# Damo12320/OptixPathtracer

Measured on AMD Instinct MI355X. Metric: Msamples/sec at 1920x1080, max-depth 8; MSE vs reference, higher is better.
Workload: dtype f32; 1 GPU; BASELINE configs[1]: Diffuse sphere-in-box 1920x1080, 1024 spp, depth 8, 1xMI355X; scene=sphere_box_diffuse, triangles=34570, width=1920, height=1080, max_depth=8, material_mode=lambert, kernel=auto (wavefront), frames_per_launch=128, wavefront_streams=1, parallelism=spp-shard x1, batch_frames=128, queue_bytes=55207544320, queue_budget_bytes=77305217024, bvh_builder=auto (GPU binned SAH + GPU SAH-optimal BVH4 collapse), primary_dedup=True

## Files before the change

### include/ptamd.h

```cpp
#ifndef PTAMD_H
#define PTAMD_H
#include <stddef.h>
#include <stdint.h>

#ifdef __cplusplus
extern "C" {
#endif

#define PT_OK 0
#define PT_ERR_INVALID (-1)
#define PT_ERR_HIP (-2)
#define PT_ERR_STATE (-3)
#define PT_ERR_NOMEM (-4)

#define PT_MAT_DEFAULT 0
#define PT_MAT_LAMBERT 1
#define PT_MAT_CONDUCTOR 2
#define PT_MAT_DIELECTRIC 3
#define PT_MAT_LAYERED 4

#define PT_KERNEL_MEGA 0
#define PT_KERNEL_WAVEFRONT 1
#define PT_BVH_AUTO 0
#define PT_BVH_LBVH 1
// ... 21 lines not shown

typedef struct pt_texture {
    const uint32_t* rgba8;
    int32_t width;
    int32_t height;
} pt_texture;

typedef struct pt_scene {
    const pt_mesh* meshes;
    int32_t n_meshes;
    const pt_texture* textures;
    int32_t n_textures;
} pt_scene;

typedef struct pt_point_light {
    float position[3];
    float color[3];
} pt_point_light;

typedef struct pt_options {
    int32_t device;
    int32_t material_mode;
    int32_t kernel;
    int32_t bvh_builder;
    int32_t n_devices;
    int32_t reserved[3];
    const int32_t* device_list;
} pt_options;

typedef struct pt_stats {
    uint64_t segments;
    uint64_t samples;
    double last_render_ms;
    double total_render_ms;
    uint64_t render_calls;
    uint64_t kernel_launches;
    double bvh_build_ms;
    int32_t bvh_nodes;
    int32_t triangles;
    int32_t frames_per_launch;
    int32_t bvh_depth;
    uint64_t nodes_visited;
    uint64_t tri_tests;
    uint64_t rays;
    uint64_t stack_overflows;
    double trace_kernel_ms;
    uint64_t trace_kernel_launches;
    uint64_t shadow_rays;
    uint64_t trace_kernel_rays;
    uint64_t trace_kernel_bytes;
    uint64_t strict_retraces;
    uint64_t wave_steps;
    uint64_t wave_active_lanes;
    uint64_t wave_node_steps;
    uint64_t wave_tri_steps;
    uint64_t wave_refills;
    uint64_t lds_nodes_visited;
    double shade_kernel_ms;
    uint64_t shade_kernel_launches;
    uint64_t shade_kernel_items;
    uint64_t frames_rendered_ahead;
    uint64_t frames_served_ahead;
    uint64_t look_ahead_cancelled;
    double pair_kernel_ms;
    uint64_t pair_kernel_launches;
    uint64_t pair_kernel_rays;
    uint64_t pair_kernel_bytes;
    uint64_t pair_kernel_shadow_rays;
    uint64_t nee_unoccluded;
    uint64_t queue_bytes;
    uint64_t queue_budget;
    int32_t last_streams;
    int32_t last_batch_frames;
    uint64_t look_ahead_held;
    uint64_t lit_table_answers;
    uint64_t lit_table_cells;
    uint64_t lit_table_bits_set;
    uint64_t lit_table_bytes;
    double lit_table_build_ms;
    uint64_t occluder_table_bytes;
    uint64_t occluder_table_candidates;
    double occluder_table_build_ms;
    uint64_t occluder_table_answers;
    uint64_t geometry_commits;
    uint64_t geometry_refits;
    uint64_t geometry_rebuilds;
    double geometry_commit_ms;
    double bvh_sah_cost;
    double bvh_sah_cost_built;
} pt_stats;

typedef struct pt_renderer pt_renderer;

int pt_create(const pt_scene* scene, const pt_options* options, pt_renderer** out);
int pt_destroy(pt_renderer* r);

int pt_resize(pt_renderer* r, int32_t width, int32_t height);
int pt_set_camera(pt_renderer* r, const float position[3], const float inverse_view[16],
                  const float inverse_projection[16]);
int pt_set_lights(pt_renderer* r, const pt_point_light* lights, int32_t count);
int pt_set_max_bounces(pt_renderer* r, int32_t max_bounces);
int pt_set_material_mode(pt_renderer* r, int32_t material_mode);
int pt_set_kernel(pt_renderer* r, int32_t kernel);
int pt_set_frames_per_launch(pt_renderer* r, int32_t frames);
int pt_set_queue_budget(pt_renderer* r, int64_t bytes);
int pt_set_debug_hold(pt_renderer* r, int32_t on);
int pt_get_trace_coherence(pt_renderer* r, uint64_t hist[8]);
int pt_set_traversal_stats(pt_renderer* r, int32_t enable);
int pt_set_kernel_timing(pt_renderer* r, int32_t enable);
int pt_set_primary_dedup(pt_renderer* r, int32_t enable);
int pt_set_wavefront_streams(pt_renderer* r, int32_t streams);
int pt_set_band_split(pt_renderer* r, int32_t enable);
int pt_set_lit_table(pt_renderer* r, int32_t enable);
typedef struct pt_lit_table_info {
    int32_t active;
    int32_t lights;
    uint32_t triangles;
    uint32_t cells;
    uint32_t words_per_light;
    float delta;
    float margin;
} pt_lit_table_info;
int pt_lit_table_download(pt_renderer* r, pt_lit_table_info* info, uint32_t* tri_words, int64_t tri_bytes,
                          uint32_t* bits, int64_t bits_bytes);
int pt_set_occluder_table(pt_renderer* r, int32_t enable);
int pt_occluder_table_download(pt_renderer* r, int64_t* entries_out, int32_t* entries, int64_t bytes);
int pt_occluder_table_upload(pt_renderer* r, const int32_t* entries, int64_t bytes);

typedef struct pt_launch_params {
    struct {
        float* color_buffer;
        int32_t size[2];
        uint32_t id;
    } frame;
    struct {
        float position[3];
        float inverse_view_matrix[16];
        float inverse_projection_matrix[16];
    } camera;
    const pt_point_light* point_lights;
    int32_t point_light_count;
    int32_t max_bounces;
} pt_launch_params;

int pt_launch(pt_renderer* r, const pt_launch_params* params);

int pt_set_mesh_transform(pt_renderer* r, int32_t mesh, const float model_matrix[16]);
int pt_set_mesh_vertices(pt_renderer* r, int32_t mesh, const float* vertices, const float* normals);
#define PT_GEOM_REFIT 0
#define PT_GEOM_REBUILD 1
int pt_commit_geometry(pt_renderer* r, int32_t how);

int pt_render(pt_renderer* r, float* host_rgb);
int pt_set_render_ahead(pt_renderer* r, int32_t frames);
int pt_set_render_ahead_budget(pt_renderer* r, float max_ms);

int pt_accum_clear(pt_renderer* r);
int pt_render_frames(pt_renderer* r, uint32_t first_frame_id, uint32_t n_frames);
int pt_render_accumulate(pt_renderer* r, uint32_t spp, uint32_t first_frame_id, float* host_rgb_mean);
int pt_set_accum_device_buffer(pt_renderer* r, float* device_sum_rgb);
float* pt_accum_device_ptr(pt_renderer* r);
int pt_accum_download(pt_renderer* r, float* host_rgb, float scale);
int pt_set_accum_fp64(pt_renderer* r, int32_t on);
double* pt_accum_device_ptr64(pt_renderer* r);
int pt_accum_download64(pt_renderer* r, double* host_rgb);

int pt_synchronize(pt_renderer* r);
void* pt_stream(pt_renderer* r);
int32_t pt_device_count(const pt_renderer* r);
int pt_devices(const pt_renderer* r, int32_t* devices, int32_t max);
uint32_t pt_frame_id(const pt_renderer* r);
int pt_set_frame_id(pt_renderer* r, uint32_t frame_id);
int pt_get_stats(pt_renderer* r, pt_stats* out);
int pt_stats_reset(pt_renderer* r);

int pt_camera_from_blender(const float blender_position[3], const float blender_rotation_deg[3],
                           float fov_deg, int32_t width, int32_t height, float position[3],
                           float inverse_view[16], float inverse_projection[16]);

int pt_trace_rays(pt_renderer* r, const float* host_rays, int32_t n, int32_t* prim, float* t,
                  float* u, float* v, int32_t* backface, int32_t any_hit);

typedef struct pt_debug_bounce {
    int32_t bounce;
    int32_t prim;
    float position[3];
    float albedo[3];
    float shading_normal[3];
    float geometry_normal[3];
    float roughness, metallic;
    float beta[3];
    float radiance[3];
} pt_debug_bounce;
int pt_set_debug_pixel(pt_renderer* r, int32_t x, int32_t y, uint32_t frame_id);
int pt_get_debug_path(pt_renderer* r, pt_debug_bounce* out, int32_t max, int32_t* n_bounces);

int pt_bvh_download(pt_renderer* r, void* nodes, int64_t node_bytes, void* triangles, int64_t triangle_bytes);

const char* pt_last_error(void);
const char* pt_version(void);

int pt_display_reset(pt_renderer* r, int32_t max_samples);
int pt_display_add_frame(pt_renderer* r, int32_t* samples);
int pt_display_download(pt_renderer* r, float* rgb);

#define PT_AOV_ALBEDO 0
#define PT_AOV_NORMAL 1
#define PT_AOV_GEOM_NORMAL 2
#define PT_AOV_POSITION 3
#define PT_AOV_DEPTH 4
// ... 99 lines not shown
```

### optixpathtracer_amd/capi.py

```python
from __future__ import annotations

import ctypes as C
import os
from pathlib import Path

_HERE = Path(__file__).resolve().parent
LIB_PATH = _HERE / "libptamd.so"

PT_MAT_DEFAULT, PT_MAT_LAMBERT, PT_MAT_CONDUCTOR, PT_MAT_DIELECTRIC, PT_MAT_LAYERED = range(5)
PT_KERNEL_MEGA, PT_KERNEL_WAVEFRONT, PT_KERNEL_AUTO = 0, 1, 2
PT_BVH_AUTO, PT_BVH_LBVH, PT_BVH_SAH, PT_BVH_PLOC, PT_BVH_SAH_GPU = 0, 1, 2, 3, 4
PT_GEOM_REFIT, PT_GEOM_REBUILD = 0, 1
PT_OK, PT_ERR_INVALID, PT_ERR_HIP, PT_ERR_STATE, PT_ERR_NOMEM = 0, -1, -2, -3, -4

MATERIAL_MODES = {
    "default": PT_MAT_DEFAULT,
    "lambert": PT_MAT_LAMBERT,
    "conductor": PT_MAT_CONDUCTOR,
    "dielectric": PT_MAT_DIELECTRIC,
    "layered": PT_MAT_LAYERED,
}


class PTError(RuntimeError):
# ... 40 lines not shown

class pt_options(C.Structure):
    _fields_ = [
        ("device", C.c_int32),
        ("material_mode", C.c_int32),
        ("kernel", C.c_int32),
        ("bvh_builder", C.c_int32),
        ("n_devices", C.c_int32),
        ("reserved", C.c_int32 * 3),
        ("device_list", C.POINTER(C.c_int32)),
    ]


class pt_debug_bounce(C.Structure):
    _fields_ = [
        ("bounce", C.c_int32),
        ("prim", C.c_int32),
        ("position", C.c_float * 3),
        ("albedo", C.c_float * 3),
        ("shading_normal", C.c_float * 3),
        ("geometry_normal", C.c_float * 3),
        ("roughness", C.c_float),
        ("metallic", C.c_float),
        ("beta", C.c_float * 3),
        ("radiance", C.c_float * 3),
    ]


class pt_stats(C.Structure):
    _fields_ = [
        ("segments", C.c_uint64),
        ("samples", C.c_uint64),
        ("last_render_ms", C.c_double),
        ("total_render_ms", C.c_double),
        ("render_calls", C.c_uint64),
        ("kernel_launches", C.c_uint64),
        ("bvh_build_ms", C.c_double),
        ("bvh_nodes", C.c_int32),
        ("triangles", C.c_int32),
        ("frames_per_launch", C.c_int32),
        ("bvh_depth", C.c_int32),
        ("nodes_visited", C.c_uint64),
        ("tri_tests", C.c_uint64),
        ("rays", C.c_uint64),
        ("stack_overflows", C.c_uint64),
        ("trace_kernel_ms", C.c_double),
        ("trace_kernel_launches", C.c_uint64),
        ("shadow_rays", C.c_uint64),
        ("trace_kernel_rays", C.c_uint64),
        ("trace_kernel_bytes", C.c_uint64),
        ("strict_retraces", C.c_uint64),
        ("wave_steps", C.c_uint64),
        ("wave_active_lanes", C.c_uint64),
        ("wave_node_steps", C.c_uint64),
        ("wave_tri_steps", C.c_uint64),
        ("wave_refills", C.c_uint64),
        ("lds_nodes_visited", C.c_uint64),
        ("shade_kernel_ms", C.c_double),
        ("shade_kernel_launches", C.c_uint64),
        ("shade_kernel_items", C.c_uint64),
        ("frames_rendered_ahead", C.c_uint64),
        ("frames_served_ahead", C.c_uint64),
        ("look_ahead_cancelled", C.c_uint64),
        ("pair_kernel_ms", C.c_double),
        ("pair_kernel_launches", C.c_uint64),
        ("pair_kernel_rays", C.c_uint64),
        ("pair_kernel_bytes", C.c_uint64),
        ("pair_kernel_shadow_rays", C.c_uint64),
        ("nee_unoccluded", C.c_uint64),
        ("queue_bytes", C.c_uint64),
        ("queue_budget", C.c_uint64),
        ("last_streams", C.c_int32),
        ("last_batch_frames", C.c_int32),
        ("look_ahead_held", C.c_uint64),
        ("lit_table_answers", C.c_uint64),
        ("lit_table_cells", C.c_uint64),
        ("lit_table_bits_set", C.c_uint64),
        ("lit_table_bytes", C.c_uint64),
        ("lit_table_build_ms", C.c_double),
        ("occluder_table_bytes", C.c_uint64),
        ("occluder_table_candidates", C.c_uint64),
        ("occluder_table_build_ms", C.c_double),
        ("occluder_table_answers", C.c_uint64),
        ("geometry_commits", C.c_uint64),
        ("geometry_refits", C.c_uint64),
        ("geometry_rebuilds", C.c_uint64),
        ("geometry_commit_ms", C.c_double),
        ("bvh_sah_cost", C.c_double),
        ("bvh_sah_cost_built", C.c_double),
    ]


class pt_lit_table_info(C.Structure):
    _fields_ = [("active", C.c_int32), ("lights", C.c_int32), ("triangles", C.c_uint32), ("cells", C.c_uint32),
                ("words_per_light", C.c_uint32), ("delta", C.c_float), ("margin", C.c_float)]


PT_AOV_ALBEDO, PT_AOV_NORMAL, PT_AOV_GEOM_NORMAL, PT_AOV_POSITION, PT_AOV_DEPTH, PT_AOV_PRIM, PT_AOV_ROUGH_METAL = range(7)
PT_DENOISE_SRC_ACCUM, PT_DENOISE_SRC_DISPLAY, PT_DENOISE_SRC_HOST = range(3)

AOV_KINDS = {
    "albedo": PT_AOV_ALBEDO,
    "normal": PT_AOV_NORMAL,
    "geom_normal": PT_AOV_GEOM_NORMAL,
    "position": PT_AOV_POSITION,
    "depth": PT_AOV_DEPTH,
    "prim": PT_AOV_PRIM,
    "rough_metal": PT_AOV_ROUGH_METAL,
}


class pt_denoise_options(C.Structure):
    _fields_ = [("struct_size", C.c_uint32), ("iterations", C.c_int32), ("demodulate", C.c_int32),
                ("sigma_color", C.c_float), ("sigma_normal", C.c_float), ("sigma_position", C.c_float),
                ("albedo_floor", C.c_float)]


class pt_denoise_info(C.Structure):
    _fields_ = [("struct_size", C.c_uint32), ("iterations", C.c_int32), ("gbuffer_renders", C.c_uint64),
                ("hit_pixels", C.c_uint64), ("gbuffer_ms", C.c_double), ("filter_ms", C.c_double)]


PT_TEMPORAL_HISTORY_LENGTH, PT_TEMPORAL_MOMENTS, PT_TEMPORAL_VARIANCE, PT_TEMPORAL_COLOR = range(4)

TEMPORAL_KINDS = {
    "history_length": PT_TEMPORAL_HISTORY_LENGTH,
    "moments": PT_TEMPORAL_MOMENTS,
    "variance": PT_TEMPORAL_VARIANCE,
    "color": PT_TEMPORAL_COLOR,
}


class pt_temporal_options(C.Structure):
    _fields_ = [("struct_size", C.c_uint32), ("alpha", C.c_float), ("alpha_moments", C.c_float),
                ("max_history", C.c_int32), ("normal_cos", C.c_float), ("plane_distance", C.c_float),
                ("sigma_luminance", C.c_float), ("variance_history", C.c_int32), ("motion_vectors", C.c_int32)]


class pt_temporal_info(C.Structure):
    _fields_ = [("struct_size", C.c_uint32), ("history_valid", C.c_int32), ("calls", C.c_uint64),
                ("reprojected_pixels", C.c_uint64), ("reset_pixels", C.c_uint64), ("temporal_ms", C.c_double),
                ("variance_ms", C.c_double), ("filter_ms", C.c_double), ("moved_pixels", C.c_uint64),
                ("snapshot_ms", C.c_double), ("motion_used", C.c_int32), ("reserved", C.c_int32)]


PT_MOTION_BARYCENTRIC, PT_MOTION_PREV_POSITION, PT_MOTION_SCREEN = range(3)

MOTION_KINDS = {
    "barycentric": PT_MOTION_BARYCENTRIC,
    "prev_position": PT_MOTION_PREV_POSITION,
    "screen": PT_MOTION_SCREEN,
}


class _pt_launch_frame(C.Structure):
    _fields_ = [("color_buffer", C.c_void_p), ("size", C.c_int32 * 2), ("id", C.c_uint32)]


class _pt_launch_camera(C.Structure):
    _fields_ = [("position", C.c_float * 3), ("inverse_view_matrix", C.c_float * 16),
                ("inverse_projection_matrix", C.c_float * 16)]


class pt_launch_params(C.Structure):
    _fields_ = [("frame", _pt_launch_frame), ("camera", _pt_launch_camera), ("point_lights", C.c_void_p),
                ("point_light_count", C.c_int32), ("max_bounces", C.c_int32)]


_FP = C.POINTER(C.c_float)
_IP = C.POINTER(C.c_int32)
_R = C.c_void_p
_M = C.c_void_p
pt_image_decode_fn = C.CFUNCTYPE(C.c_int, C.c_void_p, C.c_size_t, C.POINTER(C.c_int32), C.POINTER(C.c_int32),
                                 C.c_void_p, C.c_void_p)

SIGNATURES = {
    "pt_create": (C.c_int, [C.POINTER(pt_scene), C.POINTER(pt_options), C.POINTER(C.c_void_p)]),
    "pt_destroy": (C.c_int, [_R]),
    "pt_resize": (C.c_int, [_R, C.c_int32, C.c_int32]),
    "pt_set_camera": (C.c_int, [_R, _FP, _FP, _FP]),
    "pt_set_lights": (C.c_int, [_R, C.POINTER(pt_point_light), C.c_int32]),
    "pt_set_max_bounces": (C.c_int, [_R, C.c_int32]),
    "pt_set_material_mode": (C.c_int, [_R, C.c_int32]),
    "pt_set_kernel": (C.c_int, [_R, C.c_int32]),
    "pt_set_mesh_transform": (C.c_int, [_R, C.c_int32, _FP]),
    "pt_set_mesh_vertices": (C.c_int, [_R, C.c_int32, _FP, _FP]),
    "pt_commit_geometry": (C.c_int, [_R, C.c_int32]),
    "pt_set_frames_per_launch": (C.c_int, [_R, C.c_int32]),
    "pt_set_render_ahead": (C.c_int, [_R, C.c_int32]),
    "pt_set_render_ahead_budget": (C.c_int, [_R, C.c_float]),
    "pt_set_queue_budget": (C.c_int, [_R, C.c_int64]),
    "pt_get_trace_coherence": (C.c_int, [_R, C.POINTER(C.c_uint64)]),
    "pt_set_debug_hold": (C.c_int, [_R, C.c_int32]),
    "pt_set_traversal_stats": (C.c_int, [_R, C.c_int32]),
    "pt_set_kernel_timing": (C.c_int, [_R, C.c_int32]),
    "pt_render": (C.c_int, [_R, _FP]),
    "pt_launch": (C.c_int, [_R, C.POINTER(pt_launch_params)]),
    "pt_accum_clear": (C.c_int, [_R]),
    "pt_render_frames": (C.c_int, [_R, C.c_uint32, C.c_uint32]),
    "pt_set_primary_dedup": (C.c_int, [_R, C.c_int32]),
    "pt_set_band_split": (C.c_int, [_R, C.c_int32]),
    "pt_set_wavefront_streams": (C.c_int, [_R, C.c_int32]),
    "pt_set_lit_table": (C.c_int, [_R, C.c_int32]),
    "pt_lit_table_download": (C.c_int, [_R, C.POINTER(pt_lit_table_info), C.c_void_p, C.c_int64, C.c_void_p,
                                        C.c_int64]),
    "pt_set_occluder_table": (C.c_int, [_R, C.c_int32]),
    "pt_occluder_table_download": (C.c_int, [_R, C.POINTER(C.c_int64), C.c_void_p, C.c_int64]),
    "pt_occluder_table_upload": (C.c_int, [_R, C.c_void_p, C.c_int64]),
    "pt_render_accumulate": (C.c_int, [_R, C.c_uint32, C.c_uint32, _FP]),
    "pt_set_accum_device_buffer": (C.c_int, [_R, C.c_void_p]),
    "pt_accum_device_ptr": (C.c_void_p, [_R]),
    "pt_accum_download": (C.c_int, [_R, _FP, C.c_float]),
    "pt_set_accum_fp64": (C.c_int, [_R, C.c_int32]),
    "pt_accum_device_ptr64": (C.c_void_p, [_R]),
    "pt_accum_download64": (C.c_int, [_R, C.POINTER(C.c_double)]),
    "pt_synchronize": (C.c_int, [_R]),
    "pt_stream": (C.c_void_p, [_R]),
    "pt_device_count": (C.c_int32, [_R]),
    "pt_devices": (C.c_int, [_R, C.POINTER(C.c_int32), C.c_int32]),
    "pt_frame_id": (C.c_uint32, [_R]),
    "pt_set_frame_id": (C.c_int, [_R, C.c_uint32]),
    "pt_get_stats": (C.c_int, [_R, C.POINTER(pt_stats)]),
    "pt_stats_reset": (C.c_int, [_R]),
    "pt_camera_from_blender": (C.c_int, [_FP, _FP, C.c_float, C.c_int32, C.c_int32, _FP, _FP, _FP]),
    "pt_trace_rays": (C.c_int, [_R, _FP, C.c_int32, _IP, _FP, _FP, _FP, _IP, C.c_int32]),
    "pt_bvh_download": (C.c_int, [_R, C.c_void_p, C.c_int64, C.c_void_p, C.c_int64]),
    "pt_set_debug_pixel": (C.c_int, [_R, C.c_int32, C.c_int32, C.c_uint32]),
    "pt_get_debug_path": (C.c_int, [_R, C.POINTER(pt_debug_bounce), C.c_int32, C.POINTER(C.c_int32)]),
    "pt_last_error": (C.c_char_p, []),
    "pt_version": (C.c_char_p, []),
    "pt_display_reset": (C.c_int, [_R, C.c_int32]),
    "pt_display_add_frame": (C.c_int, [_R, C.POINTER(C.c_int32)]),
    "pt_display_download": (C.c_int, [_R, _FP]),
    "pt_aov_channels": (C.c_int, [C.c_int32]),
    "pt_aov_download": (C.c_int, [_R, C.c_int32, C.c_void_p, C.c_int64]),
    "pt_aov_device_ptr": (C.c_void_p, [_R, C.c_int32]),
    "pt_denoise_options_default": (C.c_int, [C.POINTER(pt_denoise_options)]),
    "pt_denoise": (C.c_int, [_R, C.c_int32, _FP, C.c_float, C.POINTER(pt_denoise_options), _FP]),
    "pt_denoised_device_ptr": (C.c_void_p, [_R]),
    "pt_get_denoise_info": (C.c_int, [_R, C.POINTER(pt_denoise_info)]),
    "pt_temporal_options_default": (C.c_int, [C.POINTER(pt_temporal_options)]),
    "pt_denoise_temporal": (C.c_int, [_R, C.c_int32, _FP, C.c_float, C.POINTER(pt_temporal_options),
                                      C.POINTER(pt_denoise_options), _FP]),
    "pt_temporal_reset": (C.c_int, [_R]),
    "pt_temporal_channels": (C.c_int, [C.c_int32]),
    "pt_temporal_download": (C.c_int, [_R, C.c_int32, C.c_void_p, C.c_int64]),
    "pt_get_temporal_info": (C.c_int, [_R, C.POINTER(pt_temporal_info)]),
    "pt_motion_channels": (C.c_int, [C.c_int32]),
    "pt_motion_download": (C.c_int, [_R, C.c_int32, C.c_void_p, C.c_int64]),
    "pt_model_load_gltf": (C.c_int, [C.c_char_p, pt_image_decode_fn, C.c_void_p, C.POINTER(_M)]),
    "pt_model_scene": (C.POINTER(pt_scene), [_M]),
    "pt_model_mesh_name": (C.c_char_p, [_M, C.c_int32]),
    "pt_model_destroy": (C.c_int, [_M]),
    "pt_model_last_error": (C.c_char_p, []),
    "pt_image_decode_png": (C.c_int, [C.c_void_p, C.c_size_t, C.POINTER(C.c_int32), C.POINTER(C.c_int32),
                                      C.c_void_p]),
    "pt_image_write_exr": (C.c_int, [C.c_char_p, _FP, C.c_int32, C.c_int32]),
    "pt_image_write_bmp": (C.c_int, [C.c_char_p, _FP, C.c_int32, C.c_int32]),
    "pt_image_write_pfm": (C.c_int, [C.c_char_p, _FP, C.c_int32, C.c_int32]),
    "pt_image_read": (C.c_int, [C.c_char_p, _FP, C.POINTER(C.c_int32), C.POINTER(C.c_int32)]),
    "pt_image_mse": (C.c_double, [_FP, _FP, C.c_int64]),
    "pt_image_flip": (C.c_double, [_FP, _FP, C.c_int32, C.c_int32, C.c_float, _FP]),
    "pt_image_last_error": (C.c_char_p, []),
}

_lib = None


def load(path: str | os.PathLike | None = None) -> C.CDLL:
    global _lib
    if _lib is not None and path is None:
        return _lib
    p = Path(path) if path else Path(os.environ.get("PTAMD_LIB", LIB_PATH))
    if not p.exists():
        raise PTError(
            f"{p} not found: the HIP extension is not built (run `python -c 'import __graft_entry__ as g; g.build()'`)"
        )
    lib = C.CDLL(str(p))
    variant = path is None and "PTAMD_LIB" in os.environ
    for name, (res, args) in SIGNATURES.items():
        if variant and not hasattr(lib, name):
            continue
        fn = getattr(lib, name)
        fn.restype = res
        fn.argtypes = args
    if path is None:
        _lib = lib
    return lib


def check(status: int, what: str = "") -> None:
# ... 12 lines not shown
```

### optixpathtracer_amd/csrc/pt_capi.cpp

```cpp
#include "pt_renderer.h"

using namespace pt;

namespace pt {

thread_local std::string g_last_error;

int fail(int code, const std::string& msg) {
    g_last_error = msg;
    return code;
}
int hip_fail(hipError_t e, const char* where) {
    g_last_error = std::string(where) + ": " + hipGetErrorString(e);
    return e == hipErrorOutOfMemory ? PT_ERR_NOMEM : PT_ERR_HIP;
}

}

pt_renderer::~pt_renderer() {
    wavefront_free(wf);
    for (int k = 1; k < kMaxWFStreams; ++k) wavefront_free(xwf[k]);
}

namespace {
// ... 744 lines not shown
    *n_bounces = 0;
    if (!r->d_debug) return fail(PT_ERR_STATE, "pt_get_debug_path: call pt_set_debug_pixel first");
    PT_HIP(hipSetDevice(r->device), "hipSetDevice");
    PT_HIP(hipStreamSynchronize(r->stream), "hipStreamSynchronize");
    std::vector<pt_debug_bounce> rec(kDebugMaxBounces);
    PT_HIP(hipMemcpy(rec.data(), r->d_debug, sizeof(pt_debug_bounce) * rec.size(), hipMemcpyDeviceToHost),
           "download debug records");
    int n = 0;
    while (n < kDebugMaxBounces && rec[(size_t)n].bounce == n + 1) ++n;
    *n_bounces = n;
    for (int k = 0; k < n && k < max; ++k) out[k] = rec[(size_t)k];
    return PT_OK;
}

extern "C" int pt_set_traversal_stats(pt_renderer* r, int32_t enable) {
    if (!r) return fail(PT_ERR_INVALID, "pt_set_traversal_stats: NULL");
    r->trav_stats = enable != 0;
    for (pt_renderer* p : r->multi.peers) p->trav_stats = enable != 0;
    return PT_OK;
}

extern "C" int pt_set_wavefront_streams(pt_renderer* r, int32_t streams) {
    if (!r || streams < 0 || streams > pt_renderer::kMaxWFStreams)
        return fail(PT_ERR_INVALID, "pt_set_wavefront_streams: 0 (auto) or 1 to 4");
    int rc = collect_pending(r);
    if (rc != PT_OK) return rc;
    r->wf_streams = streams;
    for (pt_renderer* p : r->multi.peers)
        if ((rc = pt_set_wavefront_streams(p, streams)) != PT_OK) return rc;
    return PT_OK;
}

extern "C" int pt_set_primary_dedup(pt_renderer* r, int32_t enable) {
    if (!r) return fail(PT_ERR_INVALID, "pt_set_primary_dedup: NULL");
    int rc = collect_pending(r);
    if (rc) return rc;
    r->primary_dedup = enable != 0;
    for (pt_renderer* p : r->multi.peers) {
        if ((rc = pt_set_primary_dedup(p, enable)) != PT_OK) return rc;
    }
    return PT_OK;
}

extern "C" int pt_set_lit_table(pt_renderer* r, int32_t enable) {
    if (!r) return fail(PT_ERR_INVALID, "pt_set_lit_table: NULL");
    const int mode = enable < 0 ? -1 : (enable > 0 ? 1 : 0);
    r->lit.mode = mode;
    for (pt_renderer* p : r->multi.peers) p->lit.mode = mode;
    return PT_OK;
}

extern "C" int pt_lit_table_download(pt_renderer* r, pt_lit_table_info* info, uint32_t* tri_words, int64_t tri_bytes,
                                     uint32_t* bits, int64_t bits_bytes) {
    if (!r || !info) return fail(PT_ERR_INVALID, "pt_lit_table_download: NULL");
    PT_HIP(hipSetDevice(r->device), "hipSetDevice");
    return lit_table_download(r, info, tri_words, tri_bytes, bits, bits_bytes);
}

extern "C" int pt_set_occluder_table(pt_renderer* r, int32_t enable) {
    if (!r) return fail(PT_ERR_INVALID, "pt_set_occluder_table: NULL");
    const int mode = enable < 0 ? -1 : (enable > 0 ? 1 : 0);
    r->occ.mode = mode;
    for (pt_renderer* p : r->multi.peers) p->occ.mode = mode;
    return PT_OK;
}

extern "C" int pt_occluder_table_download(pt_renderer* r, int64_t* entries_out, int32_t* entries, int64_t bytes) {
    if (!r || !entries_out) return fail(PT_ERR_INVALID, "pt_occluder_table_download: NULL");
    PT_HIP(hipSetDevice(r->device), "hipSetDevice");
    return occ_table_download(r, entries_out, entries, bytes);
}

extern "C" int pt_occluder_table_upload(pt_renderer* r, const int32_t* entries, int64_t bytes) {
    if (!r || !entries) return fail(PT_ERR_INVALID, "pt_occluder_table_upload: NULL");
    PT_HIP(hipSetDevice(r->device), "hipSetDevice");
    int rc = occ_table_upload(r, entries, bytes);
    if (rc) return rc;
    for (pt_renderer* p : r->multi.peers) {
        if ((rc = pt_occluder_table_upload(p, entries, bytes)) != PT_OK) return rc;
    }
    return PT_OK;
}

extern "C" int pt_set_band_split(pt_renderer* r, int32_t enable) {
    if (!r) return fail(PT_ERR_INVALID, "pt_set_band_split: NULL");
    int rc = collect_pending(r);
    if (rc) return rc;
    r->band_split = enable != 0;
    for (pt_renderer* p : r->multi.peers) {
        if ((rc = pt_set_band_split(p, enable)) != PT_OK) return rc;
    }
    return PT_OK;
}

extern "C" int pt_set_kernel_timing(pt_renderer* r, int32_t enable) {
    if (!r) return fail(PT_ERR_INVALID, "pt_set_kernel_timing: NULL");
    int rc = collect_pending(r);
    if (rc) return rc;
    r->timing.kernel_timing = enable != 0;
    for (pt_renderer* p : r->multi.peers) {
        if ((rc = pt_set_kernel_timing(p, enable)) != PT_OK) return rc;
    }
    return PT_OK;
}
```

### optixpathtracer_amd/csrc/pt_capi_launch.cpp

```cpp
#include "pt_renderer.h"

using namespace pt;

namespace {

int next_event_pair(pt_renderer* r, hipEvent_t* a, hipEvent_t* b) {
    PT_HIP(r->timing.ev.next(a, b), "hipEventCreate");
    return PT_OK;
}

DevLaunch make_launch(const pt_renderer* r, float* accum, uint32_t frame_base, uint32_t n_frames,
                      double* accum64 = nullptr, size_t frame_stride = 0) {
    DevLaunch L;
    L.width = r->width;
    L.height = r->height;
    L.row0 = 0;
    L.image_height = r->height;
    std::memcpy(L.cam_pos, r->cam_pos, sizeof L.cam_pos);
    std::memcpy(L.inv_view, r->inv_view, sizeof L.inv_view);
    std::memcpy(L.inv_proj, r->inv_proj, sizeof L.inv_proj);
    L.lights = r->d_lights;
    L.n_lights = r->n_lights;
    L.max_bounces = r->max_bounces;
    L.frame_base = frame_base;
    L.n_frames = n_frames;
    L.accum = accum;
    L.accum64 = accum64;
    L.frame_stride = frame_stride;
    L.counters = r->d_counters;
    L.debug_pixel = r->d_debug ? r->debug_pixel : -1;
    L.debug_frame = r->debug_frame;
    L.debug = r->d_debug;
    L.lit_tri = r->lit.active ? r->lit.d_tri.get() : nullptr;
    L.lit_bits = r->lit.d_bits;
    L.lit_words = r->lit.words;
    L.occ_tab = r->lit.active && r->occ.active ? r->occ.d_tab.get() : nullptr;
    L.lit_cells = r->lit.cells;
    return L;
}

}

namespace pt {

size_t queue_bytes_held(const pt_renderer* r) {
    size_t b = r->wf.paths > 0 ? wavefront_bytes(r->wf.paths, r->wf.max_bounces) : 0;
    for (int k = 1; k < pt_renderer::kMaxWFStreams; ++k)
        if (r->xwf[k].paths > 0) b += wavefront_bytes(r->xwf[k].paths, r->xwf[k].max_bounces);
    return b;
}

size_t queue_budget_bytes(const pt_renderer* r) {
    if (r->queue_budget < 0) return SIZE_MAX;
    if (r->queue_budget > 0) return (size_t)r->queue_budget;
    size_t total = 0;
    if (hipDeviceTotalMem(&total, r->device) != hipSuccess || total == 0) {
        (void)hipGetLastError();
        return SIZE_MAX;
    }
    return total / 4;
}

}

namespace {

constexpr int kMaxWFPaths = 1 << 28;

struct WFPlan {
    int nf_cap = 1;
    int ns = 1;
    bool bands = false;
};

int reserve_queues(pt_renderer* r, WFPlan* plan, size_t budget) {
    const int P = r->width * r->height;
    const int maxb = std::max(1, r->max_bounces);
    int& nf_cap = plan->nf_cap;
    for (int k = 0; k < plan->ns; ++k) {
        WFState& w = k ? r->xwf[k] : r->wf;
        const bool over = budget != SIZE_MAX && w.paths > P &&
                          (size_t)plan->ns * wavefront_bytes(w.paths, w.max_bounces) > budget;
        if (w.paths < P * nf_cap || w.max_bounces < r->max_bounces || over) {
            for (int j = 0; j < pt_renderer::kMaxWFStreams; ++j)
                if (r->wf_stream(j)) PT_HIP(hipStreamSynchronize(r->wf_stream(j)), "hipStreamSynchronize");
            wavefront_free(w);
            hipError_t ae = wavefront_alloc(w, P * nf_cap, maxb);
            if (ae == hipErrorOutOfMemory && k == 0) {
                bool freed = false;
                for (int j = 1; j < pt_renderer::kMaxWFStreams; ++j)
                    if (r->xwf[j].paths > 0) {
                        wavefront_free(r->xwf[j]);
                        freed = true;
                    }
                if (freed) ae = wavefront_alloc(w, P * nf_cap, maxb);
            }
            while (ae == hipErrorOutOfMemory && k == 0 && nf_cap > 1) {
                nf_cap = (nf_cap + 1) / 2;
                r->nf_fit = nf_cap;
                ae = wavefront_alloc(w, P * nf_cap, maxb);
            }
            if (ae == hipErrorOutOfMemory && k > 0) {
                plan->ns = k;
                break;
            }
            PT_HIP(ae, "wavefront_alloc");
        }
    }
    return PT_OK;
}

int plan_wavefront(pt_renderer* r, uint32_t n, WFPlan* plan) {
    const int P = r->width * r->height;
    const int maxb = std::max(1, r->max_bounces);
    const int nf_full = std::max(1, std::min({r->frames_per_launch, (int)std::min<uint32_t>(n, 1u << 20),
                                              kMaxWFPaths / std::max(1, P)}));
    if (r->nf_fit > 0 && r->nf_fit < nf_full) {
        size_t free_b = 0, total_b = 0;
        if (hipMemGetInfo(&free_b, &total_b) == hipSuccess) {
            if (free_b + queue_bytes_held(r) >= wavefront_bytes(P * nf_full, maxb)) r->nf_fit = 0;
// ... 10 lines not shown
    const size_t budget = queue_budget_bytes(r);
    if (budget != SIZE_MAX) {
        const size_t per_frame = wavefront_bytes(P, maxb);
        const int nf_b = (int)std::max<size_t>(1, budget / ((size_t)ns * per_frame));
        nf_cap = std::min(nf_cap, nf_b);
        size_t used = (size_t)ns * wavefront_bytes(P * nf_cap, maxb);
        for (int k = ns; k < pt_renderer::kMaxWFStreams; ++k) {
            if (r->xwf[k].paths == 0) continue;
            const size_t held = wavefront_bytes(r->xwf[k].paths, r->xwf[k].max_bounces);
            if (used + held <= budget) {
                used += held;
                continue;
            }
            PT_HIP(hipStreamSynchronize(r->xstream[k]), "hipStreamSynchronize");
            wavefront_free(r->xwf[k]);
        }
    }
    plan->nf_cap = nf_cap;
    plan->ns = ns;
    plan->bands = bands;
    const int rc = reserve_queues(r, plan, budget);
    if (rc != PT_OK) return rc;
    r->last_streams = plan->ns;
    r->last_batch = plan->nf_cap;
    return PT_OK;
}

int fork_resources(pt_renderer* r, int ns, int nband) {
    if (ns > 1) {
        PT_HIP(r->ev_fork.ensure(hipEventDisableTiming), "hipEventCreate");
        for (Event& e : r->ev_accum) PT_HIP(e.ensure(hipEventDisableTiming), "hipEventCreate");
    }
    for (int k = 1; k < ns; ++k)
        if (!r->xstream[k]) {
            PT_HIP(r->xstream[k].create(), "hipStreamCreate");
            PT_HIP(r->ev_join[k].ensure(hipEventDisableTiming), "hipEventCreate");
        }
    if (nband > 1) PT_HIP(r->ev_band0.ensure(hipEventDisableTiming), "hipEventCreate");
    return PT_OK;
}

int timing_events(pt_renderer* r, bool fused, const hipEvent_t** tev, const hipEvent_t** sev) {
    pt_renderer::Timing& t = r->timing;
    *tev = *sev = nullptr;
    if (!t.kernel_timing) return PT_OK;
    t.tev_frame.resize(2 * (size_t)(r->max_bounces + 1));
    for (int k = 0; k <= r->max_bounces; ++k)
        PT_HIP((k > 0 && fused ? t.pev : t.tev).next(&t.tev_frame[2 * k], &t.tev_frame[2 * k + 1]), "hipEventCreate");
    *tev = t.tev_frame.data();
    t.sev_frame.resize(2 * (size_t)(r->max_bounces + 1));
    for (int k = 0; k <= r->max_bounces; ++k)
        PT_HIP(t.sev.next(&t.sev_frame[2 * k], &t.sev_frame[2 * k + 1]), "hipEventCreate");
    *sev = t.sev_frame.data();
    return PT_OK;
}

WFState batch_queues(pt_renderer* r, int sk, bool speculative, bool first_batch) {
    WFState wq = sk ? r->xwf[sk] : r->wf;
    if (speculative && r->ahead.d_cancel_seen) {
        wq.cancel_host = r->ahead.cancel.d;
        wq.cancel_seen = r->ahead.d_cancel_seen;
        wq.cancel_epoch = r->ahead.cancel_epoch;
        if (r->ahead.debug_hold && r->ahead.hold.d && first_batch) {
            wq.hold_release = r->ahead.hold.d;
            r->ahead.held++;
        }
    }
    return wq;
}

int enqueue_wavefront(pt_renderer* r, const WFPlan& plan, float* accum, uint32_t first, uint32_t n, double* accum64,
                      size_t frame_stride, bool speculative) {
    int rc = PT_OK;
    const DevScene S = r->scene();
    const bool fused = r->material_mode == PT_MAT_LAMBERT || r->material_mode == PT_MAT_CONDUCTOR ||
                       r->material_mode == PT_MAT_DIELECTRIC;
    const int ns = plan.ns, nf_cap = plan.nf_cap;
    const bool dual = ns > 1;
    const int nband = plan.bands && ns > 1 ? 2 : 1;
    if ((rc = fork_resources(r, ns, nband)) != PT_OK) return rc;
    int dev_cus = 256;
    (void)hipDeviceGetAttribute(&dev_cus, hipDeviceAttributeMultiprocessorCount, r->device);
    if ((rc = lit_prepare(r)) != PT_OK) return rc;
    hipEvent_t a = nullptr, b = nullptr;
    if (dual) {
        rc = next_event_pair(r, &a, &b);
        if (rc) return rc;
        PT_HIP(hipEventRecord(a, r->stream), "hipEventRecord");
        PT_HIP(hipEventRecord(r->ev_fork, r->stream), "hipEventRecord");
        for (int k = 1; k < ns; ++k) PT_HIP(hipStreamWaitEvent(r->xstream[k], r->ev_fork, 0), "hipStreamWaitEvent");
    }
    const int rows0 = r->height * 7 / 16;
    r->band0_rows = nband > 1 ? rows0 : 0;
    int batch = 0;
    for (uint32_t f = 0; f < n; ++batch) {
        const int nf = (int)std::min<uint32_t>((uint32_t)nf_cap, n - f);
        DevLaunch L = make_launch(r, frame_stride ? accum + (size_t)f * frame_stride : accum, first + f,
                                  (uint32_t)nf, accum64, frame_stride);
        const int band = nband > 1 ? batch : 0;
        if (nband > 1) {
            L.row0 = band == 0 ? 0 : rows0;
            L.height = band == 0 ? rows0 : r->height - rows0;
            const size_t off = 3 * (size_t)r->width * (size_t)L.row0;
            L.accum += off;
            if (L.accum64) L.accum64 += off;
        }
        const int sk = batch % ns;
        hipStream_t st = r->wf_stream(sk);
        if (!dual) {
            rc = next_event_pair(r, &a, &b);
            if (rc) return rc;
        }
        const hipEvent_t* tev = nullptr;
        const hipEvent_t* sev = nullptr;
        if ((rc = timing_events(r, fused, &tev, &sev)) != PT_OK) return rc;
        if (!dual) PT_HIP(hipEventRecord(a, r->stream), "hipEventRecord");
        int n_timed = 0, n_stimed = 0;
        const WFState wq = batch_queues(r, sk, speculative, batch == 0);
        const hipEvent_t accum_wait = dual && batch > 0 && nband == 1 ? r->ev_accum[(batch - 1) & 1].e : nullptr;
        const hipEvent_t accum_done = dual && nband == 1 ? r->ev_accum[batch & 1].e : nullptr;
        PT_HIP(launch_wavefront_frame(r->material_mode, r->trav_stats, S, L, wq, first + f,
                                      nf, r->primary_dedup, dev_cus, st, tev, &n_timed,
                                      accum_wait, accum_done, sev, &n_stimed, ns == 1 && r->wide_trace),
               "wavefront launch");
        if (tev) {
            const int unused = r->max_bounces + 1 - n_timed;
            const int unused_pair = fused ? std::min(unused, r->max_bounces) : 0;
            r->timing.pev.give_back((size_t)unused_pair);
            r->timing.tev.give_back((size_t)(unused - unused_pair));
        }
        if (sev) r->timing.sev.give_back((size_t)(r->max_bounces + 1 - n_stimed));
        if (!dual) PT_HIP(hipEventRecord(b, r->stream), "hipEventRecord");
        if (nband > 1 && band == 0) PT_HIP(hipEventRecord(r->ev_band0, st), "hipEventRecord");
        if (band + 1 == nband) f += (uint32_t)nf;
    }
    if (dual) {
        for (int k = 1; k < ns; ++k) {
            PT_HIP(hipEventRecord(r->ev_join[k], r->xstream[k]), "hipEventRecord");
            PT_HIP(hipStreamWaitEvent(r->stream, r->ev_join[k], 0), "hipStreamWaitEvent");
        }
        PT_HIP(hipEventRecord(b, r->stream), "hipEventRecord");
    }
    return PT_OK;
}

int enqueue_megakernel(pt_renderer* r, int kernel, float* accum, uint32_t first, uint32_t n) {
    const DevScene S = r->scene();
    const uint32_t chunk = (uint32_t)std::max(1, r->frames_per_launch);
    for (uint32_t done = 0; done < n;) {
        uint32_t k = std::min(chunk, n - done);
        DevLaunch L = make_launch(r, accum, first + done, k);
        hipEvent_t a, b;
        const int rc = next_event_pair(r, &a, &b);
        if (rc) return rc;
        PT_HIP(hipEventRecord(a, r->stream), "hipEventRecord");
        PT_HIP(launch_render(kernel, r->material_mode, r->trav_stats, S, L, r->stream), "render launch");
        PT_HIP(hipEventRecord(b, r->stream), "hipEventRecord");
        done += k;
    }
    return PT_OK;
}

}

namespace pt {

int launch_frames(pt_renderer* r, float* accum, uint32_t first, uint32_t n, double* accum64, size_t frame_stride,
                  bool speculative) {
    int rc = PT_OK;
    const pt_renderer::Timing& t = r->timing;
    if (t.ev.used + t.tev.used + t.pev.used + t.sev.used > kMaxPendingEvents && (rc = collect_pending(r)) != PT_OK)
        return rc;
    r->timing.pending = true;
    r->band0_rows = 0;
    r->lit.active = false;
    int kernel = r->kernel;
    if (kernel == PT_KERNEL_AUTO) kernel = PT_KERNEL_WAVEFRONT;
    if (accum64 && kernel != PT_KERNEL_WAVEFRONT)
        return fail(PT_ERR_INVALID, "fp64 accumulation (pt_set_accum_fp64) runs with the wavefront kernel");
    if (frame_stride && kernel != PT_KERNEL_WAVEFRONT)
        return fail(PT_ERR_INVALID, "per-frame images (render-ahead) run with the wavefront kernel");
    if (kernel == PT_KERNEL_WAVEFRONT) {
        WFPlan plan;
        if ((rc = plan_wavefront(r, n, &plan)) != PT_OK) return rc;
        rc = enqueue_wavefront(r, plan, accum, first, n, accum64, frame_stride, speculative);
    } else {
        rc = enqueue_megakernel(r, kernel, accum, first, n);
    }
    if (rc != PT_OK) return rc;
    r->timing.samples += (uint64_t)n * (uint64_t)r->width * (uint64_t)r->height;
    r->timing.calls++;
    return PT_OK;
}

int render_frames_multi(pt_renderer* r, uint32_t first, uint32_t n) {
    const int N = (int)r->multi.comms.size();
    const size_t count = 3 * (size_t)r->width * (size_t)r->height;
    uint32_t f = first;
    for (int g = 0; g < N; ++g) {
        const uint32_t per = n / (uint32_t)N, extra = n % (uint32_t)N;
        const uint32_t ng = per + ((uint32_t)g < extra ? 1u : 0u);
        pt_renderer* d = g == 0 ? r : r->multi.peers[(size_t)g - 1];
        if (ng > 0) {
            PT_HIP(hipSetDevice(d->device), "hipSetDevice");
            const int rc = launch_frames(d, g == 0 ? r->multi.d_part : d->accum(), f, ng,
                                         r->accum64 ? (g == 0 ? r->multi.d_part64 : d->d_accum64) : nullptr);
            if (rc) return rc;
        }
        f += ng;
    }
    ncclResult_t nr = ncclGroupStart();
    for (int g = 0; g < N && nr == ncclSuccess; ++g) {
        pt_renderer* d = g == 0 ? r : r->multi.peers[(size_t)g - 1];
        if (r->accum64) {
            const double* send = g == 0 ? r->multi.d_part64 : d->d_accum64;
            double* recv = g == 0 ? r->d_accum64 : d->d_accum64;
            nr = ncclReduce(send, recv, count, ncclFloat64, ncclSum, 0, r->multi.comms[(size_t)g], d->stream);
        } else {
            const float* send = g == 0 ? r->multi.d_part : d->accum();
            float* recv = g == 0 ? r->accum() : d->accum();
            nr = ncclReduce(send, recv, count, ncclFloat32, ncclSum, 0, r->multi.comms[(size_t)g], d->stream);
        }
    }
    const ncclResult_t ne = ncclGroupEnd();
    (void)hipSetDevice(r->device);
    if (nr != ncclSuccess || ne != ncclSuccess)
        return fail(PT_ERR_HIP, std::string("ncclReduce: ") + ncclGetErrorString(nr != ncclSuccess ? nr : ne));
    if (r->accum64) PT_HIP(accum_f64_to_f32(r->d_accum64, r->accum(), count, r->stream), "fp64 -> fp32 sum");
    return PT_OK;
}

}
```

### optixpathtracer_amd/csrc/pt_capi_scene.cpp

```cpp
#include "pt_renderer.h"

using namespace pt;

namespace {

int need_tex_kernels(pt_renderer* r) {
    if (r->d_texinfo) return PT_OK;
    bool any = false;
    for (int m = 0; m < r->nmesh; ++m) any = any || r->geom.host.normal_mode(m) == 2;
    if (!any) return PT_OK;
    PT_HIP(r->d_texinfo.alloc(1), "hipMalloc texinfo");
    PT_HIP(hipMemset(r->d_texinfo, 0, sizeof(int4)), "hipMemset texinfo");
    return PT_OK;
}

int build_tree(pt_renderer* r, const std::vector<float4>& tri, const std::vector<float4>& nrm, const float cmin[3],
               const float cmax[3], BuildOutput& bo, float* ms_out = nullptr) {
    const size_t ntri = tri.size() / 3;
    DevBuf<float4> d_uv_orig, d_nrm_orig, d_tri_orig;
    hipError_t e = d_tri_orig.alloc(3 * ntri);
    if (e == hipSuccess) e = d_nrm_orig.alloc(3 * ntri);
    if (e == hipSuccess && bo.tuv) e = d_uv_orig.alloc(2 * ntri);
    if (e == hipSuccess && bo.tuv)
        e = hipMemcpyAsync(d_uv_orig, r->geom.host.uvs.data(), sizeof(float4) * 2 * ntri, hipMemcpyHostToDevice,
// ... 96 lines not shown
    r->d_isect.swap(isect);
    r->d_shade.swap(shade);
    r->d_tuv.swap(tuv);
    r->bvh_nodes = bo.n_nodes;
    r->bvh_depth = bo.depth;
    r->geom.level_base = bo.level_base;
    r->geom.commit_ms += bms;
    return PT_OK;
}

}

namespace pt {

int upload_scene(pt_renderer* r, const pt_scene* scene, const std::vector<int4>& texinfo, size_t ntexel) {
    const std::vector<float4>& mats = r->geom.mats;
    const int ntex = scene->n_textures;
    PT_HIP(r->stream.create(), "hipStreamCreate");
    PT_HIP(r->dl_stream.create(), "hipStreamCreate");
    PT_HIP(r->xstream[1].create(), "hipStreamCreate");
    PT_HIP(r->ev_join[1].ensure(hipEventDisableTiming), "hipEventCreate");
    PT_HIP(r->d_counters.alloc(kCounters), "hipMalloc counters");
    PT_HIP(hipMemsetAsync(r->d_counters, 0, kCounters * sizeof(unsigned long long), r->stream), "hipMemset");
    PT_HIP(r->d_mats.alloc(mats.size()), "hipMalloc mats");
    PT_HIP(hipMemcpyAsync(r->d_mats, mats.data(), sizeof(float4) * mats.size(), hipMemcpyHostToDevice, r->stream),
           "upload mats");
    if (ntex > 0) {
        PT_HIP(r->d_texinfo.alloc((size_t)ntex), "hipMalloc texinfo");
        PT_HIP(hipMemcpyAsync(r->d_texinfo, texinfo.data(), sizeof(int4) * (size_t)ntex, hipMemcpyHostToDevice,
                              r->stream),
               "upload texinfo");
        PT_HIP(r->d_texels.alloc(ntexel), "hipMalloc texels");
        for (int k = 0; k < ntex; ++k) {
            const pt_texture& tx = scene->textures[k];
            PT_HIP(hipMemcpy(r->d_texels + texinfo[(size_t)k].x, tx.rgba8,
                             sizeof(uint32_t) * (size_t)tx.width * (size_t)tx.height, hipMemcpyHostToDevice),
                   "upload texels");
        }
    }
    return need_tex_kernels(r);
}

int build_scene(pt_renderer* r, bool any_tex) {
    const size_t ntri = (size_t)r->ntri;
    if (ntri > 0) {
        std::vector<float4> tri, nrm;
        float cmin[3], cmax[3];
        bake_scene(r->geom.host, tri, nrm, cmin, cmax);
        if (any_tex) PT_HIP(r->d_tuv.alloc(2 * ntri), "hipMalloc tuv");
        PT_HIP(r->d_isect.alloc(3 * ntri), "hipMalloc isect");
        PT_HIP(r->d_shade.alloc(4 * ntri), "hipMalloc shade");
        PT_HIP(r->d_nodes.alloc(std::max<size_t>(1, ntri)), "hipMalloc nodes");
        BuildOutput bo;
        bo.nodes = r->d_nodes;
        bo.isect = r->d_isect;
        bo.shade = r->d_shade;
        bo.tuv = r->d_tuv;
        int rc = build_tree(r, tri, nrm, cmin, cmax, bo);
        if (rc != PT_OK) return rc;
        r->bvh_nodes = bo.n_nodes;
        r->bvh_depth = bo.depth;
        r->geom.level_base = bo.level_base;
        if (3 * bo.depth > kMinTraversalStack)
            return fail(PT_ERR_INVALID, "pt_create: BVH too deep for the traversal stack (depth " +
                                            std::to_string(bo.depth) + ")");
        const size_t nv = r->geom.host.verts.size();
        PT_HIP(r->geom.d_overts.alloc(std::max<size_t>(1, nv)), "hipMalloc vertices");
        PT_HIP(r->geom.d_onorms.alloc(std::max<size_t>(1, nv)), "hipMalloc normals");
        PT_HIP(r->geom.d_tidx.alloc(ntri), "hipMalloc indices");
        PT_HIP(r->geom.d_rmesh.alloc((size_t)std::max(1, r->nmesh)), "hipMalloc mesh records");
        PT_HIP(r->geom.d_sah_part.alloc((size_t)sah_partial_blocks((int)ntri) + 1), "hipMalloc SAH partials");
        PT_HIP(r->geom.ev[0].ensure(), "hipEventCreate");
        PT_HIP(r->geom.ev[1].ensure(), "hipEventCreate");
        if (nv > 0) {
            PT_HIP(hipMemcpy(r->geom.d_overts, r->geom.host.verts.data(), sizeof(float4) * nv, hipMemcpyHostToDevice),
                   "upload vertices");
            PT_HIP(hipMemcpy(r->geom.d_onorms, r->geom.host.norms.data(), sizeof(float4) * nv, hipMemcpyHostToDevice),
                   "upload normals");
        }
        PT_HIP(hipMemcpy(r->geom.d_tidx, r->geom.host.tidx.data(), sizeof(int4) * ntri, hipMemcpyHostToDevice),
               "upload indices");
        if ((rc = sah_cost_now(r, true)) != PT_OK) return rc;
        if ((rc = lit_resubdivide(r)) != PT_OK) return rc;
    }
    PT_HIP(hipStreamSynchronize(r->stream), "hipStreamSynchronize");
    return PT_OK;
}

int commit_geometry(pt_renderer* r, int how) {
    cancel_look_ahead(r, true);
    PT_HIP(hipStreamSynchronize(r->stream), "hipStreamSynchronize");
    for (int k = 1; k < pt_renderer::kMaxWFStreams; ++k)
        if (r->xstream[k]) PT_HIP(hipStreamSynchronize(r->xstream[k]), "hipStreamSynchronize");
    if (r->dl_stream) PT_HIP(hipStreamSynchronize(r->dl_stream), "hipStreamSynchronize");
    int rc = collect_pending(r);
    if (rc) return rc;

    std::vector<RefitMesh> rm((size_t)std::max(1, r->nmesh));
    if ((rc = apply_staged(r, rm)) != PT_OK) return rc;
    r->geom.any_staged = false;
    r->geom.version++;
    r->geom.commits++;
    r->geom.commit_ms = 0.0;
    if (r->ntri <= 0) {
        if (how == PT_GEOM_REBUILD) r->geom.rebuilds++;
        else r->geom.refits++;
        return PT_OK;
    }

    PT_HIP(hipMemcpy(r->d_mats, r->geom.mats.data(), sizeof(float4) * r->geom.mats.size(), hipMemcpyHostToDevice),
           "upload mats");
    if ((rc = need_tex_kernels(r)) != PT_OK) return rc;
    PT_HIP(hipMemcpy(r->geom.d_rmesh, rm.data(), sizeof(RefitMesh) * rm.size(), hipMemcpyHostToDevice),
           "upload mesh records");
    PT_HIP(hipEventRecord(r->geom.ev[0], r->stream), "hipEventRecord");
    PT_HIP(refit_rebake(r->geom.d_rmesh, r->geom.d_overts, r->geom.d_onorms, r->geom.d_tidx, r->ntri, r->d_isect,
                        r->d_shade, r->stream),
           "k_rebake");
    PT_HIP(refit_levels(r->d_nodes, r->d_isect, r->geom.level_base, r->stream), "k_refit_level");
    if ((rc = sah_cost_now(r, false, r->geom.ev[1])) != PT_OK) return rc;
    float ms = 0.0f;
    PT_HIP(hipEventElapsedTime(&ms, r->geom.ev[0], r->geom.ev[1]), "hipEventElapsedTime");
    r->geom.commit_ms = ms;

    int rebuild_rc = PT_OK;
    std::string rebuild_msg;
    if (how == PT_GEOM_REBUILD) {
        rebuild_rc = rebuild_tree(r);
        if (rebuild_rc != PT_OK) rebuild_msg = g_last_error;
        if (rebuild_rc == PT_OK && (rc = sah_cost_now(r, true)) != PT_OK) return rc;
    }
    if (how == PT_GEOM_REBUILD && rebuild_rc == PT_OK) r->geom.rebuilds++;
    else r->geom.refits++;

    if ((rc = lit_resubdivide(r)) != PT_OK) return rc;
    if (rebuild_rc != PT_OK) return fail(rebuild_rc, rebuild_msg);
    return PT_OK;
}

}
```

### optixpathtracer_amd/csrc/pt_capi_stats.cpp

```cpp
#include "pt_renderer.h"

using namespace pt;

namespace pt {

int collect_pending(pt_renderer* r) {
    if (!r->timing.pending) return PT_OK;
    double sum = 0.0, tsum = 0.0, ssum = 0.0;
    size_t n = 0, tn = 0, sn = 0;
    PT_HIP(r->timing.ev.collect(&sum, &n), "frame events");
    PT_HIP(r->timing.tev.collect(&tsum, &tn), "trace-kernel events");
    double psum = 0.0;
    size_t pn = 0;
    PT_HIP(r->timing.pev.collect(&psum, &pn), "pair-kernel events");
    tsum += psum;
    tn += pn;
    r->timing.pair_ms += psum;
    r->timing.pair_launches += pn;
    PT_HIP(r->timing.sev.collect(&ssum, &sn), "shading-kernel events");
    r->ahead.spec_pending = false;
    r->timing.launches += n;
    r->timing.last_ms = sum;
    r->timing.total_ms += sum;
    r->timing.trace_ms += tsum;
    r->timing.trace_launches += tn;
    r->timing.shade_ms += ssum;
    r->timing.shade_launches += sn;
    r->timing.pending = false;
    return PT_OK;
}

}

namespace {

constexpr uint64_t pt_stats::*kSummed[] = {
    &pt_stats::segments, &pt_stats::samples, &pt_stats::nodes_visited, &pt_stats::tri_tests, &pt_stats::rays,
    &pt_stats::stack_overflows, &pt_stats::wave_steps, &pt_stats::wave_active_lanes, &pt_stats::wave_node_steps,
    &pt_stats::wave_tri_steps, &pt_stats::wave_refills, &pt_stats::lds_nodes_visited, &pt_stats::shade_kernel_items,
    &pt_stats::shadow_rays, &pt_stats::trace_kernel_rays, &pt_stats::trace_kernel_bytes, &pt_stats::strict_retraces,
    &pt_stats::nee_unoccluded,
    &pt_stats::pair_kernel_rays, &pt_stats::pair_kernel_bytes, &pt_stats::pair_kernel_shadow_rays,
    &pt_stats::lit_table_answers, &pt_stats::occluder_table_answers, &pt_stats::queue_bytes};

int table_stats(pt_renderer* r, pt_stats* out) {
    r->lit.built.harvest();
    if (lit_wanted(r) && table_current(r, r->lit.built)) {
        const size_t nw = (size_t)r->lit.words * (size_t)r->lit.built.n;
        if (r->lit.built.count < 0) {
            std::vector<uint32_t> hb(nw);
            PT_HIP(hipMemcpy(hb.data(), r->lit.d_bits, sizeof(uint32_t) * nw, hipMemcpyDeviceToHost),
                   "download lit table");
            int64_t n = 0;
            for (uint32_t w : hb) n += __builtin_popcount(w);
            r->lit.built.count = n;
        }
        out->lit_table_cells = r->lit.cells;
        out->lit_table_bits_set = (uint64_t)r->lit.built.count;
        out->lit_table_bytes = sizeof(uint32_t) * ((size_t)r->ntri + (size_t)r->lit.words * kLitMaxLights);
        out->lit_table_build_ms = r->lit.built.build_ms;
    }
    r->occ.built.harvest();
    if (occ_wanted(r) && r->occ.d_tab && table_current(r, r->occ.built)) {
        const size_t ne = (size_t)r->lit.cells * (size_t)r->occ.built.n;
        if (r->occ.built.count < 0) {
            std::vector<int> ho(ne);
            PT_HIP(hipMemcpy(ho.data(), r->occ.d_tab, sizeof(int) * ne, hipMemcpyDeviceToHost), "download occluder table");
            int64_t n = 0;
            for (int t : ho) n += t >= 0;
            r->occ.built.count = n;
        }
        out->occluder_table_bytes = sizeof(int) * ne;
        out->occluder_table_candidates = (uint64_t)r->occ.built.count;
        out->occluder_table_build_ms = r->occ.built.build_ms;
    }
    return PT_OK;
}

}

extern "C" {

int pt_get_stats(pt_renderer* r, pt_stats* out) {
    if (!r || !out) return fail(PT_ERR_INVALID, "pt_get_stats: NULL");
    int rc = pt_synchronize(r);
    if (rc) return rc;
    unsigned long long c[kCounters];
    PT_HIP(hipMemcpy(c, r->d_counters, sizeof c, hipMemcpyDeviceToHost), "download counters");
    std::memset(out, 0, sizeof *out);
    out->segments = c[kCtrSegments];
    out->samples = r->timing.samples;
    out->last_render_ms = r->timing.last_ms;
    out->total_render_ms = r->timing.total_ms;
    out->render_calls = r->timing.calls;
    out->kernel_launches = r->timing.launches;
    out->frames_per_launch = r->frames_per_launch;
    out->bvh_build_ms = r->timing.bvh_ms;
    out->bvh_nodes = r->bvh_nodes;
    out->bvh_depth = r->bvh_depth;
    out->nodes_visited = c[kCtrNodes];
    out->tri_tests = c[kCtrTriTests];
    out->rays = c[kCtrRays];
    out->stack_overflows = c[kCtrStackOverflows];
    out->triangles = r->ntri;
    out->trace_kernel_ms = r->timing.trace_ms;
    out->trace_kernel_launches = r->timing.trace_launches;
    out->pair_kernel_ms = r->timing.pair_ms;
    out->pair_kernel_launches = r->timing.pair_launches;
    out->shadow_rays = c[kCtrShadowRays];
    out->trace_kernel_rays = c[kCtrTraceRays];
    out->trace_kernel_bytes = c[kCtrTraceBytes];
    out->strict_retraces = c[kCtrRetraces];
    out->wave_steps = c[kCtrWaveSteps];
    out->wave_active_lanes = c[kCtrWaveActive];
    out->wave_node_steps = c[kCtrWaveNodeSteps];
    out->wave_tri_steps = c[kCtrWaveTriSteps];
    out->wave_refills = c[kCtrWaveRefills];
    out->lds_nodes_visited = c[kCtrLdsNodes];
    out->shade_kernel_ms = r->timing.shade_ms;
    out->shade_kernel_launches = r->timing.shade_launches;
    out->shade_kernel_items = c[kCtrShadeItems];
    out->frames_rendered_ahead = r->ahead.rendered;
    out->frames_served_ahead = r->ahead.served;
    out->look_ahead_cancelled = r->ahead.cancelled;
    out->pair_kernel_rays = c[kCtrPairRays];
    out->pair_kernel_bytes = c[kCtrPairBytes];
    out->pair_kernel_shadow_rays = c[kCtrPairShadowRays];
    out->nee_unoccluded = c[kCtrNeeUnoccluded];
    out->queue_bytes = queue_bytes_held(r);
    const size_t qb = queue_budget_bytes(r);
    out->queue_budget = qb == SIZE_MAX ? 0 : qb;
    out->last_streams = r->last_streams;
    out->last_batch_frames = r->last_batch;
    out->look_ahead_held = r->ahead.held;
    out->lit_table_answers = c[kCtrLitAnswers];
    out->occluder_table_answers = c[kCtrOccAnswers];
    if ((rc = table_stats(r, out)) != PT_OK) return rc;
    out->geometry_commits = r->geom.commits;
    out->geometry_refits = r->geom.refits;
    out->geometry_rebuilds = r->geom.rebuilds;
    out->geometry_commit_ms = r->geom.commit_ms;
    out->bvh_sah_cost = r->geom.sah_cost;
    out->bvh_sah_cost_built = r->geom.sah_cost_built;
    for (pt_renderer* p : r->multi.peers) {
        pt_stats ps;
        rc = pt_get_stats(p, &ps);
        if (rc) return rc;
        for (uint64_t pt_stats::*f : kSummed) out->*f += ps.*f;
    }
    return PT_OK;
}

int pt_stats_reset(pt_renderer* r) {
    if (!r) return fail(PT_ERR_INVALID, "pt_stats_reset: NULL");
    int rc = pt_synchronize(r);
    if (rc) return rc;
    for (pt_renderer* p : r->multi.peers) {
        if ((rc = pt_stats_reset(p)) != PT_OK) return rc;
    }
    PT_HIP(hipSetDevice(r->device), "hipSetDevice");
    PT_HIP(hipMemset(r->d_counters, 0, kCounters * sizeof(unsigned long long)), "hipMemset counters");
    r->timing.reset_counts();
    r->ahead.reset_counts();
    return PT_OK;
}

}
```

### optixpathtracer_amd/csrc/pt_capi_tables.cpp

```cpp
#include "pt_renderer.h"

using namespace pt;

namespace pt {

int BuiltTable::begin(hipStream_t stream) {
    PT_HIP(ev[0].ensure(), "hipEventCreate");
    PT_HIP(ev[1].ensure(), "hipEventCreate");
    PT_HIP(hipEventRecord(ev[0], stream), "hipEventRecord");
    return PT_OK;
}
int BuiltTable::end(hipStream_t stream, uint32_t v, const void* l, int nl) {
    PT_HIP(hipEventRecord(ev[1], stream), "hipEventRecord");
    ev_pending = true;
    count = -1;
    version = v;
    lights = l;
    n = nl;
    return PT_OK;
}
void BuiltTable::harvest() {
    if (!ev_pending) return;
    float ms = 0.0f;
    if (hipEventElapsedTime(&ms, ev[0], ev[1]) == hipSuccess)
        build_ms = ms;
    else
        (void)hipGetLastError();
    ev_pending = false;
}
bool table_current(const pt_renderer* r, const BuiltTable& t) {
    return t.current(r->lit.version, r->d_lights, r->n_lights);
}

#ifndef PT_LIT_TABLE
#define PT_LIT_TABLE 1
#endif
bool lit_wanted(const pt_renderer* r) {
    const bool pays = r->material_mode == PT_MAT_LAMBERT || r->material_mode == PT_MAT_DEFAULT ||
                      r->material_mode == PT_MAT_LAYERED;
    const bool on = r->lit.mode < 0 ? PT_LIT_TABLE != 0 && pays && !r->lit.launch_call : r->lit.mode > 0;
    return on && r->lit.d_tri && r->d_lights && r->n_lights >= 1 && r->n_lights <= kLitMaxLights;
}
#ifndef PT_OCC_TABLE
#define PT_OCC_TABLE 1
#endif
bool occ_wanted(const pt_renderer* r) {
    const bool has_code = r->material_mode == PT_MAT_LAMBERT || r->material_mode == PT_MAT_DEFAULT ||
                          r->material_mode == PT_MAT_LAYERED;
    const bool pays = has_code;
    const bool on = r->occ.mode < 0 ? PT_OCC_TABLE != 0 && pays && r->lit.mode < 0 : r->occ.mode > 0;
    return on && has_code && !r->occ.alloc_failed && lit_wanted(r);
}
static int occ_prepare(pt_renderer* r) {
    r->occ.active = occ_wanted(r);
    if (!r->occ.active) return PT_OK;
    if (table_current(r, r->occ.built)) return PT_OK;
    const size_t need = (size_t)r->lit.cells * (size_t)r->n_lights;
    if (need > r->occ.d_tab.size() && r->occ.d_tab.alloc(need) != hipSuccess) {
        r->occ.alloc_failed = true;
        r->occ.active = false;
        return PT_OK;
    }
    int rc = r->occ.built.begin(r->stream);
    if (rc != PT_OK) return rc;
    PT_HIP(occ_build(r->scene(), r->lit.d_tri, r->lit.cells, r->lit.words, r->d_lights, r->n_lights, r->lit.d_bits,
                     r->occ.d_tab, r->stream),
           "occ_build");
    return r->occ.built.end(r->stream, r->lit.version, r->d_lights, r->n_lights);
}
int lit_prepare(pt_renderer* r) {
    r->lit.active = lit_wanted(r);
    r->occ.active = false;
    if (!r->lit.active) return PT_OK;
    if (table_current(r, r->lit.built)) return occ_prepare(r);
    int rc = r->lit.built.begin(r->stream);
    if (rc != PT_OK) return rc;
    PT_HIP(lit_build(r->scene(), r->lit.d_tri, r->lit.cells, r->lit.words, r->d_lights, r->n_lights, r->lit.d_bits,
                     r->lit.diag, r->stream),
           "lit_build");
    if ((rc = r->lit.built.end(r->stream, r->lit.version, r->d_lights, r->n_lights)) != PT_OK) return rc;
    return occ_prepare(r);
}

int lit_resubdivide(pt_renderer* r) {
    const size_t ntri = (size_t)r->ntri;
    std::vector<float4> isect_host(3 * ntri);
    PT_HIP(hipMemcpy(isect_host.data(), r->d_isect, sizeof(float4) * 3 * ntri, hipMemcpyDeviceToHost), "download isect");
    std::vector<uint32_t> lit_words_host;
    uint32_t cells = 0;
    float diag = 0.0f;
    r->lit.version++;
    r->lit.built.invalidate_count();
    if (!lit_subdivide(isect_host.data(), (int)ntri, lit_words_host, &cells, &diag)) {
        r->lit.d_tri.reset();
        r->lit.cells = r->lit.words = 0;
        return PT_OK;
    }
    const uint32_t words = (cells + 31) / 32;
    hipError_t e = hipSuccess;
    if (words > r->lit.words_cap) {
        e = r->lit.d_bits.alloc((size_t)words * kLitMaxLights);
        r->lit.words_cap = e == hipSuccess ? words : 0;
    }
    if (e == hipSuccess && !r->lit.d_tri) e = r->lit.d_tri.alloc(ntri);
    if (e == hipSuccess)
        e = hipMemcpy(r->lit.d_tri, lit_words_host.data(), sizeof(uint32_t) * ntri, hipMemcpyHostToDevice);
    if (e != hipSuccess) {
        r->lit.d_tri.reset();
        r->lit.cells = r->lit.words = 0;
        return hip_fail(e, "lit table");
    }
    r->lit.cells = cells;
    r->lit.words = words;
    r->lit.diag = diag;
    r->occ.alloc_failed = false;
    return PT_OK;
}

int lit_table_download(pt_renderer* r, pt_lit_table_info* info, uint32_t* tri_words, int64_t tri_bytes, uint32_t* bits,
                       int64_t bits_bytes) {
    int rc = lit_prepare(r);
    if (rc) return rc;
    std::memset(info, 0, sizeof *info);
    info->active = r->lit.active ? 1 : 0;
    info->delta = kLitDelta;
    if (!r->lit.active) return PT_OK;
    info->lights = r->n_lights;
    info->triangles = (uint32_t)r->ntri;
    info->cells = r->lit.cells;
    info->words_per_light = r->lit.words;
    info->margin = lit_margin(r->lit.diag);
    PT_HIP(hipStreamSynchronize(r->stream), "hipStreamSynchronize");
    if (tri_words) {
        if (tri_bytes != (int64_t)(sizeof(uint32_t) * (size_t)r->ntri))
            return fail(PT_ERR_INVALID, "pt_lit_table_download: tri_words size mismatch");
        PT_HIP(hipMemcpy(tri_words, r->lit.d_tri, (size_t)tri_bytes, hipMemcpyDeviceToHost), "download lit table");
    }
    if (bits) {
        if (bits_bytes != (int64_t)(sizeof(uint32_t) * (size_t)r->lit.words * (size_t)r->n_lights))
            return fail(PT_ERR_INVALID, "pt_lit_table_download: bits size mismatch");
        PT_HIP(hipMemcpy(bits, r->lit.d_bits, (size_t)bits_bytes, hipMemcpyDeviceToHost), "download lit table");
    }
    return PT_OK;
}

int occ_table_download(pt_renderer* r, int64_t* entries_out, int32_t* entries, int64_t bytes) {
    int rc = lit_prepare(r);
    if (rc) return rc;
    *entries_out = r->occ.active ? (int64_t)r->lit.cells * (int64_t)r->n_lights : 0;
    if (!r->occ.active || !entries) return PT_OK;
    if (bytes != (int64_t)sizeof(int32_t) * *entries_out)
        return fail(PT_ERR_INVALID, "pt_occluder_table_download: size mismatch");
    PT_HIP(hipStreamSynchronize(r->stream), "hipStreamSynchronize");
    PT_HIP(hipMemcpy(entries, r->occ.d_tab, (size_t)bytes, hipMemcpyDeviceToHost), "download occluder table");
    return PT_OK;
}

int occ_table_upload(pt_renderer* r, const int32_t* entries, int64_t bytes) {
    int rc = pt_synchronize(r);
    if (rc) return rc;
    if ((rc = lit_prepare(r)) != PT_OK) return rc;
    if (!r->occ.active) return fail(PT_ERR_INVALID, "pt_occluder_table_upload: the table is not in use");
    const int64_t n = (int64_t)r->lit.cells * (int64_t)r->n_lights;
    if (bytes != (int64_t)sizeof(int32_t) * n) return fail(PT_ERR_INVALID, "pt_occluder_table_upload: size mismatch");
    for (int64_t i = 0; i < n; ++i)
        if (entries[i] < -1 || entries[i] >= r->ntri)
            return fail(PT_ERR_INVALID, "pt_occluder_table_upload: entry out of range");
    PT_HIP(hipStreamSynchronize(r->stream), "hipStreamSynchronize");
    PT_HIP(hipMemcpy(r->occ.d_tab, entries, (size_t)bytes, hipMemcpyHostToDevice), "upload occluder table");
    r->occ.built.invalidate_count();
    return PT_OK;
}

}
```

### optixpathtracer_amd/csrc/pt_device.h

```cpp
#pragma once
#include "pt_bsdf.h"

namespace pt {

constexpr int kEmptyChild = (int)0x80000000;

struct __align__(16) BNode4 {
    float4 lox, hix, loy, hiy, loz, hiz;
    int4 child;
    int4 pad;
};

__device__ __forceinline__ int leaf_first(int c) { return (~c) >> 3; }
__device__ __forceinline__ int leaf_count(int c) { return ((~c) & 7) + 1; }

struct DevScene {
    const BNode4* nodes;
    const float4* isect;
    const float4* shade;
    const float4* mats;
    const float4* tuv;
    const uint32_t* texels;
    const int4* texinfo;
    int ntri;
    int n_nodes;
    const BNode4* lds_nodes;
    int n_lds;
};

constexpr int kMatStride = 6;
constexpr float kNormalNone = 0.0f, kNormalBaked = 1.0f, kNormalObject = 2.0f;
PT_HD float mat_row_dir(float4 row, f3 n) { return (row.x * n.x + row.y * n.y) + (row.z * n.z + row.w * 0.0f); }

struct DevLight {
    float px, py, pz, cr, cg, cb;
};

struct DevLaunch {
    int width, height;
    int row0, image_height;
    float cam_pos[3];
    float inv_view[16];
    float inv_proj[16];
    const DevLight* lights;
    int n_lights;
    int max_bounces;
    uint32_t frame_base;
    uint32_t n_frames;
    float* accum;
    double* accum64;
    size_t frame_stride;
    unsigned long long* counters;
    int debug_pixel;
    uint32_t debug_frame;
    float* debug;
    const uint32_t* lit_tri;
    const uint32_t* lit_bits;
    uint32_t lit_words;
    const int* occ_tab;
    uint32_t lit_cells;
};
enum Counter : int {
    kCtrSegments = 0,
    kCtrNodes,
    kCtrTriTests,
    kCtrRays,
    kCtrStackOverflows,
    kCtrShadowRays,
    kCtrTraceRays,
    kCtrTraceBytes,
    kCtrRetraces,
    kCtrWaveSteps,
    kCtrWaveActive,
    kCtrWaveNodeSteps,
    kCtrWaveTriSteps,
    kCtrWaveRefills,
    kCtrLdsNodes,
    kCtrShadeItems,
    kCtrPairRays,
    kCtrPairBytes,
    kCtrNeeUnoccluded,
    kCtrPairShadowRays,
    kCtrCoh0,
    kCtrCohLanes = kCtrCoh0 + 6,
    kCtrLitAnswers,
    kCtrOccAnswers,
    kCounters
};
static_assert(kCtrCoh0 == 20 && kCounters == 29, "the counter slots keep their numbers");
constexpr int kDebugMaxBounces = 64;
constexpr int kDebugRecordFloats = 22;

__device__ __forceinline__ int debug_path_id(const DevLaunch& L) {
    const uint32_t f = L.debug_frame - L.frame_base;
    const int P = L.width * L.height, p = L.debug_pixel - L.width * L.row0;
    return (L.debug_pixel >= 0 && p >= 0 && p < P && f < L.n_frames) ? (int)f * P + p : -1;
}

struct Hit {
    float t, u, v;
    int tri;
    int orig;
    bool back;
};

#ifndef PT_CYCLE_PROBE
#define PT_CYCLE_PROBE 0
#endif
__device__ __forceinline__ uint64_t probe_clock() {
    __builtin_amdgcn_sched_barrier(0);
    const uint64_t t = __builtin_amdgcn_s_memtime();
    __builtin_amdgcn_sched_barrier(0);
    return t;
}
template <class T>
__device__ __forceinline__ uint64_t probe_clock(const T& dep) {
    T v = dep;
    __asm__ volatile("" : "+v"(v));
    __builtin_amdgcn_s_waitcnt(0);
    return probe_clock();
}

struct TravStats {
    uint32_t nodes = 0, tris = 0, rays = 0, overflow = 0, retrace = 0;
    uint32_t lds_nodes = 0;
    uint32_t unocc = 0;
    uint32_t steps = 0, active = 0, node_steps = 0, tri_steps = 0, refills = 0;
    uint32_t coh[6] = {0, 0, 0, 0, 0, 0};
    uint32_t coh_lanes = 0;
#if PT_CYCLE_PROBE
    uint64_t probe_t = 0;
#endif
};

constexpr float kSlabWiden = 1.000244140625f;
__device__ __forceinline__ float ray_inv(float d) { return d != 0.0f ? 1.0f / d : copysignf(1e30f, d); }
__device__ __forceinline__ f3 safe_inv(f3 d) { return mk(ray_inv(d.x), ray_inv(d.y), ray_inv(d.z)); }

PT_HD float box_pad(float x) { return fabsf(x) * 9.5367431640625e-7f + 1e-6f; }
PT_HD void tri_box_padded(f3 v0, f3 e1, f3 e2, float lo[3], float hi[3]) {
    const float a[3] = {v0.x, v0.y, v0.z}, b[3] = {e1.x, e1.y, e1.z}, c[3] = {e2.x, e2.y, e2.z};
    for (int k = 0; k < 3; ++k) {
        const float p1 = a[k] + b[k], p2 = a[k] + c[k];
        const float l = fminf(fminf(a[k], p1), p2), h = fmaxf(fmaxf(a[k], p1), p2);
        lo[k] = l - box_pad(l);
        hi[k] = h + box_pad(h);
    }
}

__device__ __forceinline__ bool tri_accept(const float4 A, const float4 E1, const float4 E2, f3 inv, f3 io, float t) {
    float lo[3], hi[3];
    tri_box_padded(mk(A.x, A.y, A.z), mk(E1.x, E1.y, E1.z), mk(E2.x, E2.y, E2.z), lo, hi);
    const float ax = __fmaf_rn(lo[0], inv.x, -io.x), bx = __fmaf_rn(hi[0], inv.x, -io.x);
    const float ay = __fmaf_rn(lo[1], inv.y, -io.y), by = __fmaf_rn(hi[1], inv.y, -io.y);
    const float az = __fmaf_rn(lo[2], inv.z, -io.z), bz = __fmaf_rn(hi[2], inv.z, -io.z);
    const float tn = fmaxf(fmaxf(fminf(ax, bx), fminf(ay, by)), fminf(az, bz));
    const float tfk = fminf(fminf(fmaxf(ax, bx), fmaxf(ay, by)), fmaxf(az, bz)) * kSlabWiden;
    return tn <= t * kSlabWiden && t <= tfk && tn <= tfk;
}

__device__ __forceinline__ void cswap(float& ta, int& ca, float& tb, int& cb) {
    bool s = tb < ta;
    float t0 = s ? tb : ta, t1 = s ? ta : tb;
    int c0 = s ? cb : ca, c1 = s ? ca : cb;
    ta = t0; tb = t1; ca = c0; cb = c1;
}

constexpr int kSpillDepth = 64;
#ifndef PT_WF_STACK
#define PT_WF_STACK 11
#endif
#ifndef PT_MK_STACK
#define PT_MK_STACK 32
#endif
constexpr int stack_capacity(int lds) { return (kSpillDepth / (lds / 2)) * (lds / 2) + lds; }

__device__ __forceinline__ float srgb_to_linear(float c) {
    const float m = (c < 0.04045f) ? 0.0f : 1.0f;
    const float a = c / 12.92f;
    const float b = pt_powf_unit((c + 0.055f) / 1.055f, 2.4f);
    return a * (1.0f - m) + b * m;
}
__device__ __forceinline__ int wrapi(int i, int n) {
    const int r = i % n;
    return r < 0 ? r + n : r;
}
__device__ __forceinline__ float4 tex_sample(const DevScene& S, int tex, float x, float y, bool srgb) {
    const int4 ti = S.texinfo[tex];
    const int W = ti.y, H = ti.z;
    x = x - floorf(x);
    y = y - floorf(y);
    const float xb = x * (float)W - 0.5f, yb = y * (float)H - 0.5f;
    const float fx = floorf(xb), fy = floorf(yb);
    const float ax = rintf((xb - fx) * 256.0f) * (1.0f / 256.0f);
    const float ay = rintf((yb - fy) * 256.0f) * (1.0f / 256.0f);
    const int i0 = wrapi((int)fx, W), i1 = wrapi((int)fx + 1, W);
    const int j0 = wrapi((int)fy, H), j1 = wrapi((int)fy + 1, H);
    const uint32_t* px = S.texels + ti.x;
    const uint32_t p00 = px[(size_t)j0 * W + i0], p10 = px[(size_t)j0 * W + i1];
    const uint32_t p01 = px[(size_t)j1 * W + i0], p11 = px[(size_t)j1 * W + i1];
    float o[4];
#pragma unroll
    for (int c = 0; c < 4; ++c) {
        const float t00 = (float)((p00 >> (8 * c)) & 0xff) / 255.0f, t10 = (float)((p10 >> (8 * c)) & 0xff) / 255.0f;
        const float t01 = (float)((p01 >> (8 * c)) & 0xff) / 255.0f, t11 = (float)((p11 >> (8 * c)) & 0xff) / 255.0f;
        const float r0 = t00 * (1.0f - ax) + t10 * ax;
        const float r1 = t01 * (1.0f - ax) + t11 * ax;
        const float v = r0 * (1.0f - ay) + r1 * ay;
        o[c] = srgb ? srgb_to_linear(v) : v;
    }
    return make_float4(o[0], o[1], o[2], o[3]);
}
__device__ __forceinline__ void tri_texcoord(const DevScene& S, int ti, float u, float v, float& x, float& y) {
    const float4 a = S.tuv[2 * ti], b = S.tuv[2 * ti + 1];
    const float w = 1.0f - u - v;
    x = (w * a.x + u * a.z) + v * b.x;
    y = (w * a.y + u * a.w) + v * b.y;
}
__device__ __forceinline__ bool alpha_cut(const DevScene& S, int ti, int mi, float u, float v) {
    const int at = __float_as_int(S.mats[kMatStride * mi + 1].z);
    float x, y;
    tri_texcoord(S, ti, u, v, x, y);
    return tex_sample(S, at, x, y, true).w < 0.9f;
}

struct TravState {
    f3 o, d, inv, io;
    float tmin, best;
    int cur, sp, spc;
    int leaf;
    int nx, ny, nz;
    bool any;
    bool strict;
    int path;
    Hit h;
};

enum { kRayClosest = 0, kRayAny = 1, kRayMixed = 2 };

__device__ __forceinline__ void trav_init(TravState& s, f3 o, f3 d, float tmin, float tmax) {
    s.o = o;
    s.d = d;
    s.inv = safe_inv(d);
    s.io = mk(o.x * s.inv.x, o.y * s.inv.y, o.z * s.inv.z);
    s.nx = s.inv.x < 0.0f ? 16 : 0;
    s.ny = s.inv.y < 0.0f ? 16 : 0;
    s.nz = s.inv.z < 0.0f ? 16 : 0;
    s.tmin = tmin;
    s.best = tmax;
    s.cur = 0;
    s.sp = 0;
    s.spc = 0;
    s.leaf = kEmptyChild;
    s.any = false;
    s.strict = false;
    s.h.tri = -1;
    s.h.orig = 0x7fffffff;
}

template <int ANY>
__device__ __forceinline__ bool is_any(const TravState& s) {
    return ANY == kRayAny || (ANY == kRayMixed && s.any);
}

__device__ __forceinline__ bool tri_test(const float4 A, const float4 E1, const float4 E2, f3 o, f3 d, float tmin,
                                         float tmax, float& th, float& uh, float& vh, bool& back) {
    f3 v0 = mk(A.x, A.y, A.z), e1 = mk(E1.x, E1.y, E1.z), e2 = mk(E2.x, E2.y, E2.z);
    f3 p = cross(d, e2);
    float det = dot(e1, p);
    float inv = 1.0f / det;
    f3 tv = o - v0;
    float u = dot(tv, p) * inv;
    f3 q = cross(tv, e1);
    float v = dot(d, q) * inv;
    float t = dot(e2, q) * inv;
    th = t;
    uh = u;
    vh = v;
    back = det < 0.0f;
    return (det != 0.0f) & !(u < 0.0f || u > 1.0f) & !(v < 0.0f || u + v > 1.0f) & (t >= tmin && t <= tmax);
}

template <int DEPTH, bool STATS>
__device__ __forceinline__ void stack_spill(TravState& s, int* __restrict__ stk, int stride, int* spill,
                                         TravStats& ts) {
    if (s.spc + (DEPTH / 2) <= kSpillDepth) {
        for (int k = 0; k < (DEPTH / 2); ++k) spill[s.spc + k] = stk[k * stride];
        s.spc += (DEPTH / 2);
    } else if (STATS) {
        ts.overflow++;
    }
    for (int k = (DEPTH / 2); k < s.sp; ++k) stk[(k - (DEPTH / 2)) * stride] = stk[k * stride];
    s.sp -= (DEPTH / 2);
}

template <int DEPTH>
__device__ __forceinline__ void stack_refill(TravState& s, int* __restrict__ stk, int stride, const int* spill) {
    s.spc -= (DEPTH / 2);
    for (int k = 0; k < (DEPTH / 2); ++k) stk[k * stride] = spill[s.spc + k];
    s.sp = (DEPTH / 2);
}

typedef float pt_f2 __attribute__((ext_vector_type(2)));

struct NodeLoad {
    float4 ax, bx, ay, by, az, bz;
    int4 ch;
};

__device__ __forceinline__ NodeLoad node_load(const DevScene& S, const TravState& s, int ni) {
    NodeLoad n;
    if (ni < S.n_lds) {
        const char* b = reinterpret_cast<const char*>(S.lds_nodes + ni);
        auto ld = [&](int off) { return *reinterpret_cast<const float4*>(b + off); };
        n.ax = ld(s.nx);
        n.bx = ld(16 - s.nx);
        n.ay = ld(32 + s.ny);
        n.by = ld(48 - s.ny);
        n.az = ld(64 + s.nz);
        n.bz = ld(80 - s.nz);
        n.ch = *reinterpret_cast<const int4*>(b + 96);
        return n;
    }
    const __amdgpu_buffer_rsrc_t rs = __builtin_amdgcn_make_buffer_rsrc((void*)S.nodes, 0, 0x7fffffff, 0x00020000);
    const int nb = ni << 7;
    auto ld = [&](int off) {
        return __builtin_bit_cast(float4, __builtin_amdgcn_raw_buffer_load_b128(rs, nb + off, 0, 0));
    };
    n.ax = ld(s.nx);
    n.bx = ld(16 - s.nx);
    n.ay = ld(32 + s.ny);
    n.by = ld(48 - s.ny);
    n.az = ld(64 + s.nz);
    n.bz = ld(80 - s.nz);
    n.ch = __builtin_bit_cast(int4, __builtin_amdgcn_raw_buffer_load_b128(rs, nb + 96, 0, 0));
    return n;
}

template <int K>
__device__ __forceinline__ void stage_top_nodes(DevScene& S, BNode4* top) {
    const int n = K > 0 ? min(S.n_nodes, K) : 0;
    const float4* src = reinterpret_cast<const float4*>(S.nodes);
    float4* dst = reinterpret_cast<float4*>(top);
    for (int i = (int)threadIdx.x; i < n * 8; i += (int)blockDim.x) dst[i] = src[i];
    __syncthreads();
// ... 139 lines not shown
};

__device__ __forceinline__ int lane_prefix(unsigned long long m) {
    return (int)__builtin_amdgcn_mbcnt_hi((uint32_t)(m >> 32), __builtin_amdgcn_mbcnt_lo((uint32_t)m, 0u));
}

template <int ANY, bool STATS, bool TEX>
__device__ __forceinline__ void wave_tri_batch(const DevScene& S, TravState& s, bool has, TriBatchLds* L,
                                               TravStats& ts) {
    const int lane = (int)(threadIdx.x & 63);
    const int c1 = has ? leaf_count(s.leaf) - 1 : 0;
    const int first = leaf_first(s.leaf);
    const unsigned long long m0 = __ballot(has), m1 = __ballot(has && (c1 & 1)), m2 = __ballot(has && (c1 & 2));
    const int pre = lane_prefix(m0) + lane_prefix(m1) + 2 * lane_prefix(m2);
    const int total = (int)(__popcll(m0) + __popcll(m1) + 2 * __popcll(m2));
    if (has) {
        L->pair[pre] = ((uint32_t)first << 6) | (uint32_t)lane;
        if (c1 >= 1) L->pair[pre + 1] = ((uint32_t)(first + 1) << 6) | (uint32_t)lane;
        if (c1 >= 2) L->pair[pre + 2] = ((uint32_t)(first + 2) << 6) | (uint32_t)lane;
        if (c1 >= 3) L->pair[pre + 3] = ((uint32_t)(first + 3) << 6) | (uint32_t)lane;
        s.leaf = kEmptyChild;
    }
    L->key[lane] = ~0ull;
    const int flags = is_any<ANY>(s) ? 2 : 0;
    __builtin_amdgcn_wave_barrier();
    for (int base = 0; base < total; base += 64) {
        const int k = base + lane;
        const bool valid = k < total;
        const uint32_t pair = L->pair[valid ? k : 0];
        const int owner = (int)(pair & 63u), ti = (int)(pair >> 6);
        const f3 o = mk(__shfl(s.o.x, owner, 64), __shfl(s.o.y, owner, 64), __shfl(s.o.z, owner, 64));
        const f3 d = mk(__shfl(s.d.x, owner, 64), __shfl(s.d.y, owner, 64), __shfl(s.d.z, owner, 64));
        const float tmax = __shfl(s.best, owner, 64);
        bool bk = false;
        float t, u, v;
        if (STATS && valid) ts.tris++;
        const float4 A = S.isect[3 * ti], E1 = S.isect[3 * ti + 1], E2 = S.isect[3 * ti + 2];
        bool hit = tri_test(A, E1, E2, o, d, 0.0f, tmax, t, u, v, bk) && valid;
        if (TEX && hit && __float_as_int(E2.w) != 0) hit = !alpha_cut(S, ti, __float_as_int(E1.w), u, v);
        const int oi = __float_as_int(A.w);
        if (__ballot(hit)) {
            const f3 inv = mk(__shfl(s.inv.x, owner, 64), __shfl(s.inv.y, owner, 64), __shfl(s.inv.z, owner, 64));
            const f3 io = mk(__shfl(s.io.x, owner, 64), __shfl(s.io.y, owner, 64), __shfl(s.io.z, owner, 64));
            if (hit) hit = tri_accept(A, E1, E2, inv, io, t);
        }
        const unsigned long long key =
            ((unsigned long long)(__float_as_uint(t) & 0x7fffffffu) << 32) | (unsigned long long)(uint32_t)oi;
        if (hit) atomicMin(&L->key[owner], key);
        __builtin_amdgcn_wave_barrier();
        if (hit && L->key[owner] == key)
        {
            L->res_uv[owner] = make_float2(u, v);
            L->res_code[owner] = ti | (bk ? (int)0x80000000 : 0);
        }
        __builtin_amdgcn_wave_barrier();
        const unsigned long long w = L->key[lane];
        if (w != ~0ull) {
            const float tw = __uint_as_float((uint32_t)(w >> 32));
            const int ow = (int)(uint32_t)w;
            const float2 ruv = L->res_uv[lane];
            const float4 r = make_float4(ruv.x, ruv.y, __int_as_float(L->res_code[lane]), 0.0f);
            const int code = __float_as_int(r.z);
            if (flags & 2) {
                s.h.tri = code & 0x7fffffff;
                s.path = __float_as_int(tw);
            } else if (tw < s.best || (tw == s.best && ow < s.h.orig)) {
                s.best = tw;
                s.h.t = tw;
                s.h.u = r.x;
                s.h.v = r.y;
                s.h.tri = code & 0x7fffffff;
                s.h.back = code < 0;
                s.h.orig = ow;
            }
            L->key[lane] = ~0ull;
        }
        __builtin_amdgcn_wave_barrier();
    }
}

template <int ANY, bool STATS, int DEPTH>
__device__ __forceinline__ bool trav_node_step(const DevScene& S, TravState& s, int* __restrict__ stk, int stride,
                                               int* spill, TravStats& ts) {
    if (s.cur >= 0) {
        if (STATS) {
            ts.nodes++;
            ts.lds_nodes += s.cur < S.n_lds;
        }
        float t0, t1, t2, t3;
        int c0, c1, c2, c3;
        const NodeLoad nl = node_load(S, s, s.cur);
#if PT_CYCLE_PROBE
        if (STATS) ts.probe_t = probe_clock(nl.ch.x);
#endif
        node_eval(nl, s, t0, t1, t2, t3, c0, c1, c2, c3);
        if (ANY != kRayAny) {
            cswap(t0, c0, t1, c1);
            cswap(t2, c2, t3, c3);
            cswap(t0, c0, t2, c2);
            cswap(t1, c1, t3, c3);
            cswap(t1, c1, t2, c2);
        }
        if (s.sp > DEPTH - 3) stack_spill<DEPTH, STATS>(s, stk, stride, spill, ts);
        {
            int sp = s.sp;
            stk[sp * stride] = c3;
            sp += c3 != kEmptyChild;
            stk[sp * stride] = c2;
            sp += c2 != kEmptyChild;
            stk[sp * stride] = c1;
            sp += c1 != kEmptyChild;
            s.sp = sp;
        }
        s.cur = c0;
    }
    if (s.cur == kEmptyChild) stack_pop<DEPTH>(s, stk, stride, spill);
    if (s.cur < 0 && s.cur != kEmptyChild && s.leaf == kEmptyChild) {
        s.leaf = s.cur;
        stack_pop<DEPTH>(s, stk, stride, spill);
    }
    return s.cur == kEmptyChild && s.leaf == kEmptyChild;
}

template <int ANY>
__device__ __forceinline__ bool trav_hit_acceptable(const TravState& s, const float4 A, const float4 E1,
                                                    const float4 E2) {
    const float t = is_any<ANY>(s) ? __int_as_float(s.path) : s.h.t;
    return tri_accept(A, E1, E2, s.inv, s.io, t);
}
template <int ANY, bool TEX>
__device__ __forceinline__ bool trav_result_ok(const DevScene& S, const TravState& s) {
    if (s.strict || s.h.tri < 0) return true;
    const int ti = s.h.tri;
    return trav_hit_acceptable<ANY>(s, S.isect[3 * ti], S.isect[3 * ti + 1], S.isect[3 * ti + 2]);
}

template <int ANY>
__device__ __forceinline__ void trav_restart_strict(TravState& s, float tmax_closest) {
    s.cur = 0;
    s.sp = 0;
    s.spc = 0;
    s.leaf = kEmptyChild;
    s.strict = true;
    s.h.tri = -1;
    if (!is_any<ANY>(s)) {
        s.best = tmax_closest;
        s.h.orig = 0x7fffffff;
    }
}

template <int ANY, bool STATS, int DEPTH, bool TEX>
__device__ __forceinline__ bool traverse(const DevScene& S, f3 o, f3 d, float tmin, float tmax, Hit& h,
                                         int* __restrict__ stk, int stride, TravStats& ts) {
    if (STATS) ts.rays++;
    TravState s;
    trav_init(s, o, d, tmin, tmax);
    if (S.ntri > 0) {
        int spill[kSpillDepth];
        while (true) {
            while (!trav_step<ANY, STATS, DEPTH, TEX>(S, s, stk, stride, spill, ts)) {
            }
            if (trav_result_ok<ANY, TEX>(S, s)) break;
            if (STATS) ts.retrace++;
            trav_restart_strict<ANY>(s, tmax);
        }
    }
    h = s.h;
    return s.h.tri >= 0;
}

__device__ __forceinline__ void camera_ray(const DevLaunch& L, int x, int y, f3& o, f3& d) {
    float xs = ((float)x + 0.5f) / (float)L.width;
    float ys = ((float)(y + L.row0) + 0.5f) / (float)L.image_height;
    float ndc[4] = {xs * 2.0f - 1.0f, ys * 2.0f - 1.0f, 1.0f, 1.0f};
    float pv[4], pw[4];
    mat4_mul_vec4(L.inv_proj, ndc, pv);
    float pv0[4] = {pv[0], pv[1], pv[2], 0.0f};
    mat4_mul_vec4(L.inv_view, pv0, pw);
    float d4 = (pw[0] * pw[0] + pw[1] * pw[1]) + (pw[2] * pw[2] + pw[3] * pw[3]);
    float inv = 1.0f / sqrtf(d4);
    d = mk(pw[0] * inv, pw[1] * inv, pw[2] * inv);
    o = mk(L.cam_pos[0], L.cam_pos[1], L.cam_pos[2]);
}

struct SurfaceHit {
    f3 pos, ng;
    Frame fr;
    f3 wo;
    f3 albedo;
    float metallic, roughness;
};

__device__ __forceinline__ void apply_textures(const DevScene& S, int ti, float u, float v, const float4 M1,
                                               const float4 M2, f3& albedo, float& metallic, float& roughness,
                                               f3& Ns) {
    const int at = __float_as_int(M1.z), nt = __float_as_int(M1.w), mt = __float_as_int(M2.x);
    float x, y;
    tri_texcoord(S, ti, u, v, x, y);
    f3 ntex = mk(0.0f, 0.0f, 0.0f);
    if (at >= 0) {
        const float4 c = tex_sample(S, at, x, y, true);
        albedo = albedo * mk(c.x, c.y, c.z);
    }
    if (nt >= 0) {
        const float4 c = tex_sample(S, nt, x, y, false);
        ntex = mk(c.x, c.y, c.z);
    }
    if (mt >= 0) {
        const float4 c = tex_sample(S, mt, x, y, false);
        metallic = c.x;
        roughness = c.y;
    }
    if (ntex.x != 0.0f || ntex.y != 0.0f || ntex.z != 0.0f) {
        f3 d1 = cross(Ns, mk(0.0f, 0.0f, 1.0f));
        f3 d2 = cross(Ns, mk(0.0f, 1.0f, 0.0f));
        f3 T0 = (length(d1) > length(d2)) ? d1 : d2;
        T0 = normalize(T0);
        const f3 B0 = cross(T0, Ns);
        const f3 tn = mk(ntex.x * 2.0f - 1.0f, ntex.y * 2.0f - 1.0f, ntex.z * 2.0f - 1.0f);
        Ns = normalize(mk((T0.x * tn.x + B0.x * tn.y) + Ns.x * tn.z, (T0.y * tn.x + B0.y * tn.y) + Ns.y * tn.z,
                          (T0.z * tn.x + B0.z * tn.y) + Ns.z * tn.z));
    }
}

template <bool TEX>
__device__ __forceinline__ void reconstruct(const DevScene& S, const Hit& h, f3 d, SurfaceHit& s) {
    const int ti = h.tri;
    const float4 A = S.isect[3 * ti];
    const float4 S0 = S.shade[4 * ti], S1 = S.shade[4 * ti + 1], S2 = S.shade[4 * ti + 2], S3 = S.shade[4 * ti + 3];
    const float4 E1 = make_float4(S0.x - A.x, S0.y - A.y, S0.z - A.z, 0.0f);
    const float4 E2 = make_float4(S1.x - A.x, S1.y - A.y, S1.z - A.z, 0.0f);
    const int mi = __float_as_int(S3.w);
    const float4 M0 = S.mats[kMatStride * mi], M1 = S.mats[kMatStride * mi + 1];
    f3 wo_w = normalize(-d);
    f3 v0 = mk(A.x, A.y, A.z), v1 = mk(S0.x, S0.y, S0.z), v2 = mk(S1.x, S1.y, S1.z);
    f3 n0 = mk(S0.w, S1.w, S2.x), n1 = mk(S2.y, S2.z, S2.w), n2 = mk(S3.x, S3.y, S3.z);
    f3 Ng = cross(mk(E1.x, E1.y, E1.z), mk(E2.x, E2.y, E2.z));
    const float u = h.u, v = h.v;
    float w = 1.0f - u - v;
    f3 Ns = mk(w * n0.x + u * n1.x + v * n2.x, w * n0.y + u * n1.y + v * n2.y, w * n0.z + u * n1.z + v * n2.z);
    if (M1.y != kNormalNone) {
        if (TEX && M1.y == kNormalObject) {
            const float4 R0 = S.mats[kMatStride * mi + 3], R1 = S.mats[kMatStride * mi + 4],
                         R2 = S.mats[kMatStride * mi + 5];
            Ns = mk(mat_row_dir(R0, Ns), mat_row_dir(R1, Ns), mat_row_dir(R2, Ns));
        }
        Ns = normalize(Ns);
    }
    if (dot(wo_w, Ng) < 0.0f) Ng = -Ng;
    Ng = normalize(Ng);
    if (dot(Ng, Ns) < 0.0f) Ns = -Ns;
    Ns = normalize(Ns);
    if (h.back) {
        Ns = Ns * -1.0f;
        Ng = Ng * -1.0f;
    }
    s.pos = mk(w * v0.x + u * v1.x + v * v2.x, w * v0.y + u * v1.y + v * v2.y, w * v0.z + u * v1.z + v * v2.z);
    s.ng = Ng;
    s.albedo = mk(M0.x, M0.y, M0.z);
    s.metallic = M0.w;
    s.roughness = M1.x;
    if (TEX) {
        const float4 M2 = S.mats[kMatStride * mi + 2];
        if (M2.y != 0.0f) apply_textures(S, ti, u, v, M1, M2, s.albedo, s.metallic, s.roughness, Ns);
    }
    f3 c1 = cross(Ns, mk(0.0f, 0.0f, 1.0f));
    f3 c2 = cross(Ns, mk(0.0f, 1.0f, 0.0f));
    f3 T = (length(c1) > length(c2)) ? c1 : c2;
    T = normalize(T);
    s.fr.t = T;
    s.fr.b = cross(T, Ns);
    s.fr.n = Ns;
    s.wo = to_local(s.fr, wo_w);
}

struct PathState {
    f3 o, d, beta, radiance;
    uint32_t seed;
    int bounce;
    bool end;
};

__device__ __forceinline__ void path_start(PathState& p, f3 o, f3 d, uint32_t seed) {
    p.o = o;
    p.d = d;
    p.beta = mk(1.0f, 1.0f, 1.0f);
    p.radiance = mk(0.0f, 0.0f, 0.0f);
    p.seed = seed;
    p.bounce = 0;
    p.end = false;
}

__device__ __forceinline__ void debug_record(const DevLaunch& L, int bounce, int prim, const SurfaceHit& sf, f3 beta,
                                             f3 radiance) {
    if (bounce < 1 || bounce > kDebugMaxBounces) return;
    float* r = L.debug + (size_t)(bounce - 1) * kDebugRecordFloats;
    const float v[kDebugRecordFloats] = {__int_as_float(bounce), __int_as_float(prim),
                                         sf.pos.x, sf.pos.y, sf.pos.z, sf.albedo.x, sf.albedo.y, sf.albedo.z,
                                         sf.fr.n.x, sf.fr.n.y, sf.fr.n.z, sf.ng.x, sf.ng.y, sf.ng.z,
                                         sf.roughness, sf.metallic, beta.x, beta.y, beta.z,
                                         radiance.x, radiance.y, radiance.z};
    for (int k = 0; k < kDebugRecordFloats; ++k) r[k] = v[k];
}

__device__ __forceinline__ bool path_alive(const DevLaunch& L, const PathState& p) {
    return !p.end && p.bounce < L.max_bounces && length(p.beta) > 0.00001f;
}

template <int MODE, bool STATS, int DEPTH, bool TEX>
__device__ __forceinline__ void path_segment(const DevScene& S, const DevLaunch& L, PathState& p, int* stk,
                                             int stride, TravStats& ts, bool debug_path) {
    Hit h;
    bool hit = traverse<false, STATS, DEPTH, TEX>(S, p.o, p.d, 0.0f, 100.0f, h, stk, stride, ts);
    if (!hit) {
        p.beta = mk(0, 0, 0);
        p.bounce = 100;
        return;
    }
    p.bounce++;
    if (p.bounce > L.max_bounces) {
        p.end = true;
        return;
    }
    SurfaceHit sf;
    reconstruct<TEX>(S, h, p.d, sf);
    if (debug_path) debug_record(L, p.bounce, __float_as_int(S.isect[3 * h.tri].w), sf, p.beta, p.radiance);
    const bool conductor = rnd(p.seed) < sf.metallic;
    float P = 0.0f;
    int li = 0;
    if (L.n_lights == 1) {
        P = 1.0f;
    } else if (L.n_lights > 1) {
        float r = rnd(p.seed);
        li = (int)(r * (float)L.n_lights);
        if (li >= L.n_lights) li = L.n_lights - 1;
        P = 1.0f / (float)L.n_lights;
    }
    if (P > 0.0f) {
        const DevLight lt = L.lights[li];
        f3 lpos = mk(lt.px, lt.py, lt.pz);
        f3 ldir = lpos - sf.pos;
// ... 36 lines not shown
```

### optixpathtracer_amd/csrc/pt_internal.h

```cpp
#pragma once
#include <hip/hip_runtime.h>

#include <algorithm>
#include <vector>

#include "pt_device.h"

namespace pt {

struct BuildInput {
    const float4* tri_orig;
    const float4* nrm_orig;
    const float4* uv_orig;
    int n;
    float cmin[3], cmax[3];
    int builder;
    const float4* tri_host;
};
constexpr int kBuilderPLOC = 0;
constexpr int kBuilderLBVH = 1;
constexpr int kBuilderSAH = 2;
constexpr int kBuilderSAHGPU = 3;

void sah_binary_tree(const float4* tri, int n, std::vector<uint32_t>& order, std::vector<int2>& child,
                     std::vector<int2>& range, std::vector<float4>& box);
hipError_t sah_build_gpu(const float4* tri, int n, uint32_t* order, int2* child, int2* range, float4* box,
                         hipStream_t stream);
#ifndef PT_SAH_REINSERT
#define PT_SAH_REINSERT 0
#endif
double sah_reinsert(std::vector<uint32_t>& order, std::vector<int2>& child, std::vector<int2>& range,
                    std::vector<float4>& box, const float4* tri, int rounds);

struct BuildOutput {
    BNode4* nodes;
    float4* isect;
    float4* shade;
    float4* tuv;
    int n_nodes;
    int depth;
    std::vector<int> level_base;
};

#ifndef PT_SAH_CTRI
#define PT_SAH_CTRI 0.5f
#endif
constexpr float kSahCNode = 1.0f;
constexpr float kSahCTri = PT_SAH_CTRI;

hipError_t lbvh_build(const BuildInput& in, BuildOutput& out, hipStream_t stream, float* ms);

struct WFState {
    float4* ray_o[2] = {nullptr, nullptr};
    float4* ray_d[2] = {nullptr, nullptr};
    float4* hit = nullptr;
    float4* beta = nullptr;
    float4* beta_q = nullptr;
    float4* L = nullptr;
    float4* sh_o = nullptr;
    float4* sh_d = nullptr;
    float4* sh_c = nullptr;
    int* aux = nullptr;
    int* vis = nullptr;
    int* nq = nullptr;
    int* sq = nullptr;
    int* count = nullptr;
    int paths = 0;
    int max_bounces = 0;
    const unsigned* cancel_host = nullptr;
    unsigned* cancel_seen = nullptr;
    unsigned cancel_epoch = 0;
    const unsigned* hold_release = nullptr;
};
size_t wavefront_bytes(int paths, int max_bounces);
hipError_t accum_f64_to_f32(const double* sum64, float* sum32, size_t n, hipStream_t stream);
hipError_t wavefront_alloc(WFState& W, int paths, int max_bounces);
void wavefront_free(WFState& W);
hipError_t launch_wavefront_frame(int mode, bool stats, const DevScene& S, const DevLaunch& L, const WFState& W,
                                  uint32_t frame, int nf, bool primary_dedup, int cus, hipStream_t stream,
                                  const hipEvent_t* trace_events,
                                  int* n_timed = nullptr, hipEvent_t accum_wait = nullptr,
                                  hipEvent_t accum_done = nullptr, const hipEvent_t* shade_events = nullptr,
                                  int* n_shade_timed = nullptr, bool wide_trace = false);

hipError_t launch_render(int kernel, int mode, bool stats, const DevScene& S, const DevLaunch& L,
                         hipStream_t stream);
hipError_t launch_trace(const DevScene& S, const float* d_rays, int n, int* d_prim, float* d_thit, float* d_u,
                        float* d_v, int* d_back, int any_hit, hipStream_t stream);

bool lit_subdivide(const float4* isect, int ntri, std::vector<uint32_t>& words, uint32_t* cells, float* diagonal);
hipError_t lit_build(const DevScene& S, const uint32_t* tri_words, uint32_t cells, uint32_t words,
                     const DevLight* lights, int n_lights, uint32_t* bits, float diag, hipStream_t stream);
hipError_t occ_build(const DevScene& S, const uint32_t* tri_words, uint32_t cells, uint32_t words,
                     const DevLight* lights, int n_lights, const uint32_t* bits, int* occ, hipStream_t stream);

struct RefitMesh {
    float m[16];
    int dirty;
    int normal_mode;
    int pad[2];
};
hipError_t refit_rebake(const RefitMesh* meshes, const float4* overts, const float4* onorms, const int4* tidx, int n,
                        float4* isect, float4* shade, hipStream_t stream);
hipError_t refit_levels(BNode4* nodes, const float4* isect, const std::vector<int>& level_base, hipStream_t stream);
int sah_partial_blocks(int n_nodes);
hipError_t sah_partial_launch(const BNode4* nodes, int n_nodes, double* partial, hipStream_t stream);

hipError_t display_fill(float* p, size_t n, float v, hipStream_t stream);
hipError_t display_blend(float* fb, const float* frame, size_t n, float w, bool continuous, hipStream_t stream);

struct AovBuffers {
    float *albedo, *normal, *gnormal, *position, *depth, *rough_metal;
    int* prim;
    float4 *guide_n, *guide_p, *guide_a, *guide_b;
    unsigned long long* hits;
};
hipError_t gbuffer_render(const DevScene& S, const DevLaunch& L, const AovBuffers& B, hipStream_t stream);
struct AtrousParams {
    const float4* cin;
    float4* cout;
    float* out;
    const float4 *gn, *gp, *ga;
    int w, h, step;
    float inv_c, inv_n, inv_p, floor;
    int demodulate;
};
constexpr int kAtrousLdsMaxStep = 16;
constexpr int kAtrousLdsDefaultStep = 16;
hipError_t atrous_pack(const float* in, float scale, bool demodulate, float floor, const float4* gn, const float4* ga,
                       float4* c, size_t n, hipStream_t stream);
hipError_t atrous_iteration(const AtrousParams& A, bool last, int lds_max_step, hipStream_t stream);

struct TemporalParams {
    const float4* c;
    const float4 *gn, *gp;
    const float4 *pgn, *pgp;
    const float4 *hc, *hm;
    float4 *tc, *tm;
    unsigned long long* count;
    int w, h, history;
    float prev_view[16], prev_proj[16];
    float alpha, alpha_moments, max_history, normal_cos, plane_distance;
    const float4 *gb, *snap;
    float4* pp;
    int ntri;
};
hipError_t temporal_blend(const TemporalParams& T, bool motion, hipStream_t stream);
hipError_t temporal_snapshot(const float4* isect, const float4* shade, int ntri, float4* snap, hipStream_t stream);
hipError_t temporal_motion_screen(const float4* pp, const float4* gn, const float* prev_view, const float* prev_proj,
                                  int history, int w, int h, float* out, hipStream_t stream);
hipError_t temporal_variance(const float4* gn, const float4* gp, const float4* tm, float4* tc, int w, int h, float inv_n,
                             float inv_p, float variance_history, hipStream_t stream);
hipError_t temporal_luminance_scale(const float4* cin, const float4* gn, float* den, int w, int h, float sigma_luminance,
                                    hipStream_t stream);
hipError_t temporal_atrous_iteration(const AtrousParams& A, const float* den, float4* hist, bool last, int lds_max_step,
                                     hipStream_t stream);

}
```

### optixpathtracer_amd/csrc/pt_lit.hip

```cpp
#include "pt_internal.h"
#include "pt_lit.h"

namespace pt {

bool lit_subdivide(const float4* isect, int ntri, std::vector<uint32_t>& words, uint32_t* cells, float* diagonal) {
    words.clear();
    *cells = 0;
    *diagonal = 0.0f;
    if (ntri <= 0) return false;
    float lo[3] = {INFINITY, INFINITY, INFINITY}, hi[3] = {-INFINITY, -INFINITY, -INFINITY};
    for (int t = 0; t < ntri; ++t) {
        const float4 A = isect[3 * t], E1 = isect[3 * t + 1], E2 = isect[3 * t + 2];
        const float v[3][3] = {{A.x, A.y, A.z}, {A.x + E1.x, A.y + E1.y, A.z + E1.z}, {A.x + E2.x, A.y + E2.y, A.z + E2.z}};
        for (int k = 0; k < 3; ++k)
            for (int a = 0; a < 3; ++a) {
                if (!(fabsf(v[k][a]) <= kLitMaxCoord)) return false;
                lo[a] = std::min(lo[a], v[k][a]);
                hi[a] = std::max(hi[a], v[k][a]);
            }
    }
    const double dx = (double)hi[0] - lo[0], dy = (double)hi[1] - lo[1], dz = (double)hi[2] - lo[2];
    const float diag = (float)std::sqrt(dx * dx + dy * dy + dz * dz);
    if (!(diag > 0.0f)) return false;
    const float target = kLitCellFraction * diag;
    words.resize((size_t)ntri);
    uint64_t n = 0;
    for (int t = 0; t < ntri; ++t) {
        const float4 E1 = isect[3 * t + 1], E2 = isect[3 * t + 2];
        const double a[3] = {E1.x, E1.y, E1.z}, b[3] = {E2.x, E2.y, E2.z}, o[3] = {0.0, 0.0, 0.0};
        LitPlane p;
        int k = kLitNoCells;
        if (lit_plane_through(o, a, b, p)) {
            const double l1 = std::sqrt(a[0] * a[0] + a[1] * a[1] + a[2] * a[2]);
            const double l2 = std::sqrt(b[0] * b[0] + b[1] * b[1] + b[2] * b[2]);
            const double c[3] = {b[0] - a[0], b[1] - a[1], b[2] - a[2]};
            const double l3 = std::sqrt(c[0] * c[0] + c[1] * c[1] + c[2] * c[2]);
            k = lit_level_for((float)std::max(l1, std::max(l2, l3)), target);
        }
        if (n > kLitMaxCells) return false;
        words[(size_t)t] = lit_word(k, (uint32_t)n);
        n += lit_cells(k);
    }
    if (n == 0 || n > kLitMaxCells) return false;
    *cells = (uint32_t)n;
    *diagonal = diag;
    return true;
}

namespace {

constexpr int kLitBlock = 64;
constexpr int kLitStack = 72;

__global__ __launch_bounds__(kLitBlock) void k_lit_build(DevScene S, const uint32_t* __restrict__ tri_words,
                                                        uint32_t cells, uint32_t words, const DevLight* __restrict__ lights,
                                                        int n_lights, uint32_t* __restrict__ bits, float diag) {
    __shared__ int lds_stack[kLitStack * kLitBlock];
    int* const stack = lds_stack + threadIdx.x;
    const uint64_t id = (uint64_t)blockIdx.x * kLitBlock + threadIdx.x;
    if (id >= (uint64_t)cells * (uint64_t)n_lights) return;
    const int li = (int)(id / cells);
    const uint32_t cell = (uint32_t)(id - (uint64_t)li * cells);
    int a = 0, b = S.ntri - 1;
    while (a < b) {
        const int m = (a + b + 1) >> 1;
        if (lit_first(tri_words[m]) <= cell) a = m; else b = m - 1;
    }
    const int t = a;
    const uint32_t w = tri_words[t];
    const int k = lit_level(w);
    if (k == kLitNoCells || cell - lit_first(w) >= lit_cells(k)) return;
    const float4 A = S.isect[3 * t], E1 = S.isect[3 * t + 1], E2 = S.isect[3 * t + 2];
    const float v0[3] = {A.x, A.y, A.z}, e1[3] = {E1.x, E1.y, E1.z}, e2[3] = {E2.x, E2.y, E2.z};
    const DevLight lt = lights[li];
    const float lp[3] = {lt.px, lt.py, lt.pz};
    if (!(fabsf(lp[0]) <= kLitMaxCoord && fabsf(lp[1]) <= kLitMaxCoord && fabsf(lp[2]) <= kLitMaxCoord)) return;
    LitPyramid P;
    const float margin = lit_margin_cell(diag, lit_cell_reach(v0, e1, e2, k, cell - lit_first(w), lp));
    if (!lit_pyramid(v0, e1, e2, k, cell - lit_first(w), lp, kLitDelta, margin, P)) return;
    int sp = 0;
    stack[kLitBlock * sp++] = 0;
    while (sp > 0) {
        const int c = stack[kLitBlock * --sp];
        if (c >= 0) {
            const BNode4 nd = S.nodes[c];
            const float lox[4] = {nd.lox.x, nd.lox.y, nd.lox.z, nd.lox.w}, hix[4] = {nd.hix.x, nd.hix.y, nd.hix.z, nd.hix.w};
            const float loy[4] = {nd.loy.x, nd.loy.y, nd.loy.z, nd.loy.w}, hiy[4] = {nd.hiy.x, nd.hiy.y, nd.hiy.z, nd.hiy.w};
            const float loz[4] = {nd.loz.x, nd.loz.y, nd.loz.z, nd.loz.w}, hiz[4] = {nd.hiz.x, nd.hiz.y, nd.hiz.z, nd.hiz.w};
            const int ch[4] = {nd.child.x, nd.child.y, nd.child.z, nd.child.w};
            for (int q = 0; q < 4; ++q) {
                if (ch[q] == kEmptyChild) continue;
                const double lo[3] = {lox[q], loy[q], loz[q]}, hi[3] = {hix[q], hiy[q], hiz[q]};
                if (lit_box_outside(P, lo, hi)) continue;
                if (sp >= kLitStack) return;
                stack[kLitBlock * sp++] = ch[q];
            }
        } else {
            const int first = leaf_first(c), cnt = leaf_count(c);
            for (int q = 0; q < cnt; ++q) {
                const int u = first + q;
                const float4 UA = S.isect[3 * u], U1 = S.isect[3 * u + 1], U2 = S.isect[3 * u + 2];
                const double pa[3] = {UA.x, UA.y, UA.z};
                const double pb[3] = {(double)UA.x + U1.x, (double)UA.y + U1.y, (double)UA.z + U1.z};
                const double pc[3] = {(double)UA.x + U2.x, (double)UA.y + U2.y, (double)UA.z + U2.z};
                if (!lit_tri_outside(P, pa, pb, pc)) return;
            }
        }
    }
    atomicOr(&bits[(size_t)li * words + (cell >> 5)], 1u << (cell & 31));
}

constexpr int kOccStack = 2 * kSpillDepth + 2;
static_assert(kOccStack / 2 > kSpillDepth && kOccStack - 3 > 72, "k_occ_build: the spill must stay unused");

__global__ __launch_bounds__(kLitBlock) void k_occ_build(DevScene S, const uint32_t* __restrict__ tri_words,
                                                        uint32_t cells, uint32_t words, const DevLight* __restrict__ lights,
                                                        int n_lights, const uint32_t* __restrict__ bits,
                                                        int* __restrict__ occ) {
    __shared__ int lds_stack[kOccStack * kLitBlock];
    __shared__ int lds_spill[1];
    const uint64_t id = (uint64_t)blockIdx.x * kLitBlock + threadIdx.x;
    if (id >= (uint64_t)cells * (uint64_t)n_lights) return;
    const int li = (int)(id / cells);
    const uint32_t cell = (uint32_t)(id - (uint64_t)li * cells);
    int cand = -1;
    do {
        if ((bits[(size_t)li * words + (cell >> 5)] >> (cell & 31)) & 1u) break;
        int a = 0, b = S.ntri - 1;
        while (a < b) {
            const int m = (a + b + 1) >> 1;
            if (lit_first(tri_words[m]) <= cell) a = m; else b = m - 1;
        }
        const int t = a;
        const uint32_t w = tri_words[t];
        const int k = lit_level(w);
        if (k == kLitNoCells || cell - lit_first(w) >= lit_cells(k)) break;
        const DevLight lt = lights[li];
        if (!(fabsf(lt.px) <= kLitMaxCoord && fabsf(lt.py) <= kLitMaxCoord && fabsf(lt.pz) <= kLitMaxCoord)) break;
        const float4 A = S.isect[3 * t], E1 = S.isect[3 * t + 1], E2 = S.isect[3 * t + 2];
        int cu[3], cv[3];
        lit_cell_corners(k, cell - lit_first(w), cu, cv);
        const float s = 1.0f / (3.0f * (float)(1 << k));
        const float u = (float)(cu[0] + cu[1] + cu[2]) * s, v = (float)(cv[0] + cv[1] + cv[2]) * s;
        const f3 e1 = mk(E1.x, E1.y, E1.z), e2 = mk(E2.x, E2.y, E2.z);
        const f3 p = mk(A.x, A.y, A.z) + u * e1 + v * e2;
        const f3 n = cross(e1, e2);
        const float nl = length(n);
        if (!(nl > 0.0f)) break;
        f3 ng = n / nl;
        const f3 ldir = mk(lt.px, lt.py, lt.pz) - p;
        float h = dot(ldir, ng);
        if (h < 0.0f) {
            ng = -ng;
            h = -h;
        }
        if (!(h > kLitDelta)) break;
        TravState st;
        TravStats ts;
        trav_init(st, p + 1e-3f * ng, normalize(ldir), 0.0f, length(ldir));
        while (!trav_step<kRayClosest, false, kOccStack, false>(S, st, lds_stack + threadIdx.x, kLitBlock, lds_spill, ts)) {
        }
        if (st.h.tri >= 0 && st.h.tri < S.ntri && __float_as_int(S.isect[3 * st.h.tri + 2].w) == 0) cand = st.h.tri;
    } while (false);
    occ[id] = cand;
}

}

hipError_t occ_build(const DevScene& S, const uint32_t* tri_words, uint32_t cells, uint32_t words,
                     const DevLight* lights, int n_lights, const uint32_t* bits, int* occ, hipStream_t stream) {
    if (n_lights <= 0 || cells == 0) return hipSuccess;
    const uint64_t n = (uint64_t)cells * (uint64_t)n_lights;
    hipLaunchKernelGGL(k_occ_build, dim3((unsigned)((n + kLitBlock - 1) / kLitBlock)), dim3(kLitBlock), 0, stream, S,
                       tri_words, cells, words, lights, n_lights, bits, occ);
    return hipGetLastError();
}

hipError_t lit_build(const DevScene& S, const uint32_t* tri_words, uint32_t cells, uint32_t words,
                     const DevLight* lights, int n_lights, uint32_t* bits, float diag, hipStream_t stream) {
    hipError_t e = hipMemsetAsync(bits, 0, sizeof(uint32_t) * (size_t)words * (size_t)n_lights, stream);
    if (e != hipSuccess || n_lights <= 0) return e;
    const uint64_t n = (uint64_t)cells * (uint64_t)n_lights;
    hipLaunchKernelGGL(k_lit_build, dim3((unsigned)((n + kLitBlock - 1) / kLitBlock)), dim3(kLitBlock), 0, stream, S,
                       tri_words, cells, words, lights, n_lights, bits, diag);
    return hipGetLastError();
}

}
```

### optixpathtracer_amd/csrc/pt_renderer.h

```cpp
#pragma once
#include <hip/hip_runtime.h>
#include <rccl/rccl.h>

#include <algorithm>
#include <cmath>
#include <cstdio>
#include <cstdlib>
#include <cstring>
#include <string>
#include <vector>

#include "../../include/ptamd.h"
#include "pt_internal.h"
#include "pt_lit.h"
#include "pt_resource.h"

namespace pt {

extern thread_local std::string g_last_error;
int fail(int code, const std::string& msg);
int hip_fail(hipError_t e, const char* where);

#define PT_HIP(call, where)                              \
    do {                                                 \
// ... 160 lines not shown
        pt::DevBuf<float4> d_onorms;
        pt::DevBuf<int4> d_tidx;
        pt::DevBuf<pt::RefitMesh> d_rmesh;
        pt::DevBuf<double> d_sah_part;
        pt::Event ev[2];
        uint32_t version = 0;
        uint64_t commits = 0, refits = 0, rebuilds = 0;
        double commit_ms = 0.0;
        double sah_cost = 0.0, sah_cost_built = 0.0;
        double sah_root_built = 0.0;
    } geom;

    struct Ahead {
        int max_frames = 64;
        double budget_ms = 50.0;
        double frame_ms_est = 0.0;
        int oom_cap = 1 << 30;
        pt::RingSlot ring[2];
        int ring_k = 1, ring_last = 0;
        bool spec_pending = false;
        uint64_t rendered = 0, served = 0;
        pt::PinnedWord cancel;
        pt::DevBuf<unsigned> d_cancel_seen;
        unsigned cancel_epoch = 0;
        uint64_t cancelled = 0;
        bool debug_hold = false;
        pt::PinnedWord hold;
        uint64_t held = 0;
        void reset_counts() { rendered = served = cancelled = held = 0; }
    } ahead;

    struct Timing {
        pt::EventPool ev;
        uint64_t launches = 0;
        bool kernel_timing = false;
        pt::EventPool tev;
        std::vector<hipEvent_t> tev_frame;
        double trace_ms = 0.0;
        uint64_t trace_launches = 0;
        pt::EventPool pev;
        double pair_ms = 0.0;
        uint64_t pair_launches = 0;
        pt::EventPool sev;
        std::vector<hipEvent_t> sev_frame;
        double shade_ms = 0.0;
        uint64_t shade_launches = 0;
        bool pending = false;
        uint64_t samples = 0;
        double last_ms = 0.0, total_ms = 0.0;
        uint64_t calls = 0;
        double bvh_ms = 0.0;
        void reset_counts() {
            samples = calls = launches = trace_launches = pair_launches = shade_launches = 0;
            last_ms = total_ms = trace_ms = pair_ms = shade_ms = 0.0;
        }
    } timing;

    struct Multi {
        std::vector<pt_renderer*> peers;
        std::vector<ncclComm_t> comms;
        pt::DevBuf<float> d_part;
        pt::DevBuf<double> d_part64;
    } multi;

    struct Lit {
        int mode = -1;
        pt::DevBuf<uint32_t> d_tri;
        pt::DevBuf<uint32_t> d_bits;
        uint32_t cells = 0, words = 0;
        uint32_t words_cap = 0;
        float diag = 0.0f;
        uint32_t version = 1;
        bool active = false;
        bool launch_call = false;
        pt::BuiltTable built;
    } lit;
    struct Occ {
        int mode = -1;
        pt::DevBuf<int> d_tab;
        bool alloc_failed = false;
        bool active = false;
        pt::BuiltTable built;
    } occ;

    struct Aov {
        pt::DevBuf<float> d_albedo, d_normal, d_gnormal, d_position, d_depth, d_rough_metal;
        pt::DevBuf<int> d_prim;
        pt::DevBuf<float4> d_gn, d_gp, d_ga, d_gb;
        pt::DevBuf<unsigned long long> d_hits;
        pt::DevBuf<float4> d_c[2];
        pt::DevBuf<float> d_out, d_in;
        pt::ViewKey key;
        bool rendered = false;
        uint64_t renders = 0;
        int iterations = 0;
        pt::Event ev_g[2], ev_f[2];
        bool g_timed = false, f_timed = false;
        void release() {
            for (pt::DevBuf<float>* b :
                 {&d_albedo, &d_normal, &d_gnormal, &d_position, &d_depth, &d_rough_metal, &d_out, &d_in})
                b->reset();
            for (pt::DevBuf<float4>* b : {&d_gn, &d_gp, &d_ga, &d_gb, &d_c[0], &d_c[1]}) b->reset();
            d_prim.reset();
            rendered = g_timed = f_timed = false;
        }
    } aov;

    struct Temporal {
        pt::DevBuf<float4> d_pgn, d_pgp;
        pt::DevBuf<float4> d_hc;
        pt::DevBuf<float4> d_m[2];
        pt::DevBuf<float4> d_tc;
        pt::DevBuf<float> d_den;
        pt::DevBuf<unsigned long long> d_count;
        int cur = 0;
        bool valid = false;
        float inv_view[16] = {}, inv_proj[16] = {};
        uint64_t calls = 0;
        pt::Event ev[4];
        bool timed = false;
        pt::DevBuf<float4> d_snap, d_pp;
        uint32_t snap_version = 0;
        bool snap_have = false, snap_prev = false;
        bool mv_last = false, mv_used = false;
        bool had_history = false;
        float prev_view[16] = {}, prev_proj[16] = {};
        pt::Event ev_s[2];
        bool snap_timed = false;
        void release() {
            for (pt::DevBuf<float4>* b : {&d_pgn, &d_pgp, &d_hc, &d_m[0], &d_m[1], &d_tc, &d_snap, &d_pp}) b->reset();
            d_den.reset();
            valid = timed = snap_have = snap_prev = mv_last = mv_used = had_history = snap_timed = false;
        }
    } temporal;

    pt_renderer() = default;
    ~pt_renderer();
    pt::DevScene scene() const {
        pt::DevScene S;
        S.nodes = d_nodes;
        S.isect = d_isect;
        S.shade = d_shade;
        S.mats = d_mats;
        S.tuv = d_tuv;
        S.texels = d_texels;
        S.texinfo = d_texinfo;
        S.ntri = ntri;
        S.n_nodes = bvh_nodes;
        S.lds_nodes = nullptr;
        S.n_lds = 0;
        return S;
    }
    float* accum() const { return user_accum ? user_accum : d_accum.get(); }
};

namespace pt {

int ingest_scene(const pt_scene* scene, GeomHost& G, std::vector<float4>& mats, std::vector<int4>& texinfo,
                 size_t* ntexel, bool* any_tex, std::string* err);
void bake_scene(const GeomHost& G, std::vector<float4>& tri, std::vector<float4>& nrm, float cmin[3], float cmax[3]);

int upload_scene(pt_renderer* r, const pt_scene* scene, const std::vector<int4>& texinfo, size_t ntexel);
int build_scene(pt_renderer* r, bool any_tex);
int commit_geometry(pt_renderer* r, int how);

size_t queue_bytes_held(const pt_renderer* r);
size_t queue_budget_bytes(const pt_renderer* r);
int launch_frames(pt_renderer* r, float* accum, uint32_t first, uint32_t n, double* accum64 = nullptr,
                  size_t frame_stride = 0, bool speculative = false);
int render_frames_multi(pt_renderer* r, uint32_t first, uint32_t n);

ViewKey view_key(const pt_renderer* r);
void ring_free(pt_renderer* r);
void cancel_look_ahead(pt_renderer* r, bool force = false);
int render_frame_image(pt_renderer* r, const float** img, hipEvent_t* ready = nullptr, bool look_ahead = false,
                       hipEvent_t* part_ready = nullptr, size_t* part_floats = nullptr);

bool lit_wanted(const pt_renderer* r);
bool occ_wanted(const pt_renderer* r);
bool table_current(const pt_renderer* r, const BuiltTable& t);
int lit_prepare(pt_renderer* r);
int lit_resubdivide(pt_renderer* r);
int lit_table_download(pt_renderer* r, pt_lit_table_info* info, uint32_t* tri_words, int64_t tri_bytes, uint32_t* bits,
                       int64_t bits_bytes);
int occ_table_download(pt_renderer* r, int64_t* entries_out, int32_t* entries, int64_t bytes);
int occ_table_upload(pt_renderer* r, const int32_t* entries, int64_t bytes);

int collect_pending(pt_renderer* r);

template <class T>
size_t versioned_bytes(const T* s) {
    return s->struct_size < sizeof(uint32_t) ? 0 : std::min<size_t>(s->struct_size, sizeof(T));
}
template <class T>
size_t versioned_merge(T& into, const T* user) {
    const size_t n = user ? versioned_bytes(user) : sizeof(T);
    if (user && n) std::memcpy(&into, user, n);
    return n;
}
template <class T>
size_t versioned_write(T* user, T d) {
    const size_t n = versioned_bytes(user);
    d.struct_size = user->struct_size;
    std::memcpy(user, &d, n);
    return n;
}

int gbuffer_prepare(pt_renderer* r);
struct DenoiseCall {
    const char* fn;
    pt_renderer* r;
    int32_t source;
    const float* host_in;
    pt_denoise_options o;
    size_t n;
    const float* src;
    int lds;
    AtrousParams P;

    int err(int code, const char* what) const;
    int check_source() const;
    int merge(const pt_denoise_options* opt);
    int begin(bool reads_sigma_color);
    int finish(float* host_out) const;
};

void mat4_inverse(const float* m, float* out);

}
```

### optixpathtracer_amd/csrc/pt_wavefront.hip

```cpp
#include <type_traits>
#include <unordered_map>

#include "pt_internal.h"
#include "pt_lit.h"

namespace pt {

namespace {

constexpr int kBlockWF = 256;
#ifndef PT_TRACE_BLOCK
#define PT_TRACE_BLOCK 256
#endif
constexpr int kBlockTrace = PT_TRACE_BLOCK;
constexpr int kStack = PT_WF_STACK;
#ifndef PT_LDS_NODES
#define PT_LDS_NODES 49
#endif
constexpr int kLdsNodes = PT_LDS_NODES;
#ifndef PT_TRACE_BLOCK_WIDE
#define PT_TRACE_BLOCK_WIDE 768
#endif
#ifndef PT_LDS_NODES_WIDE
#define PT_LDS_NODES_WIDE 150
#endif
constexpr int kBlockTraceWide = PT_TRACE_BLOCK_WIDE;
template <int BLK>
constexpr int lds_nodes_of() { return BLK == kBlockTrace ? kLdsNodes : PT_LDS_NODES_WIDE; }
#ifndef PT_WF_WAVES
#define PT_WF_WAVES 6
#endif
#ifndef PT_WF_WAVES_TEX
#define PT_WF_WAVES_TEX 6
#endif
constexpr int wf_waves(bool tex) { return tex ? PT_WF_WAVES_TEX : PT_WF_WAVES; }
constexpr int kMissTri = -1;

__device__ __forceinline__ int lane_id() { return threadIdx.x & 63; }

__device__ __forceinline__ bool wf_cancel_poll(const WFState& W, bool relay) {
    if (relay) {
        const unsigned h = __hip_atomic_load(W.cancel_host, __ATOMIC_RELAXED, __HIP_MEMORY_SCOPE_SYSTEM);
        __hip_atomic_fetch_max(W.cancel_seen, h, __ATOMIC_RELAXED, __HIP_MEMORY_SCOPE_AGENT);
    }
    const unsigned v = __hip_atomic_load(W.cancel_seen, __ATOMIC_RELAXED, __HIP_MEMORY_SCOPE_AGENT);
    return __builtin_amdgcn_readfirstlane(v) > W.cancel_epoch;
}
__device__ __forceinline__ bool wf_cancelled(const WFState& W) {
    if (!W.cancel_seen) return false;
    return wf_cancel_poll(W, (blockIdx.x & 63) == 0 && threadIdx.x == 0);
}

__global__ void k_hold(WFState W) {
    if (threadIdx.x != 0 || blockIdx.x != 0) return;
    const unsigned long long t0 = wall_clock64();
    for (int it = 0; it < (1 << 22); ++it) {
        const unsigned h = __hip_atomic_load(W.cancel_host, __ATOMIC_RELAXED, __HIP_MEMORY_SCOPE_SYSTEM);
        if (h > W.cancel_epoch) {
            __hip_atomic_fetch_max(W.cancel_seen, h, __ATOMIC_RELAXED, __HIP_MEMORY_SCOPE_AGENT);
            return;
        }
        if (__hip_atomic_load(W.hold_release, __ATOMIC_RELAXED, __HIP_MEMORY_SCOPE_SYSTEM) != 0u) return;
        if (wall_clock64() - t0 > 1000000000ull) return;
        __builtin_amdgcn_s_sleep(64);
    }
}

__device__ __forceinline__ float4 hit_record(const Hit& h, int path) {
    const float x = __int_as_float(path);
    return h.tri >= 0 ? make_float4(x, h.u, h.v, __int_as_float(h.tri | (h.back ? (int)0x80000000 : 0)))
                      : make_float4(x, 0.0f, 0.0f, __int_as_float(kMissTri));
}

__device__ __forceinline__ unsigned long long wave_sum_u64(unsigned long long v) {
#pragma unroll
    for (int o = 32; o >= 1; o >>= 1) v += __shfl_xor(v, o, 64);
    return v;
}

template <bool STATS>
__device__ __forceinline__ void flush_trav_stats(unsigned long long* counters, const TravStats& ts) {
    if (!STATS || !counters) return;
    const unsigned long long a = wave_sum_u64(ts.nodes), c = wave_sum_u64(ts.tris), d = wave_sum_u64(ts.rays);
    const unsigned long long e = wave_sum_u64(ts.overflow), r = wave_sum_u64(ts.retrace);
    const unsigned long long l = wave_sum_u64(ts.lds_nodes), u = wave_sum_u64(ts.unocc);
    if (lane_id() == 0) {
        atomicAdd(&counters[kCtrNodes], a);
        atomicAdd(&counters[kCtrTriTests], c);
        atomicAdd(&counters[kCtrRays], d);
        atomicAdd(&counters[kCtrStackOverflows], e);
        atomicAdd(&counters[kCtrRetraces], r);
        atomicAdd(&counters[kCtrWaveSteps], (unsigned long long)ts.steps);
        atomicAdd(&counters[kCtrWaveActive], (unsigned long long)ts.active);
        atomicAdd(&counters[kCtrWaveNodeSteps], (unsigned long long)ts.node_steps);
        atomicAdd(&counters[kCtrWaveTriSteps], (unsigned long long)ts.tri_steps);
        atomicAdd(&counters[kCtrWaveRefills], (unsigned long long)ts.refills);
        atomicAdd(&counters[kCtrLdsNodes], l);
        atomicAdd(&counters[kCtrNeeUnoccluded], u);
        for (int k = 0; k < 6; ++k) atomicAdd(&counters[kCtrCoh0 + k], (unsigned long long)ts.coh[k]);
        atomicAdd(&counters[kCtrCohLanes], (unsigned long long)ts.coh_lanes);
    }
}

constexpr int kShadeBuckets = 3;
#ifndef PT_NEE_CLASSES
#define PT_NEE_CLASSES 2
#endif
#ifndef PT_NEE_DARK
#define PT_NEE_DARK 0.5f
#endif
#ifndef PT_NEE_MID
#define PT_NEE_MID 0.7f
#endif
constexpr int kNeeClasses = PT_NEE_CLASSES;
constexpr int kNeeBuckets = 2 + 2 * kNeeClasses;
constexpr int kNeeRegions = kNeeBuckets / 2;
constexpr int kNeeCross = 1;
static_assert(kNeeBuckets <= 8, "a shadow ray's item code holds the NEE bucket in bits 28-30");
constexpr int kCnt = 5 + kNeeBuckets + kShadeBuckets;
constexpr int kCntStride = 32;
enum { kQueue = 0, kShadowQ = 1, kNee0 = 2, kSmp0 = 2 + kNeeBuckets, kPool = 2 + kNeeBuckets + kShadeBuckets, kPoolExt, kPoolSh };
__device__ __forceinline__ int* cnt(const WFState& W, int b, int k) { return W.count + (kCnt * b + k) * kCntStride; }
__device__ __forceinline__ size_t nee_index(const WFState& W, int q, int slot) {
    const size_t r = (size_t)(q >> 1) * W.paths;
    return (q & 1) ? r + W.paths - 1 - slot : r + slot;
}
__device__ __forceinline__ int nee_layered_bucket(int bk, f3 albedo) {
    const float m = fmaxf(fmaxf(albedo.x, albedo.y), albedo.z);
    int cls = 0;
    if (kNeeClasses >= 3 && m < PT_NEE_MID) cls = 1;
    if (kNeeClasses >= 2 && m < PT_NEE_DARK) cls = kNeeClasses - 1;
    return 2 + 2 * cls + (bk - 1);
}
__device__ __forceinline__ size_t smp_index(const WFState& W, int q, int slot) {
    return (size_t)q * W.paths + slot;
}
__device__ __forceinline__ float4* queue_beta(const WFState& W, int b) { return (b & 1) ? W.beta_q : W.beta; }
inline size_t count_bytes(int max_bounces) { return sizeof(int) * kCntStride * kCnt * (size_t)(max_bounces + 2); }

constexpr int kBlockSh = 1024;
constexpr int kWavesSh = kBlockSh / 64;
#ifndef PT_SHA_BLOCK
#define PT_SHA_BLOCK 1024
#endif
constexpr int kBlockShA = PT_SHA_BLOCK, kWavesShA = kBlockShA / 64;
#ifndef PT_SHF_WAVES
#define PT_SHF_WAVES 8
#endif
#ifndef PT_SHF_WAVES_OTHER
#define PT_SHF_WAVES_OTHER 1
#endif
constexpr int shf_waves(int mode) { return (mode == 1 || mode == 3)  ? PT_SHF_WAVES : PT_SHF_WAVES_OTHER; }
#ifndef PT_SHF_BLOCK_DIELECTRIC
#define PT_SHF_BLOCK_DIELECTRIC 256
#endif
#ifndef PT_SHF_BLOCK_CONDUCTOR
#define PT_SHF_BLOCK_CONDUCTOR 256
#endif
#ifndef PT_SHF_BLOCK_LAMBERT
#define PT_SHF_BLOCK_LAMBERT 1024
#endif
constexpr int shf_block(int mode) {
    return mode == 3 ? PT_SHF_BLOCK_DIELECTRIC : mode == 2 ? PT_SHF_BLOCK_CONDUCTOR : PT_SHF_BLOCK_LAMBERT;
}
#ifndef PT_SHB_BLOCK
#define PT_SHB_BLOCK 256
#endif
#ifndef PT_SHB_WAVES
#define PT_SHB_WAVES 4
#endif
#ifndef PT_SMP_WAVES
#define PT_SMP_WAVES 5
#endif
constexpr int kBlockShB = PT_SHB_BLOCK;

template <int WAVES>
__device__ __forceinline__ int block_append(int* counter, bool pred, int* lds) {
    const unsigned long long m = __ballot(pred ? 1 : 0);
    const int prefix = __builtin_amdgcn_mbcnt_hi((uint32_t)(m >> 32), __builtin_amdgcn_mbcnt_lo((uint32_t)m, 0u));
    const int wave = threadIdx.x >> 6;
    if (lane_id() == 0) lds[wave] = __popcll(m);
// ... 282 lines not shown
        S, n_trace, ts, W,
        [&](int ri, TravState& st) {
            const float4 a = ro[ri], c = rd[ri];
            trav_init(st, mk(a.x, a.y, a.z), mk(c.x, c.y, c.z), 0.0f, 100.0f);
            st.path = __float_as_int(a.w);
        },
        [&](int ri, const TravState& st) {
            for (int k = 0; k < copies; ++k) {
                float4* rec = W.hit + ri + (size_t)k * n_trace;
                *rec = hit_record(st.h, st.path + k * n_trace);
            }
        }, cnt(W, b, kPoolExt));
    if (blockIdx.x == 0 && threadIdx.x == 0 && counters) {
        atomicAdd(&counters[kCtrSegments], (unsigned long long)n);
        atomicAdd(&counters[kCtrTraceRays], (unsigned long long)n_trace);
        atomicAdd(&counters[kCtrTraceBytes], (32ull + 16ull * (unsigned long long)copies) * (unsigned long long)n_trace);
    }
    flush_trav_stats<STATS>(counters, ts);
}

__device__ __forceinline__ Hit decode_hit(float4 hv) {
    Hit h;
    const int code = __float_as_int(hv.w);
    h.t = hv.x;
    h.u = hv.y;
    h.v = hv.z;
    h.back = code != kMissTri && (code & (int)0x80000000);
    h.tri = code == kMissTri ? -1 : (code & 0x7fffffff);
    return h;
}

__device__ __forceinline__ float pick_light(const DevLaunch& L, uint32_t& seed, int& li) {
    li = 0;
    if (L.n_lights == 1) return 1.0f;
    if (L.n_lights <= 0) return 0.0f;
    float r = rnd(seed);
    li = (int)(r * (float)L.n_lights);
    if (li >= L.n_lights) li = L.n_lights - 1;
    return 1.0f / (float)L.n_lights;
}

__device__ __forceinline__ bool continue_path(const SurfaceHit& sf, const BSample& bs, f3& beta, f3& o, f3& d,
                                              int next_bounce, int max_bounces) {
    float ac = abs_dot(bs.dir, mk(0.0f, 0.0f, 1.0f));
    beta = beta * mk(bs.color.x * ac / bs.pdf, bs.color.y * ac / bs.pdf, bs.color.z * ac / bs.pdf);
    f3 off = 1e-3f * sf.ng;
    if (dot(bs.dir, mk(0.0f, 0.0f, 1.0f)) < 0.0f) off = -off;
    o = sf.pos + off;
    d = normalize(to_world(sf.fr, bs.dir));
    return next_bounce < max_bounces && length(beta) > 0.00001f;
}

__device__ __forceinline__ int lit_cell(const DevLaunch& L, const Hit& h) {
    const uint32_t w = L.lit_tri[h.tri];
    const int k = lit_level(w);
    return k == kLitNoCells ? -1 : (int)(lit_first(w) + lit_cell_index(k, h.u, h.v));
}
__device__ __forceinline__ bool lit_bit(const DevLaunch& L, int li, int cell) {
    return (L.lit_bits[(size_t)li * L.lit_words + ((uint32_t)cell >> 5)] >> (cell & 31)) & 1u;
}
__device__ __forceinline__ void lit_count_wave(bool answered, int* lds) {
    const unsigned long long m = __ballot(answered ? 1 : 0);
    if (lane_id() == 0) lds[threadIdx.x >> 6] = __popcll(m);
}
template <int WAVES, int SLOT = kCtrLitAnswers>
__device__ __forceinline__ void lit_count_block(const DevLaunch& L, const int* lds) {
    if (threadIdx.x != 0 || !L.counters) return;
    int tot = 0;
    for (int w = 0; w < WAVES; ++w) tot += lds[w];
    if (tot > 0) atomicAdd(&L.counters[SLOT], (unsigned long long)tot);
}
template <bool TEX>
__device__ __forceinline__ bool occ_answers(const DevScene& S, int t, f3 o, f3 d, float tmax) {
    if (t < 0) return false;
    const float4 A = S.isect[3 * t], E1 = S.isect[3 * t + 1], E2 = S.isect[3 * t + 2];
    float th, uh, vh;
    bool bk;
    if (!tri_test(A, E1, E2, o, d, 0.0f, tmax, th, uh, vh, bk)) return false;
    if (TEX && __float_as_int(E2.w) != 0) return false;
    const f3 inv = safe_inv(d);
    return tri_accept(A, E1, E2, inv, mk(o.x * inv.x, o.y * inv.y, o.z * inv.z), th);
}

__device__ __forceinline__ int vis0_index(const DevLaunch& L, int path, int li) {
    const int P1 = L.width * L.height;
    return li * P1 + path % P1;
}

template <bool TEX>
__global__ __launch_bounds__(kBlockWF) void k_shadow0_setup(DevScene S, DevLaunch L, WFState W) {
    const int P1 = L.width * L.height;
    const int nl = L.n_lights;
    const int n = P1 * nl;
    if (wf_cancelled(W)) return;
    for (int k = blockIdx.x * blockDim.x + threadIdx.x; k < n; k += gridDim.x * blockDim.x) {
        const int li = k / P1, p = k - li * P1;
        const Hit h = decode_hit(W.hit[p]);
        float4 so = make_float4(0.0f, 0.0f, 0.0f, __int_as_float(k)), sd = make_float4(0.0f, 0.0f, 1.0f, 0.0f);
        if (h.tri >= 0) {
            const float4 c = W.ray_d[0][p];
            SurfaceHit sf;
            reconstruct<TEX>(S, h, mk(c.x, c.y, c.z), sf);
            const DevLight lt = L.lights[li];
            const f3 ldir = mk(lt.px, lt.py, lt.pz) - sf.pos;
            const f3 o = sf.pos + 1e-3f * sf.ng;
            const f3 d = normalize(ldir);
            so = make_float4(o.x, o.y, o.z, __int_as_float(k));
            sd = make_float4(d.x, d.y, d.z, length(ldir));
        }
        W.sh_o[k] = so;
        W.sh_d[k] = sd;
    }
    if (blockIdx.x == 0 && threadIdx.x == 0) *cnt(W, 0, kShadowQ) = n;
}

template <int MODE, bool TEX, bool SHADE0>
__global__ __launch_bounds__(shf_block(MODE), shf_waves(MODE)) void k_shade_fused(DevScene S, DevLaunch L, WFState W, int b, int vis0) {
    constexpr bool shade0 = SHADE0;
    constexpr bool kBetaQ = MODE == kModeLambert;
    constexpr bool kShareOrigin = MODE == kModeLambert;
    constexpr int kBlock = shf_block(MODE), kWaves = kBlock / 64;
    const int n = *cnt(W, b, kQueue);
    const float4* rd = W.ray_d[b & 1];
    float4* no = W.ray_o[(b + 1) & 1];
    float4* nd = W.ray_d[(b + 1) & 1];
    __shared__ int lds_sh[kWaves + 1], lds_q[kWaves + 1];
    __shared__ int lds_lit[kWaves];
    constexpr bool kOcc = MODE == kModeLambert;
    __shared__ int lds_occ[kOcc ? kWaves : 1];
    const bool lit = !vis0 && L.lit_tri;
    const bool occ = kOcc && lit && L.occ_tab;
    if (blockIdx.x == 0 && threadIdx.x == 0 && L.counters) atomicAdd(&L.counters[kCtrShadeItems], (unsigned long long)n);
    if ((int)(blockIdx.x * kBlock) >= n) return;
    {
        const int i = (int)(blockIdx.x * kBlock + threadIdx.x);
        const bool valid = i < n && !wf_cancelled(W);
        bool emit_shadow = false, emit_next = false, lit_answer = false;
        f3 so, sdir, contrib, o, d, beta;
        uint32_t seed = 0;
        float stmax = 0.0f;
        int path = 0;
        int occ_t = -1;
        const int P1 = L.width * L.height;
        float4 l0 = make_float4(0.0f, 0.0f, 0.0f, 0.0f);
        if (valid) {
            const float4 hv = ldqs(W.hit + i);
            const float4 c_q = shade0 ? make_float4(0.0f, 0.0f, 0.0f, 0.0f) : ldqs(rd + i);
            const float4 bv_q = (!shade0 && kBetaQ) ? ldqs(queue_beta(W, b) + i) : make_float4(0.0f, 0.0f, 0.0f, 0.0f);
            path = __float_as_int(hv.x);
            const Hit h = decode_hit(hv);
            if (h.tri >= 0) {
                const int lit_c = lit ? lit_cell(L, h) : -1;
                const float4 c = shade0 ? ldqs(rd + path % P1) : c_q;
                d = mk(c.x, c.y, c.z);
                SurfaceHit sf;
                reconstruct<TEX>(S, h, d, sf);
                if (shade0) {
                    seed = tea16((uint32_t)(path % P1 + L.width * L.row0), L.frame_base + (uint32_t)(path / P1));
                    beta = mk(1.0f, 1.0f, 1.0f);
                } else {
                    float4 bv = kBetaQ ? bv_q : ldqs(W.beta + path);
                    seed = __float_as_uint(bv.w);
                    beta = mk(bv.x, bv.y, bv.z);
                }
                if (path == debug_path_id(L)) {
                    const float4 l = shade0 ? l0 : W.L[path];
                    debug_record(L, b + 1, __float_as_int(S.isect[3 * h.tri].w), sf, beta, mk(l.x, l.y, l.z));
                }
                const bool conductor = rnd(seed) < sf.metallic;
                int li;
                const float P = pick_light(L, seed, li);
                if (P > 0.0f) {
                    const DevLight lt = L.lights[li];
                    f3 lpos = mk(lt.px, lt.py, lt.pz);
                    f3 ldir = lpos - sf.pos;
                    f3 ldn = normalize(ldir);
                    f3 lds = to_local(sf.fr, ldn);
                    f3 f = bsdf_f<MODE>(seed, sf.albedo, sf.roughness, conductor, sf.wo, lds);
                    f3 spectrum = f * abs_dot(lds, mk(0.0f, 0.0f, 1.0f));
                    if (!is_zero(spectrum)) {
                        f3 dd = sf.pos - lpos;
                        float d2 = dd.x * dd.x + dd.y * dd.y + dd.z * dd.z;
                        f3 Li = mk(lt.cr, lt.cg, lt.cb) / d2;
                        contrib = ((beta * spectrum) * Li) / (P * 1.0f);
                        lit_answer = lit_c >= 0 && dot(ldir, sf.ng) > kLitDelta && lit_bit(L, li, lit_c);
                        if (vis0 || lit_answer) {
                            if (lit_answer || W.vis[vis0_index(L, path, li)]) {
                                const float4 l = shade0 ? l0 : W.L[path];
                                l0 = make_float4(l.x + contrib.x, l.y + contrib.y, l.z + contrib.z, 0.0f);
                                if (!shade0) W.L[path] = l0;
                            }
                        } else {
                            so = sf.pos + 1e-3f * sf.ng;
                            sdir = normalize(ldir);
                            stmax = length(ldir);
                            emit_shadow = true;
                            if (kOcc && occ && lit_c >= 0 && dot(ldir, sf.ng) > kLitDelta)
                                occ_t = L.occ_tab[li * (int)L.lit_cells + lit_c];
                        }
                    }
                }
                BSample bs;
                if (b + 1 < L.max_bounces &&
                    bsdf_sample<MODE>(seed, sf.albedo, sf.roughness, conductor, sf.wo, bs)) {
                    emit_next = continue_path(sf, bs, beta, o, d, b + 1, L.max_bounces);
                    if (!kBetaQ) stqs(W.beta + path, make_float4(beta.x, beta.y, beta.z, __uint_as_float(seed)));
                }
            }
        }
        if (shade0 && valid) W.L[path] = l0;
        if (lit) lit_count_wave(lit_answer, lds_lit);
        const int qi = block_append<kWaves>(cnt(W, b + 1, kQueue), emit_next, lds_q);
        if (lit) lit_count_block<kWaves>(L, lds_lit);
        if (emit_next) {
            stqs(no + qi, make_float4(o.x, o.y, o.z, __int_as_float(path)));
            stqs(nd + qi, make_float4(d.x, d.y, d.z, 0.0f));
            if (kBetaQ) stqs(queue_beta(W, b + 1) + qi, make_float4(beta.x, beta.y, beta.z, __uint_as_float(seed)));
        }
        if constexpr (kOcc) {
            if (occ) {
                bool answered = false;
                if (occ_t >= 0) answered = occ_answers<TEX>(S, occ_t, (kShareOrigin && emit_next) ? o : so, sdir, stmax);
                if (answered) emit_shadow = false;
                lit_count_wave(answered, lds_occ);
            }
        }
        const int si = block_append<kWaves>(cnt(W, b, kShadowQ), emit_shadow, lds_sh);
        if constexpr (kOcc) {
            if (occ) lit_count_block<kWaves, kCtrOccAnswers>(L, lds_occ);
        }
        if (emit_shadow) {
            const bool share = kShareOrigin && emit_next;
            if (!share) stqs(W.sh_o + si, make_float4(so.x, so.y, so.z, __int_as_float(path)));
            stqs(W.sh_d + si, make_float4(sdir.x, sdir.y, sdir.z, stmax));
            stqs(W.sh_c + si, make_float4(contrib.x, contrib.y, contrib.z, __int_as_float(share ? qi : -1)));
        }
    }
}

template <int MODE, bool TEX>
__global__ __launch_bounds__(shf_block(MODE), 1) void k_shade0_pixel(DevScene S, DevLaunch L, WFState W, int nf) {
    constexpr bool kBetaQ = MODE == kModeLambert;
    constexpr int kBlock = shf_block(MODE), kWaves = kBlock / 64;
    const int P1 = L.width * L.height;
    __shared__ int lds_q[kWaves + 1];
    if (blockIdx.x == 0 && threadIdx.x == 0 && L.counters)
        atomicAdd(&L.counters[kCtrShadeItems], (unsigned long long)P1 * (unsigned long long)nf);
    if ((int)(blockIdx.x * kBlock) >= P1) return;
    const int p = (int)(blockIdx.x * kBlock + threadIdx.x);
    const bool valid = p < P1 && !wf_cancelled(W);
    int tri = -1;
    SurfaceHit sf;
    if (valid) {
        const float4 hv = W.hit[p];
        const Hit h = decode_hit(hv);
        tri = h.tri;
        if (tri >= 0) {
            const float4 c = W.ray_d[0][p];
            reconstruct<TEX>(S, h, mk(c.x, c.y, c.z), sf);
        }
    }
    const int dbg = debug_path_id(L);
    float4* no = W.ray_o[1];
    float4* nd = W.ray_d[1];
    for (int f = 0; f < nf; ++f) {
        const int path = f * P1 + p;
        bool emit_next = false;
        f3 o, d, beta = mk(1.0f, 1.0f, 1.0f);
        uint32_t seed = 0;
        float4 l0 = make_float4(0.0f, 0.0f, 0.0f, 0.0f);
        if (valid && tri >= 0) {
            seed = tea16((uint32_t)(p + L.width * L.row0), L.frame_base + (uint32_t)f);
            if (path == dbg) debug_record(L, 1, __float_as_int(S.isect[3 * tri].w), sf, beta, mk(0.0f, 0.0f, 0.0f));
            const bool conductor = rnd(seed) < sf.metallic;
            int li;
            const float P = pick_light(L, seed, li);
            if (P > 0.0f) {
                const DevLight lt = L.lights[li];
                f3 lpos = mk(lt.px, lt.py, lt.pz);
                f3 lds = to_local(sf.fr, normalize(lpos - sf.pos));
                f3 fv = bsdf_f<MODE>(seed, sf.albedo, sf.roughness, conductor, sf.wo, lds);
                f3 spectrum = fv * abs_dot(lds, mk(0.0f, 0.0f, 1.0f));
                if (!is_zero(spectrum) && W.vis[vis0_index(L, path, li)]) {
                    f3 dd = sf.pos - lpos;
                    float d2 = dd.x * dd.x + dd.y * dd.y + dd.z * dd.z;
                    f3 Li = mk(lt.cr, lt.cg, lt.cb) / d2;
                    f3 contrib = ((beta * spectrum) * Li) / (P * 1.0f);
                    l0 = make_float4(0.0f + contrib.x, 0.0f + contrib.y, 0.0f + contrib.z, 0.0f);
                }
            }
            BSample bs;
            if (1 < L.max_bounces && bsdf_sample<MODE>(seed, sf.albedo, sf.roughness, conductor, sf.wo, bs)) {
                emit_next = continue_path(sf, bs, beta, o, d, 1, L.max_bounces);
                if (!kBetaQ) stqs(W.beta + path, make_float4(beta.x, beta.y, beta.z, __uint_as_float(seed)));
            }
        }
        if (valid) stqs(W.L + path, l0);
        const int qi = block_append<kWaves>(cnt(W, 1, kQueue), emit_next, lds_q);
        if (emit_next) {
            stqs(no + qi, make_float4(o.x, o.y, o.z, __int_as_float(path)));
            stqs(nd + qi, make_float4(d.x, d.y, d.z, 0.0f));
            if (kBetaQ) stqs(queue_beta(W, 1) + qi, make_float4(beta.x, beta.y, beta.z, __uint_as_float(seed)));
        }
    }
}

template <bool STATS, bool TEX, int BLK = kBlockTrace>
__global__ __launch_bounds__(BLK, wf_waves(TEX)) void k_trace_pair(DevScene S, WFState W, int b,
                                                                      unsigned long long* counters) {
    const int n_ext = *cnt(W, b + 1, kQueue);
    const int n_sh = *cnt(W, b, kShadowQ);
    const float4* ro = W.ray_o[(b + 1) & 1];
    const float4* rd = W.ray_d[(b + 1) & 1];
    TravStats ts;
    auto fetch = [&](int i, TravState& st) {
        if (i < n_ext) {
            const float4 a = ldqs(ro + i), c = ldqs(rd + i);
            trav_init(st, mk(a.x, a.y, a.z), mk(c.x, c.y, c.z), 0.0f, 100.0f);
            st.path = __float_as_int(a.w);
        } else {
            const int j = i - n_ext;
            const float4 c = ldqs(W.sh_d + j), k = ldqs(W.sh_c + j);
            const int q = __float_as_int(k.w);
            const float4 a = ldqs(q >= 0 ? ro + q : W.sh_o + j);
            trav_init(st, mk(a.x, a.y, a.z), mk(c.x, c.y, c.z), 0.0f, c.w);
            st.any = true;
            st.h.orig = __float_as_int(a.w);
            st.h.t = k.x;
            st.h.u = k.y;
            st.h.v = k.z;
        }
    };
    struct NeeAdd {
        float4* p;
        float4 v;
        float x, y, z;
    };
    auto finish = [&](int i, const TravState& st) -> NeeAdd {
        NeeAdd a{nullptr, make_float4(0.0f, 0.0f, 0.0f, 0.0f), 0.0f, 0.0f, 0.0f};
        const Hit& h = st.h;
        if (i < n_ext) stqs(W.hit + i, hit_record(h, st.path));
        __builtin_amdgcn_sched_barrier(0);
        if (STATS && i >= n_ext && h.tri < 0) ts.unocc++;
        if (i >= n_ext && h.tri < 0) {
            a.p = W.L + h.orig;
            a.v = *a.p;
            a.x = h.t;
            a.y = h.u;
            a.z = h.v;
        }
        return a;
    };
    auto commit = [&](const NeeAdd& a) {
        if (a.p) *a.p = make_float4(a.v.x + a.x, a.v.y + a.y, a.v.z + a.z, 0.0f);
    };
    int first, end;
    const int n_all = n_ext + n_sh;
    RayPool pool;
    if (PT_TRACE_POOL > 0 && pool_pays(n_all)) {
        pool.ctr = cnt(W, b, kPool);
        pool.end = n_all;
        pool.begin = n_all - (int)((long long)n_all * PT_TRACE_POOL / 100);
    } else {
        pool.begin = pool.end = n_all;
    }
    wave_slice(pool.begin, first, end);
    trace_queue<kRayMixed, STATS, TEX, BLK>(S, first, end, ts, W, fetch, finish, commit, pool);
    if (blockIdx.x == 0 && threadIdx.x == 0 && counters) {
        atomicAdd(&counters[kCtrSegments], (unsigned long long)n_ext);
        atomicAdd(&counters[kCtrShadowRays], (unsigned long long)n_sh);
        atomicAdd(&counters[kCtrTraceRays], (unsigned long long)(n_ext + n_sh));
        atomicAdd(&counters[kCtrTraceBytes], 48ull * (unsigned long long)(n_ext + n_sh));
        atomicAdd(&counters[kCtrPairRays], (unsigned long long)(n_ext + n_sh));
        atomicAdd(&counters[kCtrPairBytes], 48ull * (unsigned long long)(n_ext + n_sh));
        atomicAdd(&counters[kCtrPairShadowRays], (unsigned long long)n_sh);
    }
    flush_trav_stats<STATS>(counters, ts);
}

template <int MODE, bool TEX>
__global__ __launch_bounds__(kBlockShA) void k_shade_a(DevScene S, DevLaunch L, WFState W, int b, int vis0) {
    const int n = *cnt(W, b, kQueue);
    const float4* rd = W.ray_d[b & 1];
    __shared__ int lds_sh[kWavesShA + 1];
    __shared__ int lds_nee[kNeeBuckets * (kWavesShA + 1)], lds_smp[kShadeBuckets * (kWavesShA + 1)];
    __shared__ int lds_lit[kWavesShA], lds_occ[kWavesShA];
    const bool lit = !vis0 && L.lit_tri;
    const bool occ = lit && L.occ_tab;
    if ((int)(blockIdx.x * kBlockShA) >= n) return;
    const int i = (int)(blockIdx.x * kBlockShA + threadIdx.x);
    bool emit = false, lit_answer = false, occ_answer = false;
    int nee_bucket = -1, smp_bucket = -1, code = 0;
    f3 so, sdir;
    float stmax = 0.0f;
    if (i < n && !wf_cancelled(W)) {
        const float4 hv = W.hit[i];
        const float4 c = rd[i];
        const int path = __float_as_int(hv.x);
        const Hit h = decode_hit(hv);
        if (h.tri >= 0) {
            const int lit_c = lit ? lit_cell(L, h) : -1;
            SurfaceHit sf;
            reconstruct<TEX>(S, h, mk(c.x, c.y, c.z), sf);
            float4 bv = W.beta[path];
            uint32_t seed = __float_as_uint(bv.w);
            if (path == debug_path_id(L)) {
                const float4 l = W.L[path];
                debug_record(L, b + 1, __float_as_int(S.isect[3 * h.tri].w), sf, mk(bv.x, bv.y, bv.z),
                             mk(l.x, l.y, l.z));
            }
            const bool conductor = rnd(seed) < sf.metallic;
            int li;
            const float P = pick_light(L, seed, li);
            W.beta[path] = make_float4(bv.x, bv.y, bv.z, __uint_as_float(seed));
            W.aux[path] = (li << 1) | (conductor ? 1 : 0);
            const int bk = shade_bucket<MODE>(conductor, sf.roughness);
            if (b + 1 < L.max_bounces) smp_bucket = bk;
            if (P > 0.0f) {
                const DevLight lt = L.lights[li];
                f3 ldir = mk(lt.px, lt.py, lt.pz) - sf.pos;
                const f3 ln = normalize(ldir);
                int nb = 0;
                if (MODE == kModeLayered || !conductor)
                    nb = !same_hemisphere(sf.wo, to_local(sf.fr, ln)) ? kNeeCross : nee_layered_bucket(bk, sf.albedo);
                lit_answer = lit_c >= 0 && dot(ldir, sf.ng) > kLitDelta && lit_bit(L, li, lit_c);
                if (vis0 || lit_answer) {
                    if (lit_answer || W.vis[vis0_index(L, path, li)]) nee_bucket = nb;
                } else {
                    so = sf.pos + 1e-3f * sf.ng;
                    sdir = ln;
                    stmax = length(ldir);
                    code = i | (nb << kItemBits);
                    emit = true;
                    if (occ && lit_c >= 0 && dot(ldir, sf.ng) > kLitDelta)
                        occ_answer = occ_answers<TEX>(S, L.occ_tab[li * (int)L.lit_cells + lit_c], so, sdir, stmax);
                    if (occ_answer) emit = false;
                }
            }
        }
    }
    if (lit) lit_count_wave(lit_answer, lds_lit);
    if (occ) lit_count_wave(occ_answer, lds_occ);
    const int si = block_append<kWavesShA>(cnt(W, b, kShadowQ), emit, lds_sh);
    if (lit) lit_count_block<kWavesShA>(L, lds_lit);
    if (occ) lit_count_block<kWavesShA, kCtrOccAnswers>(L, lds_occ);
    if (emit) {
        W.sh_o[si] = make_float4(so.x, so.y, so.z, __int_as_float(code));
        W.sh_d[si] = make_float4(sdir.x, sdir.y, sdir.z, stmax);
    }
    const int ni = block_append_k<kWavesShA, kNeeBuckets>(cnt(W, b, kNee0), nee_bucket, lds_nee);
// ... 355 lines not shown
    al((void**)&W.ray_d[1], P * sizeof(float4));
    al((void**)&W.hit, P * sizeof(float4));
    al((void**)&W.beta, P * sizeof(float4));
    al((void**)&W.beta_q, P * sizeof(float4));
    al((void**)&W.L, P * sizeof(float4));
    al((void**)&W.sh_o, P * sizeof(float4));
    al((void**)&W.sh_d, P * sizeof(float4));
    al((void**)&W.sh_c, P * sizeof(float4));
    al((void**)&W.aux, P * sizeof(int));
    al((void**)&W.vis, P * sizeof(int));
    al((void**)&W.nq, P * kNeeRegions * sizeof(int));
    al((void**)&W.sq, P * kShadeBuckets * sizeof(int));
    al((void**)&W.count, count_bytes(max_bounces));
    if (e != hipSuccess) {
        wavefront_free(W);
        (void)hipGetLastError();
        return e;
    }
    W.paths = paths;
    W.max_bounces = max_bounces;
    return e;
}

void wavefront_free(WFState& W) {
    void* ps[] = {W.ray_o[0], W.ray_o[1], W.ray_d[0], W.ray_d[1], W.hit, W.beta, W.beta_q, W.L, W.sh_o, W.sh_d, W.sh_c,
                  W.aux, W.vis, W.nq, W.sq, W.count};
    for (void* p : ps)
        if (p) (void)hipFree(p);
    W = WFState{};
}

hipError_t launch_wavefront_frame(int mode, bool stats, const DevScene& S, const DevLaunch& L, const WFState& W,
                                  uint32_t frame, int nf, bool primary_dedup, int cus, hipStream_t stream,
                                  const hipEvent_t* trace_events, int* n_timed, hipEvent_t accum_wait,
                                  hipEvent_t accum_done, const hipEvent_t* shade_events, int* n_shade_timed,
                                  bool wide_trace) {
    const int P = L.width * L.height * nf;
    const int maxb = L.max_bounces;
    hipError_t e = hipSuccess;
    if (W.cancel_seen && W.hold_release) {
        hipLaunchKernelGGL(k_hold, dim3(1), dim3(64), 0, stream, W);
        if ((e = hipGetLastError()) != hipSuccess) return e;
    }
    e = hipMemsetAsync(W.count, 0, count_bytes(maxb), stream);
    if (e != hipSuccess) return e;
    const bool lean = fused_mode(mode) && primary_dedup && nf > 1 && maxb > 0;
    hipLaunchKernelGGL(k_camera, item_grid(lean ? L.width * L.height : P, kBlockWF), dim3(kBlockWF), 0, stream, W, L,
                       frame, nf, lean ? 1 : 0);
    if ((e = hipGetLastError()) != hipSuccess) return e;
    const bool fused = fused_mode(mode);
    const bool tex = S.texinfo != nullptr;
    int timed = 0;
    int stimed = 0;
    auto shade_timed = [&](auto launch) -> hipError_t {
        hipError_t r;
        if (shade_events && (r = hipEventRecord(shade_events[2 * stimed], stream)) != hipSuccess) return r;
        if ((r = launch()) != hipSuccess) return r;
        if (shade_events && (r = hipEventRecord(shade_events[2 * stimed + 1], stream)) != hipSuccess) return r;
        ++stimed;
        return hipSuccess;
    };
    auto trace_timed = [&](auto launch) -> hipError_t {
        hipError_t r;
        if (trace_events && (r = hipEventRecord(trace_events[2 * timed], stream)) != hipSuccess) return r;
        if ((r = launch()) != hipSuccess) return r;
        if (trace_events && (r = hipEventRecord(trace_events[2 * timed + 1], stream)) != hipSuccess) return r;
        ++timed;
        return hipSuccess;
    };
    auto trace_launch = [&](auto kernel, int block, auto... args) -> hipError_t {
        hipLaunchKernelGGL(kernel, occupancy_grid(kernel, cus, block), dim3(block), 0, stream, args...);
        return hipGetLastError();
    };
    auto extend = [&](int b, int dup, int copies) -> hipError_t {
        return trace_timed([&] {
            return trace_variant(tex, wide_trace, stats, [&](auto tx, auto st, auto blk) {
                return trace_launch(k_extend<st(), tx(), blk()>, blk(), S, W, b, dup, copies, L.counters);
            });
        });
    };
    auto pair = [&](int b) -> hipError_t {
        return trace_timed([&] {
            return trace_variant(tex, wide_trace, stats, [&](auto tx, auto st, auto blk) {
                return trace_launch(k_trace_pair<st(), tx(), blk()>, blk(), S, W, b, L.counters);
            });
        });
    };
    auto shadow_vis = [&](int b, int table) -> hipError_t {
        const hipError_t r = trace_variant(tex, wide_trace, false, [&](auto tx, auto, auto blk) {
            return trace_launch(k_shadow_vis<tx(), blk()>, blk(), S, W, b, table, L.counters);
        });
        if (r != hipSuccess) return r;
        if (!table) hipLaunchKernelGGL(k_nee_compact, item_grid(P, kBlockSh * kCompactPer), dim3(kBlockSh), 0, stream, W, b);
        return hipGetLastError();
    };
    const int P1 = L.width * L.height;
    const int vis0 = (primary_dedup && nf > 1 && L.n_lights >= 1 && L.n_lights <= nf) ? L.n_lights : 0;
    auto shadow0 = [&]() -> hipError_t {
        if (!vis0) return hipSuccess;
        hipError_t r = with_flag(tex, [&](auto tx) {
            hipLaunchKernelGGL(k_shadow0_setup<tx()>, item_grid(P1 * vis0, kBlockWF), dim3(kBlockWF), 0, stream, S, L, W);
            return hipGetLastError();
        });
        if (r != hipSuccess || (r = shadow_vis(0, 1)) != hipSuccess) return r;
        return hipMemsetAsync(W.count + kShadowQ * kCntStride, 0, sizeof(int), stream);
    };
    if (maxb <= 0) {
    } else if (fused) {
        const bool pixel0 = lean && vis0;
        if ((e = extend(0, primary_dedup ? nf : 1, pixel0 ? 1 : (primary_dedup ? nf : 1))) != hipSuccess) return e;
        if ((e = shadow0()) != hipSuccess) return e;
        for (int b = 0; b < maxb; ++b) {
            if (b == 0 && pixel0) {
                if ((e = shade_timed([&] { return launch_shade0_pixel(mode, S, L, W, nf, stream); })) != hipSuccess)
                    return e;
            } else if ((e = shade_timed([&] {
                            return launch_shade_mode(mode, true, S, L, W, b, P, stream, 0, b == 0 ? vis0 : 0,
                                                     b == 0 && lean);
                        })) != hipSuccess) {
                return e;
            }
            if ((e = pair(b)) != hipSuccess) return e;
        }
    } else {
        for (int b = 0; b < maxb; ++b) {
            const int dup = b == 0 && primary_dedup ? nf : 1;
            if ((e = extend(b, dup, dup)) != hipSuccess) return e;
            const int v0 = b == 0 ? vis0 : 0;
            if (v0 && (e = shadow0()) != hipSuccess) return e;
            if ((e = launch_shade_mode(mode, false, S, L, W, b, P, stream, 0, v0)) != hipSuccess) return e;
            if (!v0 && (e = shadow_vis(b, 0)) != hipSuccess) return e;
            if ((e = shade_timed([&] { return launch_shade_mode(mode, false, S, L, W, b, P, stream, 1, v0); })) !=
                hipSuccess)
                return e;
            if (b + 1 < maxb && (e = launch_shade_mode(mode, false, S, L, W, b, P, stream, 2, v0)) != hipSuccess)
                return e;
        }
    }
    if (accum_wait && (e = hipStreamWaitEvent(stream, accum_wait, 0)) != hipSuccess) return e;
    hipLaunchKernelGGL(k_accum, item_grid(L.width * L.height, kBlockWF), dim3(kBlockWF), 0, stream, W, L, nf);
    if (accum_done && (e = hipEventRecord(accum_done, stream)) != hipSuccess) return e;
    if (n_timed) *n_timed = timed;
    if (n_shade_timed) *n_shade_timed = stimed;
    return hipGetLastError();
}

}
```

### optixpathtracer_amd/renderer.py

```python
from __future__ import annotations

import ctypes as C
import dataclasses

import numpy as np

from . import capi
from .capi import check, fptr, load
from .scenes import Scene


def _f32(a, shape=None) -> np.ndarray:
    a = np.ascontiguousarray(a, dtype=np.float32)
    if shape is not None:
        a = a.reshape(shape)
    return a


class _SceneBinding:

    def __init__(self, scene: Scene):
        self.keep = []
        meshes = (capi.pt_mesh * max(1, len(scene.meshes)))()
        for i, m in enumerate(scene.meshes):
# ... 268 lines not shown
            src = srcs[source]
        else:
            host = _f32(source)
            if host.size != w * h * 3:
                raise capi.PTError("denoise_temporal: the source array must hold H * W * 3 floats", capi.PT_ERR_INVALID)
            src = capi.PT_DENOISE_SRC_HOST
        out = np.empty((h, w, 3), np.float32) if download else None
        check(self.lib.pt_denoise_temporal(self.h, src, fptr(host) if host is not None else None, float(scale),
                                           C.byref(t), C.byref(o), fptr(out) if download else None), "pt_denoise_temporal")
        return out

    def temporal_reset(self) -> None:
        check(self.lib.pt_temporal_reset(self.h), "pt_temporal_reset")

    def temporal_state(self, kind) -> np.ndarray:
        k = capi.TEMPORAL_KINDS[kind] if isinstance(kind, str) else int(kind)
        ch = int(self.lib.pt_temporal_channels(k))
        if ch < 0:
            raise capi.PTError(f"temporal_state: no such kind {kind!r}", capi.PT_ERR_INVALID)
        w, h = self.size
        out = np.empty((h, w) if ch == 1 else (h, w, ch), np.float32)
        check(self.lib.pt_temporal_download(self.h, k, out.ctypes.data, out.nbytes), "pt_temporal_download")
        return out

    def motion(self, kind) -> np.ndarray:
        k = capi.MOTION_KINDS[kind] if isinstance(kind, str) else int(kind)
        ch = int(self.lib.pt_motion_channels(k))
        if ch < 0:
            raise capi.PTError(f"motion: no such kind {kind!r}", capi.PT_ERR_INVALID)
        w, h = self.size
        out = np.empty((h, w, ch), np.float32)
        check(self.lib.pt_motion_download(self.h, k, out.ctypes.data, out.nbytes), "pt_motion_download")
        return out

    def temporal_info(self) -> dict:
        s = capi.pt_temporal_info()
        s.struct_size = C.sizeof(s)
        check(self.lib.pt_get_temporal_info(self.h, C.byref(s)), "pt_get_temporal_info")
        return {k: getattr(s, k) for k, _ in capi.pt_temporal_info._fields_ if k != "struct_size"}

    def accum_clear(self) -> None:
        check(self.lib.pt_accum_clear(self.h), "pt_accum_clear")

    def render_frames(self, first_frame_id: int, n_frames: int) -> None:
        check(self.lib.pt_render_frames(self.h, int(first_frame_id), int(n_frames)), "pt_render_frames")

    def set_primary_dedup(self, enable: bool) -> None:
        check(self.lib.pt_set_primary_dedup(self.h, 1 if enable else 0), "pt_set_primary_dedup")

    def set_wavefront_streams(self, streams: int) -> None:
        check(self.lib.pt_set_wavefront_streams(self.h, int(streams)), "pt_set_wavefront_streams")

    def set_band_split(self, enable: bool) -> None:
        check(self.lib.pt_set_band_split(self.h, 1 if enable else 0), "pt_set_band_split")

    def set_lit_table(self, enable: bool | None) -> None:
        check(self.lib.pt_set_lit_table(self.h, -1 if enable is None else (1 if enable else 0)), "pt_set_lit_table")

    def lit_table(self):
        info = capi.pt_lit_table_info()
        check(self.lib.pt_lit_table_download(self.h, C.byref(info), None, 0, None, 0), "pt_lit_table_download")
        d = {k: getattr(info, k) for k, _ in capi.pt_lit_table_info._fields_}
        if not info.active:
            return d, None, None
        tri = np.zeros(info.triangles, np.uint32)
        bits = np.zeros((info.lights, info.words_per_light), np.uint32)
        check(self.lib.pt_lit_table_download(self.h, C.byref(info), tri.ctypes.data, tri.nbytes, bits.ctypes.data,
                                             bits.nbytes), "pt_lit_table_download")
        return d, tri, bits

    def set_occluder_table(self, enable: bool | None) -> None:
        check(self.lib.pt_set_occluder_table(self.h, -1 if enable is None else (1 if enable else 0)),
              "pt_set_occluder_table")

    def occluder_table(self):
        n = C.c_int64(0)
        check(self.lib.pt_occluder_table_download(self.h, C.byref(n), None, 0), "pt_occluder_table_download")
        if n.value == 0:
            return None
        e = np.zeros(n.value, np.int32)
        check(self.lib.pt_occluder_table_download(self.h, C.byref(n), e.ctypes.data, e.nbytes), "pt_occluder_table_download")
        return e

    def upload_occluder_table(self, entries) -> None:
        e = np.ascontiguousarray(entries, np.int32)
        check(self.lib.pt_occluder_table_upload(self.h, e.ctypes.data, e.nbytes), "pt_occluder_table_upload")

    def render_accumulate(self, spp: int, first_frame_id: int = 1) -> np.ndarray:
        w, h = self.size
        out = np.empty((h, w, 3), np.float32)
        check(self.lib.pt_render_accumulate(self.h, int(spp), int(first_frame_id), fptr(out)),
              "pt_render_accumulate")
        return out

    def set_accum_device_buffer(self, ptr: int | None) -> None:
        check(self.lib.pt_set_accum_device_buffer(self.h, C.c_void_p(ptr) if ptr else None),
              "pt_set_accum_device_buffer")

    def accum(self, scale: float = 1.0) -> np.ndarray:
        w, h = self.size
        out = np.empty((h, w, 3), np.float32)
        check(self.lib.pt_accum_download(self.h, fptr(out), float(scale)), "pt_accum_download")
        return out

    def set_accum_fp64(self, enable: bool) -> None:
        check(self.lib.pt_set_accum_fp64(self.h, 1 if enable else 0), "pt_set_accum_fp64")

    def accum64(self) -> np.ndarray:
        w, h = self.size
        out = np.empty((h, w, 3), np.float64)
        check(self.lib.pt_accum_download64(self.h, out.ctypes.data_as(C.POINTER(C.c_double))), "pt_accum_download64")
        return out

    def synchronize(self) -> None:
        check(self.lib.pt_synchronize(self.h), "pt_synchronize")

    def stream(self) -> int:
        return int(self.lib.pt_stream(self.h) or 0)

    @property
    def frame_id(self) -> int:
        return int(self.lib.pt_frame_id(self.h))

    @frame_id.setter
    def frame_id(self, v: int) -> None:
        check(self.lib.pt_set_frame_id(self.h, int(v)), "pt_set_frame_id")

    def stats(self) -> dict:
        s = capi.pt_stats()
        check(self.lib.pt_get_stats(self.h, C.byref(s)), "pt_get_stats")
        return {k: getattr(s, k) for k, _ in capi.pt_stats._fields_}

    def stats_reset(self) -> None:
        check(self.lib.pt_stats_reset(self.h), "pt_stats_reset")

    def trace_rays(self, rays: np.ndarray, any_hit: bool = False):
        r = _f32(rays).reshape(-1, 8)
        n = len(r)
        prim = np.empty(n, np.int32)
        t, u, v = (np.empty(n, np.float32) for _ in range(3))
        back = np.empty(n, np.int32)
        check(self.lib.pt_trace_rays(self.h, fptr(r), n, prim.ctypes.data_as(C.POINTER(C.c_int32)), fptr(t),
                                     fptr(u), fptr(v), back.ctypes.data_as(C.POINTER(C.c_int32)),
                                     1 if any_hit else 0), "pt_trace_rays")
        return prim, t, u, v, back

    def set_debug_pixel(self, x: int, y: int, frame_id: int) -> None:
        check(self.lib.pt_set_debug_pixel(self.h, int(x), int(y), int(frame_id)), "pt_set_debug_pixel")

    def debug_path(self) -> list:
        recs = (capi.pt_debug_bounce * 64)()
        n = C.c_int32()
        check(self.lib.pt_get_debug_path(self.h, recs, 64, C.byref(n)), "pt_get_debug_path")
        out = []
        for k in range(n.value):
            r = recs[k]
            out.append({f: (list(getattr(r, f)) if isinstance(getattr(r, f), C.Array) else getattr(r, f))
                        for f, _ in capi.pt_debug_bounce._fields_})
        return out

    def devices(self) -> list:
        n = int(self.lib.pt_device_count(self.h))
        out = (C.c_int32 * max(1, n))()
        check(self.lib.pt_devices(self.h, out, n), "pt_devices")
        return [int(out[i]) for i in range(n)]

# ... 30 lines not shown
```

Before: 1776 Msamples/sec.

## Add per-triangle BVH skip table to prune subtrees on bounce rays

Builds a per-triangle, per-side table of BVH node indices that a bounce ray leaving that surface in the upward hemisphere cannot hit. The index is packed into the unused w component of the queued ray direction, and the pair trace kernel skips that node during traversal. The goal is fewer node and triangle tests for secondary rays in scenes like convex objects inside a box. It adds a GPU build pass, an extra table read per shade, and a new traversal template variant. The pruning is only correct if the precomputed table is conservative, which makes this a correctness risk.

```diff
diff --git a/include/ptamd.h b/include/ptamd.h
--- a/include/ptamd.h
+++ b/include/ptamd.h
@@ -127,6 +127,9 @@
     uint64_t occluder_table_candidates;
     double occluder_table_build_ms;
     uint64_t occluder_table_answers;
+    uint64_t skip_table_bytes;
+    double skip_table_build_ms;
+    uint64_t skip_table_rays;
     uint64_t geometry_commits;
     uint64_t geometry_refits;
     uint64_t geometry_rebuilds;
@@ -171,6 +174,8 @@
 int pt_set_occluder_table(pt_renderer* r, int32_t enable);
 int pt_occluder_table_download(pt_renderer* r, int64_t* entries_out, int32_t* entries, int64_t bytes);
 int pt_occluder_table_upload(pt_renderer* r, const int32_t* entries, int64_t bytes);
+int pt_set_skip_table(pt_renderer* r, int32_t enable);
+int pt_skip_table_download(pt_renderer* r, int64_t* words_out, uint32_t* words, int64_t bytes);
 
 typedef struct pt_launch_params {
     struct {
diff --git a/optixpathtracer_amd/capi.py b/optixpathtracer_amd/capi.py
--- a/optixpathtracer_amd/capi.py
+++ b/optixpathtracer_amd/capi.py
@@ -146,6 +146,9 @@
         ("occluder_table_candidates", C.c_uint64),
         ("occluder_table_build_ms", C.c_double),
         ("occluder_table_answers", C.c_uint64),
+        ("skip_table_bytes", C.c_uint64),
+        ("skip_table_build_ms", C.c_double),
+        ("skip_table_rays", C.c_uint64),
         ("geometry_commits", C.c_uint64),
         ("geometry_refits", C.c_uint64),
         ("geometry_rebuilds", C.c_uint64),
@@ -271,6 +274,8 @@
     "pt_set_occluder_table": (C.c_int, [_R, C.c_int32]),
     "pt_occluder_table_download": (C.c_int, [_R, C.POINTER(C.c_int64), C.c_void_p, C.c_int64]),
     "pt_occluder_table_upload": (C.c_int, [_R, C.c_void_p, C.c_int64]),
+    "pt_set_skip_table": (C.c_int, [_R, C.c_int32]),
+    "pt_skip_table_download": (C.c_int, [_R, C.POINTER(C.c_int64), C.c_void_p, C.c_int64]),
     "pt_render_accumulate": (C.c_int, [_R, C.c_uint32, C.c_uint32, _FP]),
     "pt_set_accum_device_buffer": (C.c_int, [_R, C.c_void_p]),
     "pt_accum_device_ptr": (C.c_void_p, [_R]),
diff --git a/optixpathtracer_amd/csrc/pt_capi.cpp b/optixpathtracer_amd/csrc/pt_capi.cpp
--- a/optixpathtracer_amd/csrc/pt_capi.cpp
+++ b/optixpathtracer_amd/csrc/pt_capi.cpp
@@ -850,6 +850,20 @@
     return PT_OK;
 }
 
+extern "C" int pt_set_skip_table(pt_renderer* r, int32_t enable) {
+    if (!r) return fail(PT_ERR_INVALID, "pt_set_skip_table: NULL");
+    const int mode = enable < 0 ? -1 : (enable > 0 ? 1 : 0);
+    r->skip.mode = mode;
+    for (pt_renderer* p : r->multi.peers) p->skip.mode = mode;
+    return PT_OK;
+}
+
+extern "C" int pt_skip_table_download(pt_renderer* r, int64_t* words_out, uint32_t* words, int64_t bytes) {
+    if (!r || !words_out) return fail(PT_ERR_INVALID, "pt_skip_table_download: NULL");
+    PT_HIP(hipSetDevice(r->device), "hipSetDevice");
+    return skip_table_download(r, words_out, words, bytes);
+}
+
 extern "C" int pt_set_band_split(pt_renderer* r, int32_t enable) {
     if (!r) return fail(PT_ERR_INVALID, "pt_set_band_split: NULL");
     int rc = collect_pending(r);
diff --git a/optixpathtracer_amd/csrc/pt_capi_launch.cpp b/optixpathtracer_amd/csrc/pt_capi_launch.cpp
--- a/optixpathtracer_amd/csrc/pt_capi_launch.cpp
+++ b/optixpathtracer_amd/csrc/pt_capi_launch.cpp
@@ -36,6 +36,7 @@
     L.lit_words = r->lit.words;
     L.occ_tab = r->lit.active && r->occ.active ? r->occ.d_tab.get() : nullptr;
     L.lit_cells = r->lit.cells;
+    L.skip_tab = r->skip.active ? r->skip.d_words.get() : nullptr;
     return L;
 }
 
@@ -212,6 +213,7 @@
     int dev_cus = 256;
     (void)hipDeviceGetAttribute(&dev_cus, hipDeviceAttributeMultiprocessorCount, r->device);
     if ((rc = lit_prepare(r)) != PT_OK) return rc;
+    if ((rc = skip_prepare(r)) != PT_OK) return rc;
     hipEvent_t a = nullptr, b = nullptr;
     if (dual) {
         rc = next_event_pair(r, &a, &b);
@@ -304,6 +306,7 @@
     r->timing.pending = true;
     r->band0_rows = 0;
     r->lit.active = false;
+    r->skip.active = false;
     int kernel = r->kernel;
     if (kernel == PT_KERNEL_AUTO) kernel = PT_KERNEL_WAVEFRONT;
     if (accum64 && kernel != PT_KERNEL_WAVEFRONT)
diff --git a/optixpathtracer_amd/csrc/pt_capi_scene.cpp b/optixpathtracer_amd/csrc/pt_capi_scene.cpp
--- a/optixpathtracer_amd/csrc/pt_capi_scene.cpp
+++ b/optixpathtracer_amd/csrc/pt_capi_scene.cpp
@@ -202,6 +202,7 @@
                "upload indices");
         if ((rc = sah_cost_now(r, true)) != PT_OK) return rc;
         if ((rc = lit_resubdivide(r)) != PT_OK) return rc;
+        if ((rc = skip_prepare(r)) != PT_OK) return rc;
     }
     PT_HIP(hipStreamSynchronize(r->stream), "hipStreamSynchronize");
     return PT_OK;
@@ -254,6 +255,7 @@
     else r->geom.refits++;
 
     if ((rc = lit_resubdivide(r)) != PT_OK) return rc;
+    if ((rc = skip_prepare(r)) != PT_OK) return rc;
     if (rebuild_rc != PT_OK) return fail(rebuild_rc, rebuild_msg);
     return PT_OK;
 }
diff --git a/optixpathtracer_amd/csrc/pt_capi_stats.cpp b/optixpathtracer_amd/csrc/pt_capi_stats.cpp
--- a/optixpathtracer_amd/csrc/pt_capi_stats.cpp
+++ b/optixpathtracer_amd/csrc/pt_capi_stats.cpp
@@ -41,7 +41,8 @@
     &pt_stats::shadow_rays, &pt_stats::trace_kernel_rays, &pt_stats::trace_kernel_bytes, &pt_stats::strict_retraces,
     &pt_stats::nee_unoccluded,
     &pt_stats::pair_kernel_rays, &pt_stats::pair_kernel_bytes, &pt_stats::pair_kernel_shadow_rays,
-    &pt_stats::lit_table_answers, &pt_stats::occluder_table_answers, &pt_stats::queue_bytes};
+    &pt_stats::lit_table_answers, &pt_stats::occluder_table_answers, &pt_stats::skip_table_rays,
+    &pt_stats::queue_bytes};
 
 int table_stats(pt_renderer* r, pt_stats* out) {
     r->lit.built.harvest();
@@ -73,6 +74,11 @@
         out->occluder_table_bytes = sizeof(int) * ne;
         out->occluder_table_candidates = (uint64_t)r->occ.built.count;
         out->occluder_table_build_ms = r->occ.built.build_ms;
+    }
+    r->skip.built.harvest();
+    if (skip_wanted(r) && r->skip.d_words && r->skip.built.current(r->skip.version, nullptr, 0)) {
+        out->skip_table_bytes = sizeof(uint32_t) * 2 * (size_t)r->ntri;
+        out->skip_table_build_ms = r->skip.built.build_ms;
     }
     return PT_OK;
 }
@@ -135,6 +141,7 @@
     out->look_ahead_held = r->ahead.held;
     out->lit_table_answers = c[kCtrLitAnswers];
     out->occluder_table_answers = c[kCtrOccAnswers];
+    out->skip_table_rays = c[kCtrSkipRays];
     if ((rc = table_stats(r, out)) != PT_OK) return rc;
     out->geometry_commits = r->geom.commits;
     out->geometry_refits = r->geom.refits;
diff --git a/optixpathtracer_amd/csrc/pt_capi_tables.cpp b/optixpathtracer_amd/csrc/pt_capi_tables.cpp
--- a/optixpathtracer_amd/csrc/pt_capi_tables.cpp
+++ b/optixpathtracer_amd/csrc/pt_capi_tables.cpp
@@ -1,4 +1,5 @@
 #include "pt_renderer.h"
+#include "pt_skip.h"
 
 using namespace pt;
 
@@ -82,6 +83,46 @@
     return occ_prepare(r);
 }
 
+#ifndef PT_SKIP_TABLE
+#define PT_SKIP_TABLE 1
+#endif
+bool skip_wanted(const pt_renderer* r) {
+    const bool has_code = r->material_mode == PT_MAT_LAMBERT || r->material_mode == PT_MAT_CONDUCTOR ||
+                          r->material_mode == PT_MAT_DIELECTRIC;
+    const bool pays = r->material_mode == PT_MAT_LAMBERT;
+    const bool on = r->skip.mode < 0 ? PT_SKIP_TABLE != 0 && pays : r->skip.mode > 0;
+    return on && has_code && r->skip.in_bounds && !r->skip.alloc_failed && r->ntri > 0 && r->bvh_nodes > 0;
+}
+int skip_prepare(pt_renderer* r) {
+    r->skip.active = skip_wanted(r);
+    if (!r->skip.active) return PT_OK;
+    if (r->skip.built.current(r->skip.version, nullptr, 0)) return PT_OK;
+    const size_t ntri = (size_t)r->ntri, nn = (size_t)r->bvh_nodes + 1;
+    if ((2 * ntri > r->skip.d_words.size() && r->skip.d_words.alloc(2 * ntri) != hipSuccess) ||
+        (nn > r->skip.d_node_parent.size() && r->skip.d_node_parent.alloc(nn) != hipSuccess) ||
+        (ntri > r->skip.d_tri_parent.size() && r->skip.d_tri_parent.alloc(ntri) != hipSuccess)) {
+        (void)hipGetLastError();
+        r->skip.alloc_failed = true;
+        r->skip.active = false;
+        return PT_OK;
+    }
+    int rc = r->skip.built.begin(r->stream);
+    if (rc != PT_OK) return rc;
+    PT_HIP(skip_build(r->scene(), r->skip.d_node_parent, r->skip.d_tri_parent, r->skip.d_words, r->stream), "skip_build");
+    return r->skip.built.end(r->stream, r->skip.version, nullptr, 0);
+}
+
+int skip_table_download(pt_renderer* r, int64_t* words_out, uint32_t* words, int64_t bytes) {
+    int rc = skip_prepare(r);
+    if (rc) return rc;
+    *words_out = r->skip.active ? 2 * (int64_t)r->ntri : 0;
+    if (!r->skip.active || !words) return PT_OK;
+    if (bytes != (int64_t)sizeof(uint32_t) * *words_out) return fail(PT_ERR_INVALID, "pt_skip_table_download: size mismatch");
+    PT_HIP(hipStreamSynchronize(r->stream), "hipStreamSynchronize");
+    PT_HIP(hipMemcpy(words, r->skip.d_words, (size_t)bytes, hipMemcpyDeviceToHost), "download skip table");
+    return PT_OK;
+}
+
 int lit_resubdivide(pt_renderer* r) {
     const size_t ntri = (size_t)r->ntri;
     std::vector<float4> isect_host(3 * ntri);
@@ -91,6 +132,11 @@
     float diag = 0.0f;
     r->lit.version++;
     r->lit.built.invalidate_count();
+    r->skip.version++;
+    r->skip.alloc_failed = false;
+    r->skip.in_bounds = true;
+    for (size_t t = 0; t < ntri && r->skip.in_bounds; ++t)
+        r->skip.in_bounds = skip_tri_in_bounds(reinterpret_cast<const float*>(isect_host.data()), (int)t);
     if (!lit_subdivide(isect_host.data(), (int)ntri, lit_words_host, &cells, &diag)) {
         r->lit.d_tri.reset();
         r->lit.cells = r->lit.words = 0;
diff --git a/optixpathtracer_amd/csrc/pt_device.h b/optixpathtracer_amd/csrc/pt_device.h
--- a/optixpathtracer_amd/csrc/pt_device.h
+++ b/optixpathtracer_amd/csrc/pt_device.h
@@ -59,6 +59,7 @@
     uint32_t lit_words;
     const int* occ_tab;
     uint32_t lit_cells;
+    const uint32_t* skip_tab;
 };
 enum Counter : int {
     kCtrSegments = 0,
@@ -85,9 +86,10 @@
     kCtrCohLanes = kCtrCoh0 + 6,
     kCtrLitAnswers,
     kCtrOccAnswers,
+    kCtrSkipRays,
     kCounters
 };
-static_assert(kCtrCoh0 == 20 && kCounters == 29, "the counter slots keep their numbers");
+static_assert(kCtrCoh0 == 20 && kCounters == 30, "the counter slots keep their numbers");
 constexpr int kDebugMaxBounces = 64;
 constexpr int kDebugRecordFloats = 22;
 
@@ -125,6 +127,7 @@
     uint32_t nodes = 0, tris = 0, rays = 0, overflow = 0, retrace = 0;
     uint32_t lds_nodes = 0;
     uint32_t unocc = 0;
+    uint32_t skips = 0;
     uint32_t steps = 0, active = 0, node_steps = 0, tri_steps = 0, refills = 0;
     uint32_t coh[6] = {0, 0, 0, 0, 0, 0};
     uint32_t coh_lanes = 0;
@@ -233,10 +236,11 @@
     bool any;
     bool strict;
     int path;
+    int skip;
     Hit h;
 };
 
-enum { kRayClosest = 0, kRayAny = 1, kRayMixed = 2 };
+enum { kRayClosest = 0, kRayAny = 1, kRayMixed = 2, kRayMixedSkip = 3 };
 
 __device__ __forceinline__ void trav_init(TravState& s, f3 o, f3 d, float tmin, float tmax) {
     s.o = o;
@@ -254,13 +258,14 @@
     s.leaf = kEmptyChild;
     s.any = false;
     s.strict = false;
+    s.skip = kEmptyChild;
     s.h.tri = -1;
     s.h.orig = 0x7fffffff;
 }
 
 template <int ANY>
 __device__ __forceinline__ bool is_any(const TravState& s) {
-    return ANY == kRayAny || (ANY == kRayMixed && s.any);
+    return ANY == kRayAny || ((ANY == kRayMixed || ANY == kRayMixedSkip) && s.any);
 }
 
 __device__ __forceinline__ bool tri_test(const float4 A, const float4 E1, const float4 E2, f3 o, f3 d, float tmin,
@@ -566,6 +571,8 @@
 template <int ANY, bool STATS, int DEPTH>
 __device__ __forceinline__ bool trav_node_step(const DevScene& S, TravState& s, int* __restrict__ stk, int stride,
                                                int* spill, TravStats& ts) {
+    constexpr bool kSkip = ANY == kRayMixedSkip;
+    if (kSkip && s.cur == s.skip) s.cur = kEmptyChild;
     if (s.cur >= 0) {
         if (STATS) {
             ts.nodes++;
@@ -599,7 +606,7 @@
         s.cur = c0;
     }
     if (s.cur == kEmptyChild) stack_pop<DEPTH>(s, stk, stride, spill);
-    if (s.cur < 0 && s.cur != kEmptyChild && s.leaf == kEmptyChild) {
+    if (s.cur < 0 && s.cur != kEmptyChild && (!kSkip || s.cur != s.skip) && s.leaf == kEmptyChild) {
         s.leaf = s.cur;
         stack_pop<DEPTH>(s, stk, stride, spill);
     }
@@ -669,6 +676,7 @@
 
 struct SurfaceHit {
     f3 pos, ng;
+    bool ng_back;
     Frame fr;
     f3 wo;
     f3 albedo;
@@ -731,7 +739,8 @@
         }
         Ns = normalize(Ns);
     }
-    if (dot(wo_w, Ng) < 0.0f) Ng = -Ng;
+    const bool ng_flip = dot(wo_w, Ng) < 0.0f;
+    if (ng_flip) Ng = -Ng;
     Ng = normalize(Ng);
     if (dot(Ng, Ns) < 0.0f) Ns = -Ns;
     Ns = normalize(Ns);
@@ -741,6 +750,7 @@
     }
     s.pos = mk(w * v0.x + u * v1.x + v * v2.x, w * v0.y + u * v1.y + v * v2.y, w * v0.z + u * v1.z + v * v2.z);
     s.ng = Ng;
+    s.ng_back = ng_flip != h.back;
     s.albedo = mk(M0.x, M0.y, M0.z);
     s.metallic = M0.w;
     s.roughness = M1.x;
diff --git a/optixpathtracer_amd/csrc/pt_internal.h b/optixpathtracer_amd/csrc/pt_internal.h
--- a/optixpathtracer_amd/csrc/pt_internal.h
+++ b/optixpathtracer_amd/csrc/pt_internal.h
@@ -93,6 +93,7 @@
                      const DevLight* lights, int n_lights, uint32_t* bits, float diag, hipStream_t stream);
 hipError_t occ_build(const DevScene& S, const uint32_t* tri_words, uint32_t cells, uint32_t words,
                      const DevLight* lights, int n_lights, const uint32_t* bits, int* occ, hipStream_t stream);
+hipError_t skip_build(const DevScene& S, int* node_parent, int* tri_parent, uint32_t* words, hipStream_t stream);
 
 struct RefitMesh {
     float m[16];
diff --git a/optixpathtracer_amd/csrc/pt_lit.hip b/optixpathtracer_amd/csrc/pt_lit.hip
--- a/optixpathtracer_amd/csrc/pt_lit.hip
+++ b/optixpathtracer_amd/csrc/pt_lit.hip
@@ -1,5 +1,6 @@
 #include "pt_internal.h"
 #include "pt_lit.h"
+#include "pt_skip.h"
 
 namespace pt {
 
@@ -165,6 +166,38 @@
     occ[id] = cand;
 }
 
+__global__ __launch_bounds__(kLitBlock) void k_skip_parents(const BNode4* __restrict__ nodes,
+                                                           const float4* __restrict__ isect, int n_nodes,
+                                                           int* __restrict__ node_parent, int* __restrict__ tri_parent) {
+    const int i = (int)(blockIdx.x * kLitBlock + threadIdx.x);
+    if (i < n_nodes && skip_parents_of(nodes, reinterpret_cast<const float*>(isect), i, node_parent, tri_parent))
+        atomicOr(&node_parent[n_nodes], 1);
+}
+
+__global__ __launch_bounds__(kLitBlock) void k_skip_build(DevScene S, const int* __restrict__ node_parent,
+                                                         const int* __restrict__ tri_parent,
+                                                         uint32_t* __restrict__ words) {
+    __shared__ int lds_stack[kLitStack * kLitBlock];
+    const int id = (int)(blockIdx.x * kLitBlock + threadIdx.x);
+    if (id >= 2 * S.ntri) return;
+    const int side = id >= S.ntri ? 1 : 0, t = id - side * S.ntri;
+    words[2 * t + side] = skip_word(S.nodes, reinterpret_cast<const float*>(S.isect), node_parent, tri_parent, t, side,
+                                    lds_stack + threadIdx.x, kLitBlock, kLitStack, node_parent[S.n_nodes] == 0);
+}
+
+}
+
+hipError_t skip_build(const DevScene& S, int* node_parent, int* tri_parent, uint32_t* words, hipStream_t stream) {
+    if (S.ntri <= 0 || S.n_nodes <= 0) return hipSuccess;
+    hipError_t e = hipMemsetAsync(node_parent + S.n_nodes, 0, sizeof(int), stream);
+    if (e != hipSuccess) return e;
+    hipLaunchKernelGGL(k_skip_parents, dim3((unsigned)((S.n_nodes + kLitBlock - 1) / kLitBlock)), dim3(kLitBlock), 0,
+                       stream, S.nodes, S.isect, S.n_nodes, node_parent, tri_parent);
+    e = hipGetLastError();
+    if (e != hipSuccess) return e;
+    hipLaunchKernelGGL(k_skip_build, dim3((unsigned)((2 * S.ntri + kLitBlock - 1) / kLitBlock)), dim3(kLitBlock), 0,
+                       stream, S, node_parent, tri_parent, words);
+    return hipGetLastError();
 }
 
 hipError_t occ_build(const DevScene& S, const uint32_t* tri_words, uint32_t cells, uint32_t words,
diff --git a/optixpathtracer_amd/csrc/pt_renderer.h b/optixpathtracer_amd/csrc/pt_renderer.h
--- a/optixpathtracer_amd/csrc/pt_renderer.h
+++ b/optixpathtracer_amd/csrc/pt_renderer.h
@@ -266,6 +266,16 @@
         bool active = false;
         pt::BuiltTable built;
     } occ;
+    struct Skip {
+        int mode = -1;
+        pt::DevBuf<uint32_t> d_words;
+        pt::DevBuf<int> d_node_parent, d_tri_parent;
+        uint32_t version = 1;
+        bool in_bounds = false;
+        bool alloc_failed = false;
+        bool active = false;
+        pt::BuiltTable built;
+    } skip;
 
     struct Aov {
         pt::DevBuf<float> d_albedo, d_normal, d_gnormal, d_position, d_depth, d_rough_metal;
@@ -369,6 +379,9 @@
                        int64_t bits_bytes);
 int occ_table_download(pt_renderer* r, int64_t* entries_out, int32_t* entries, int64_t bytes);
 int occ_table_upload(pt_renderer* r, const int32_t* entries, int64_t bytes);
+bool skip_wanted(const pt_renderer* r);
+int skip_prepare(pt_renderer* r);
+int skip_table_download(pt_renderer* r, int64_t* words_out, uint32_t* words, int64_t bytes);
 
 int collect_pending(pt_renderer* r);
 
diff --git a/optixpathtracer_amd/csrc/pt_skip.h b/optixpathtracer_amd/csrc/pt_skip.h
--- /dev/null
+++ b/optixpathtracer_amd/csrc/pt_skip.h
@@ -0,0 +1,160 @@
+#pragma once
+#include "pt_lit.h"
+
+namespace pt {
+
+constexpr float kSkipMinCos = 0.015625f;
+constexpr double kSkipMinAspectT = 0.0009765625;
+constexpr double kSkipMinAspect = 0.015625;
+constexpr int kSkipMaxTris = 4096;
+constexpr uint32_t kSkipNone = 0u;
+
+constexpr int kSkipNodeWords = 32;
+constexpr int kSkipEmptyChild = (int)0x80000000;
+PT_LIT_HD int skip_leaf_first(int c) { return (~c) >> 3; }
+PT_LIT_HD int skip_leaf_count(int c) { return ((~c) & 7) + 1; }
+
+PT_LIT_HD void skip_tri_vertices(const float* isect, int t, double a[3], double b[3], double c[3]) {
+    const float* r = isect + 12 * (size_t)t;
+    for (int k = 0; k < 3; ++k) {
+        a[k] = (double)r[k];
+        b[k] = (double)r[k] + (double)r[4 + k];
+        c[k] = (double)r[k] + (double)r[8 + k];
+    }
+}
+
+PT_LIT_HD double skip_aspect(const double a[3], const double b[3], const double c[3], double* lmax) {
+    const double e1[3] = {b[0] - a[0], b[1] - a[1], b[2] - a[2]}, e2[3] = {c[0] - a[0], c[1] - a[1], c[2] - a[2]};
+    const double e3[3] = {c[0] - b[0], c[1] - b[1], c[2] - b[2]};
+    const double nv[3] = {e1[1] * e2[2] - e1[2] * e2[1], e1[2] * e2[0] - e1[0] * e2[2], e1[0] * e2[1] - e1[1] * e2[0]};
+    const double l2 = fmax(e1[0] * e1[0] + e1[1] * e1[1] + e1[2] * e1[2],
+                           fmax(e2[0] * e2[0] + e2[1] * e2[1] + e2[2] * e2[2], e3[0] * e3[0] + e3[1] * e3[1] + e3[2] * e3[2]));
+    *lmax = sqrt(l2);
+    if (!(l2 > 0.0)) return 0.0;
+    return sqrt(nv[0] * nv[0] + nv[1] * nv[1] + nv[2] * nv[2]) / l2;
+}
+
+struct SkipOrigin {
+    LitPlane plane;
+};
+PT_LIT_HD bool skip_origin(const float* isect, int t, int side, SkipOrigin& T) {
+    double a[3], b[3], c[3], lmax;
+    skip_tri_vertices(isect, t, a, b, c);
+    if (!lit_plane_through(a, b, c, T.plane)) return false;
+    if (!(skip_aspect(a, b, c, &lmax) >= kSkipMinAspectT)) return false;
+    if (side) {
+        for (int k = 0; k < 3; ++k) T.plane.n[k] = -T.plane.n[k];
+        T.plane.d = -T.plane.d;
+    }
+    return true;
+}
+
+PT_LIT_HD bool skip_tri_below(const SkipOrigin& T, const double a[3], const double b[3], const double c[3]) {
+    const double ha = lit_dist(T.plane, a), hb = lit_dist(T.plane, b), hc = lit_dist(T.plane, c);
+    if (!(ha <= (double)kLitDelta && hb <= (double)kLitDelta && hc <= (double)kLitDelta)) return false;
+    double lmax;
+    return skip_aspect(a, b, c, &lmax) >= kSkipMinAspect;
+}
+
+PT_LIT_HD bool skip_leaf_below(const SkipOrigin& T, const float* isect, int code, int* budget) {
+    const int first = skip_leaf_first(code), cnt = skip_leaf_count(code);
+    for (int q = 0; q < cnt; ++q) {
+        double a[3], b[3], c[3];
+        skip_tri_vertices(isect, first + q, a, b, c);
+        --*budget;
+        if (!skip_tri_below(T, a, b, c)) return false;
+    }
+    return true;
+}
+
+PT_LIT_HD bool skip_subtree_below(const SkipOrigin& T, const void* nodes, const float* isect, int link, int* stk,
+                                  int stride, int cap, int* budget, bool box_accept) {
+    int sp = 0;
+    stk[0] = link;
+    sp = 1;
+    while (sp > 0) {
+        const int c = stk[(size_t)(--sp) * stride];
+        if (*budget <= 0) return false;
+        if (c < 0) {
+            if (!skip_leaf_below(T, isect, c, budget)) return false;
+            continue;
+        }
+        const float* f = (const float*)nodes + (size_t)kSkipNodeWords * c;
+        const int* ch = (const int*)nodes + (size_t)kSkipNodeWords * c + 24;
+        for (int q = 0; q < 4; ++q) {
+            if (ch[q] == kSkipEmptyChild) continue;
+            const double lo[3] = {f[q], f[8 + q], f[16 + q]}, hi[3] = {f[4 + q], f[12 + q], f[20 + q]};
+            if (lit_box_min(T.plane, lo, hi) > (double)kLitDelta) return false;
+            if (box_accept && lit_box_max(T.plane, lo, hi) <= (double)kLitDelta) continue;
+            if (sp >= cap) return false;
+            stk[(size_t)(sp++) * stride] = ch[q];
+        }
+    }
+    return true;
+}
+
+PT_LIT_HD bool skip_tri_sliver(const float* isect, int t) {
+    double a[3], b[3], c[3], lmax;
+    skip_tri_vertices(isect, t, a, b, c);
+    return !(skip_aspect(a, b, c, &lmax) >= kSkipMinAspect);
+}
+
+PT_LIT_HD bool skip_parents_of(const void* nodes, const float* isect, int ni, int* node_parent, int* tri_parent) {
+    bool sliver = false;
+    const int* ch = (const int*)nodes + (size_t)kSkipNodeWords * ni + 24;
+    if (ni == 0) node_parent[0] = -1;
+    for (int q = 0; q < 4; ++q) {
+        const int c = ch[q];
+        if (c == kSkipEmptyChild) continue;
+        if (c >= 0) {
+            node_parent[c] = (ni << 2) | q;
+        } else {
+            const int first = skip_leaf_first(c), cnt = skip_leaf_count(c);
+            for (int k = 0; k < cnt; ++k) {
+                tri_parent[first + k] = (ni << 2) | q;
+                sliver = sliver || skip_tri_sliver(isect, first + k);
+            }
+        }
+    }
+    return sliver;
+}
+
+PT_LIT_HD uint32_t skip_word(const void* nodes, const float* isect, const int* node_parent, const int* tri_parent,
+                             int t, int side, int* stk, int stride, int cap, bool box_accept) {
+    SkipOrigin T;
+    if (!skip_origin(isect, t, side, T)) return kSkipNone;
+    int budget = kSkipMaxTris;
+    int at = tri_parent[t];
+    const int* ch = (const int*)nodes + (size_t)kSkipNodeWords * (at >> 2) + 24;
+    if (!skip_leaf_below(T, isect, ch[at & 3], &budget)) return kSkipNone;
+    uint32_t best = (uint32_t)ch[at & 3];
+    for (int level = 0; level < 64; ++level) {
+        const int ni = at >> 2, slot = at & 3;
+        if (ni == 0) break;
+        const float* f = (const float*)nodes + (size_t)kSkipNodeWords * ni;
+        ch = (const int*)nodes + (size_t)kSkipNodeWords * ni + 24;
+        bool ok = true;
+        for (int q = 0; q < 4 && ok; ++q) {
+            if (q == slot || ch[q] == kSkipEmptyChild) continue;
+            const double lo[3] = {f[q], f[8 + q], f[16 + q]}, hi[3] = {f[4 + q], f[12 + q], f[20 + q]};
+            if (lit_box_min(T.plane, lo, hi) > (double)kLitDelta) ok = false;
+            else if (box_accept && lit_box_max(T.plane, lo, hi) <= (double)kLitDelta) ok = true;
+            else ok = skip_subtree_below(T, nodes, isect, ch[q], stk, stride, cap, &budget, box_accept);
+        }
+        if (!ok) break;
+        at = node_parent[ni];
+        best = (uint32_t)ni;
+    }
+    return best;
+}
+
+PT_LIT_HD bool skip_tri_in_bounds(const float* isect, int t) {
+    const float* r = isect + 12 * (size_t)t;
+    for (int k = 0; k < 3; ++k) {
+        if (!(fabsf(r[k]) <= kLitMaxCoord && fabsf(r[k] + r[4 + k]) <= kLitMaxCoord && fabsf(r[k] + r[8 + k]) <= kLitMaxCoord))
+            return false;
+    }
+    return true;
+}
+
+}
diff --git a/optixpathtracer_amd/csrc/pt_wavefront.hip b/optixpathtracer_amd/csrc/pt_wavefront.hip
--- a/optixpathtracer_amd/csrc/pt_wavefront.hip
+++ b/optixpathtracer_amd/csrc/pt_wavefront.hip
@@ -3,6 +3,7 @@
 
 #include "pt_internal.h"
 #include "pt_lit.h"
+#include "pt_skip.h"
 
 namespace pt {
 
@@ -84,6 +85,7 @@
     const unsigned long long a = wave_sum_u64(ts.nodes), c = wave_sum_u64(ts.tris), d = wave_sum_u64(ts.rays);
     const unsigned long long e = wave_sum_u64(ts.overflow), r = wave_sum_u64(ts.retrace);
     const unsigned long long l = wave_sum_u64(ts.lds_nodes), u = wave_sum_u64(ts.unocc);
+    const unsigned long long sk = wave_sum_u64(ts.skips);
     if (lane_id() == 0) {
         atomicAdd(&counters[kCtrNodes], a);
         atomicAdd(&counters[kCtrTriTests], c);
@@ -97,6 +99,7 @@
         atomicAdd(&counters[kCtrWaveRefills], (unsigned long long)ts.refills);
         atomicAdd(&counters[kCtrLdsNodes], l);
         atomicAdd(&counters[kCtrNeeUnoccluded], u);
+        atomicAdd(&counters[kCtrSkipRays], sk);
         for (int k = 0; k < 6; ++k) atomicAdd(&counters[kCtrCoh0 + k], (unsigned long long)ts.coh[k]);
         atomicAdd(&counters[kCtrCohLanes], (unsigned long long)ts.coh_lanes);
     }
@@ -545,6 +548,24 @@
     return tri_accept(A, E1, E2, inv, mk(o.x * inv.x, o.y * inv.y, o.z * inv.z), th);
 }
 
+template <int MODE>
+constexpr bool kSkipCode = MODE == kModeLambert || MODE == kModeConductor || MODE == kModeDielectric;
+__device__ __forceinline__ uint2 skip_words(const DevLaunch& L, int tri) {
+    return reinterpret_cast<const uint2*>(L.skip_tab)[tri];
+}
+__device__ __forceinline__ uint2 skip_orient(uint2 w, const SurfaceHit& sf) {
+    return sf.ng_back ? make_uint2(w.y, w.x) : w;
+}
+template <int MODE>
+__device__ __forceinline__ bool skip_under(const BSample& bs) {
+    return MODE != kModeLambert && dot(bs.dir, mk(0.0f, 0.0f, 1.0f)) < 0.0f;
+}
+__device__ __forceinline__ uint32_t skip_pick(uint2 w, const SurfaceHit& sf, bool under, f3 d) {
+    const float up = dot(d, sf.ng);
+    const bool climbs = (under ? -up : up) > kSkipMinCos;
+    return climbs ? (under ? w.y : w.x) : 0u;
+}
+
 __device__ __forceinline__ int vis0_index(const DevLaunch& L, int path, int li) {
     const int P1 = L.width * L.height;
     return li * P1 + path % P1;
@@ -593,6 +614,7 @@
     __shared__ int lds_occ[kOcc ? kWaves : 1];
     const bool lit = !vis0 && L.lit_tri;
     const bool occ = kOcc && lit && L.occ_tab;
+    const bool skip = kSkipCode<MODE> && L.skip_tab;
     if (blockIdx.x == 0 && threadIdx.x == 0 && L.counters) atomicAdd(&L.counters[kCtrShadeItems], (unsigned long long)n);
     if ((int)(blockIdx.x * kBlock) >= n) return;
     {
@@ -604,6 +626,7 @@
         float stmax = 0.0f;
         int path = 0;
         int occ_t = -1;
+        uint32_t skip_w = 0;
         const int P1 = L.width * L.height;
         float4 l0 = make_float4(0.0f, 0.0f, 0.0f, 0.0f);
         if (valid) {
@@ -614,6 +637,7 @@
             const Hit h = decode_hit(hv);
             if (h.tri >= 0) {
                 const int lit_c = lit ? lit_cell(L, h) : -1;
+                const uint2 skip2 = skip ? skip_words(L, h.tri) : make_uint2(0u, 0u);
                 const float4 c = shade0 ? ldqs(rd + path % P1) : c_q;
                 d = mk(c.x, c.y, c.z);
                 SurfaceHit sf;
@@ -668,6 +692,7 @@
                     bsdf_sample<MODE>(seed, sf.albedo, sf.roughness, conductor, sf.wo, bs)) {
                     emit_next = continue_path(sf, bs, beta, o, d, b + 1, L.max_bounces);
                     if (!kBetaQ) stqs(W.beta + path, make_float4(beta.x, beta.y, beta.z, __uint_as_float(seed)));
+                    if (kSkipCode<MODE> && skip) skip_w = skip_pick(skip_orient(skip2, sf), sf, skip_under<MODE>(bs), d);
                 }
             }
         }
@@ -677,7 +702,7 @@
         if (lit) lit_count_block<kWaves>(L, lds_lit);
         if (emit_next) {
             stqs(no + qi, make_float4(o.x, o.y, o.z, __int_as_float(path)));
-            stqs(nd + qi, make_float4(d.x, d.y, d.z, 0.0f));
+            stqs(nd + qi, make_float4(d.x, d.y, d.z, __uint_as_float(skip_w)));
             if (kBetaQ) stqs(queue_beta(W, b + 1) + qi, make_float4(beta.x, beta.y, beta.z, __uint_as_float(seed)));
         }
         if constexpr (kOcc) {
@@ -714,13 +739,17 @@
     const bool valid = p < P1 && !wf_cancelled(W);
     int tri = -1;
     SurfaceHit sf;
+    const bool skip = kSkipCode<MODE> && L.skip_tab;
+    uint2 skip2 = make_uint2(0u, 0u);
     if (valid) {
         const float4 hv = W.hit[p];
         const Hit h = decode_hit(hv);
         tri = h.tri;
         if (tri >= 0) {
+            if (skip) skip2 = skip_words(L, tri);
             const float4 c = W.ray_d[0][p];
             reconstruct<TEX>(S, h, mk(c.x, c.y, c.z), sf);
+            skip2 = skip_orient(skip2, sf);
         }
     }
     const int dbg = debug_path_id(L);
@@ -732,6 +761,7 @@
         f3 o, d, beta = mk(1.0f, 1.0f, 1.0f);
         uint32_t seed = 0;
         float4 l0 = make_float4(0.0f, 0.0f, 0.0f, 0.0f);
+        bool under = false;
         if (valid && tri >= 0) {
             seed = tea16((uint32_t)(p + L.width * L.row0), L.frame_base + (uint32_t)f);
             if (path == dbg) debug_record(L, 1, __float_as_int(S.isect[3 * tri].w), sf, beta, mk(0.0f, 0.0f, 0.0f));
@@ -756,19 +786,21 @@
             if (1 < L.max_bounces && bsdf_sample<MODE>(seed, sf.albedo, sf.roughness, conductor, sf.wo, bs)) {
                 emit_next = continue_path(sf, bs, beta, o, d, 1, L.max_bounces);
                 if (!kBetaQ) stqs(W.beta + path, make_float4(beta.x, beta.y, beta.z, __uint_as_float(seed)));
+                if (kSkipCode<MODE> && skip) under = skip_under<MODE>(bs);
             }
         }
         if (valid) stqs(W.L + path, l0);
         const int qi = block_append<kWaves>(cnt(W, 1, kQueue), emit_next, lds_q);
         if (emit_next) {
             stqs(no + qi, make_float4(o.x, o.y, o.z, __int_as_float(path)));
-            stqs(nd + qi, make_float4(d.x, d.y, d.z, 0.0f));
+            const uint32_t skip_w = (kSkipCode<MODE> && skip) ? skip_pick(skip2, sf, under, d) : 0u;
+            stqs(nd + qi, make_float4(d.x, d.y, d.z, __uint_as_float(skip_w)));
             if (kBetaQ) stqs(queue_beta(W, 1) + qi, make_float4(beta.x, beta.y, beta.z, __uint_as_float(seed)));
         }
     }
 }
 
-template <bool STATS, bool TEX, int BLK = kBlockTrace>
+template <bool STATS, bool TEX, int BLK = kBlockTrace, bool SKIP = false>
 __global__ __launch_bounds__(BLK, wf_waves(TEX)) void k_trace_pair(DevScene S, WFState W, int b,
                                                                       unsigned long long* counters) {
     const int n_ext = *cnt(W, b + 1, kQueue);
@@ -781,6 +813,11 @@
             const float4 a = ldqs(ro + i), c = ldqs(rd + i);
             trav_init(st, mk(a.x, a.y, a.z), mk(c.x, c.y, c.z), 0.0f, 100.0f);
             st.path = __float_as_int(a.w);
+            if (SKIP) {
+                const int w = __float_as_int(c.w);
+                st.skip = w != 0 ? w : kEmptyChild;
+                if (STATS) ts.skips += w != 0;
+            }
         } else {
             const int j = i - n_ext;
             const float4 c = ldqs(W.sh_d + j), k = ldqs(W.sh_c + j);
@@ -828,7 +865,7 @@
         pool.begin = pool.end = n_all;
     }
     wave_slice(pool.begin, first, end);
-    trace_queue<kRayMixed, STATS, TEX, BLK>(S, first, end, ts, W, fetch, finish, commit, pool);
+    trace_queue<SKIP ? kRayMixedSkip : kRayMixed, STATS, TEX, BLK>(S, first, end, ts, W, fetch, finish, commit, pool);
     if (blockIdx.x == 0 && threadIdx.x == 0 && counters) {
         atomicAdd(&counters[kCtrSegments], (unsigned long long)n_ext);
         atomicAdd(&counters[kCtrShadowRays], (unsigned long long)n_sh);
@@ -1350,7 +1387,9 @@
     auto pair = [&](int b) -> hipError_t {
         return trace_timed([&] {
             return trace_variant(tex, wide_trace, stats, [&](auto tx, auto st, auto blk) {
-                return trace_launch(k_trace_pair<st(), tx(), blk()>, blk(), S, W, b, L.counters);
+                return with_flag(L.skip_tab != nullptr, [&](auto sk) {
+                    return trace_launch(k_trace_pair<st(), tx(), blk(), sk()>, blk(), S, W, b, L.counters);
+                });
             });
         });
     };
diff --git a/optixpathtracer_amd/renderer.py b/optixpathtracer_amd/renderer.py
--- a/optixpathtracer_amd/renderer.py
+++ b/optixpathtracer_amd/renderer.py
@@ -374,6 +374,18 @@
         check(self.lib.pt_occluder_table_download(self.h, C.byref(n), e.ctypes.data, e.nbytes), "pt_occluder_table_download")
         return e
 
+    def set_skip_table(self, enable: bool | None) -> None:
+        check(self.lib.pt_set_skip_table(self.h, -1 if enable is None else (1 if enable else 0)), "pt_set_skip_table")
+
+    def skip_table(self):
+        n = C.c_int64(0)
+        check(self.lib.pt_skip_table_download(self.h, C.byref(n), None, 0), "pt_skip_table_download")
+        if n.value == 0:
+            return None
+        w = np.empty(n.value, np.uint32)
+        check(self.lib.pt_skip_table_download(self.h, C.byref(n), w.ctypes.data, w.nbytes), "pt_skip_table_download")
+        return w.reshape(-1, 2)
+
     def upload_occluder_table(self, entries) -> None:
         e = np.ascontiguousarray(entries, np.int32)
         check(self.lib.pt_occluder_table_upload(self.h, e.ctypes.data, e.nbytes), "pt_occluder_table_upload")
```

Result: faster. 1928 Msamples/sec, median of 6 (+8.6%).
